# Lolash/graphSAGE-pytorch

Hardware: AMD Instinct MI355X
Metric: sampled nodes/sec (2-layer, fanout 25,10) at 1/2/4/8 MI355X (higher is better)
Workload: dtype fp32

## Files before the change

graphsage-pytorch_amd/_lib.py:

```python
import ctypes
import os

import torch

_HERE = os.path.dirname(os.path.abspath(__file__))
_ASAN_LIB = os.environ.get("GS_HOST_ASAN_LIB")
LIB_PATH = _ASAN_LIB or os.path.join(_HERE, "libgraphsage_amd.so")

GS_OK, GS_EINVAL, GS_ENOMEM, GS_EHIP, GS_ERANGE, GS_EEMPTY, GS_ELIMIT = range(7)
GS_F32, GS_BF16 = 0, 1
GS_AGG_MEAN, GS_AGG_MAX = 0, 1
GS_SAMPLE_GCN, GS_SAMPLE_FULL = 1, 2
GS_DSAMPLER_NO_AUX = 8
GS_DSAMPLER_FAST = 16
GS_SAMPLE_FAIL_EMPTY = 4
GS_MAX_HOPS = 8
GS_TOPT_FUSED_BWD, GS_TOPT_TOP_LAUNCH, GS_TOPT_SELF_ROWS, GS_TOPT_DEFER_UPDATE = range(4)
GS_OPT_SGD, GS_OPT_ADAM = 0, 1
(GS_PK_POS_PTR, GS_PK_POS, GS_PK_DST_IDS, GS_PK_NBR_PTR, GS_PK_NBR, GS_PK_SELF,
 GS_PK_TPTR, GS_PK_TIDX, GS_PK_NFIELDS) = range(9)

_i32, _i64, _u32, _u64, _f32, _f64 = (ctypes.c_int32, ctypes.c_int64, ctypes.c_uint32,
                                      ctypes.c_uint64, ctypes.c_float, ctypes.c_double)
_vp = ctypes.c_void_p
_p = ctypes.POINTER


class HopView(ctypes.Structure):
    _fields_ = [
        ("n_dst", _i64), ("n_pos", _i64), ("n_src", _i64), ("n_nbr", _i64),
        ("dst_ids", _p(_i64)), ("pos_ptr", _p(_i32)), ("pos", _p(_i32)),
        ("src_ids", _p(_i64)), ("nbr_ptr", _p(_i32)), ("nbr", _p(_i32)),
        ("self_local", _p(_i32)), ("set_ptr", _p(_i32)), ("set_items", _p(_i64)),
        ("n_empty", _i64),
    ]


class PackLayout(ctypes.Structure):
    _fields_ = [("total", _i64), ("off", (_i64 * GS_PK_NFIELDS) * GS_MAX_HOPS)]


_SIGS = {
    "gs_last_error": (ctypes.c_char_p, []),
    "gs_version": (ctypes.c_char_p, []),
    "gs_rng_create": (_i32, [_p(_vp)]),
    "gs_rng_destroy": (None, [_vp]),
    "gs_rng_seed_words": (_i32, [_vp, _vp, _i64]),
    "gs_rng_set_state": (_i32, [_vp, _vp, _i64]),
    "gs_rng_get_state": (_i32, [_vp, _vp, _p(_i64)]),
    "gs_rng_getrandbits": (_i32, [_vp, _i32, _i64, _vp]),
    "gs_rng_randbelow": (_i32, [_vp, _u32, _i64, _vp]),
    "gs_rng_sample_positions": (_i32, [_vp, _i64, _i64, _vp]),
    "gs_rng_choice_position": (_i32, [_vp, _i64, _p(_i64)]),
    "gs_pyset_union_of_lists": (_i32, [_vp, _vp, _i64, _vp, _p(_i64)]),
    "gs_graph_build": (_i32, [_vp, _vp, _i64, _i64, _i32, _p(_vp)]),
    "gs_graph_from_tables": (_i32, [_i64, _vp, _vp, _vp, _vp, _vp, _p(_vp)]),
    "gs_graph_destroy": (None, [_vp]),
    "gs_graph_dims": (_i32, [_vp, _p(_i64), _p(_i64), _p(_i64)]),
    "gs_graph_row_ptr": (_vp, [_vp]),
    "gs_graph_col": (_vp, [_vp]),
    "gs_graph_image_bytes": (_i64, [_vp]),
    "gs_graph_write_image": (_i32, [_vp, _vp, _i64]),
    "gs_graph_from_image": (_i32, [_vp, _i64, _p(_vp)]),
    "gs_rmat_pairs": (_i32, [_i32, _i64, _f64, _f64, _f64, _u64, _i32, _i32, _vp, _vp, _p(_i64)]),
    "gs_sample_run": (_i32, [_vp, _vp, _vp, _i64, _vp, _i32, _i32, _p(_vp)]),
    "gs_sample_destroy": (None, [_vp]),
    "gs_sample_n_hops": (_i32, [_vp, _p(_i32)]),
    "gs_sample_hop": (_i32, [_vp, _i32, _p(HopView)]),
    "gs_sample_pack_layout": (_i32, [_vp, _p(PackLayout)]),
    "gs_sample_pack": (_i32, [_vp, _vp, _i64]),
    "gs_sample_pack_bound": (_i64, [_vp, _i64, _vp, _i32]),
    "gs_sample_pack_run": (_i32, [_vp, _vp, _vp, _i64, _vp, _i32, _i32, _vp, _i64, _vp, _vp, _p(_i64)]),
    "gs_sample_pack_bound_multi": (_i64, [_vp, _i64, _i64, _vp, _i32]),
    "gs_sample_pack_run_multi": (_i32, [_vp, _vp, _vp, _i64, _i64, _vp, _i32, _i32, _vp, _i64, _vp, _vp,
                                        _p(_i64)]),
    "gs_fsample_pack_run": (_i32, [_vp, _u64, _i64, _vp, _i64, _vp, _i32, _i32, _vp, _i64, _vp, _vp, _p(_i64)]),
    "gs_philox4x32": (_i32, [_vp, _vp, _vp]),
    "gs_team_create": (_i32, [_i32, _p(_vp)]),
    "gs_team_create_shared": (_i32, [_vp, _p(_vp)]),
    "gs_team_destroy": (None, [_vp]),
    "gs_sample_pack_run_multi_team": (_i32, [_vp, _vp, _vp, _i64, _i64, _vp, _i32, _i32, _vp, _i64, _vp,
                                             _vp, _p(_i64), _vp]),
    "gs_fill_uniform": (_i32, [_vp, _i32, _i64, _i64, _i64, _u64, _vp]),
    "gs_uniform_host": (_i32, [_u64, _i64, _i64, _i64, _vp]),
    "gs_agg_fwd": (_i32, [_i32, _i32, _vp, _i64, _i64, _i64, _vp, _vp, _vp, _vp, _vp, _i32,
                          _vp, _i32, _i64, _vp, _vp]),
    "gs_sage_linear_fwd": (_i32, [_i32, _i64, _i64, _i64, _vp, _i64, _vp, _vp, _i64, _vp, _vp,
                                  _i64, _i32, _vp]),
    "gs_sage_linear_bwd_weight_ws": (_i64, [_i64, _i64, _i64]),
    "gs_sage_linear_bwd_weight": (_i32, [_i32, _i64, _i64, _i64, _vp, _i64, _vp, _vp, _i64, _vp,
                                         _vp, _i64, _i32, _vp, _vp, _i64, _vp]),
    "gs_sage_linear_bwd_input": (_i32, [_i64, _i64, _i64, _vp, _vp, _i64, _i32, _vp, _vp, _vp,
                                        _i64, _vp]),
    "gs_agg_bwd": (_i32, [_i32, _i64, _i64, _vp, _vp, _vp, _vp, _vp, _i64, _vp, _vp, _i64, _vp,
                          _vp]),
    "gs_sage1_fwd_supported": (_i32, [_i32, _i64, _i64, _i32]),
    "gs_sage1_fwd": (_i32, [_i32, _i32, _vp, _i64, _i64, _i64, _i64, _vp, _vp, _vp, _vp, _i32,
                            _vp, _vp, _i64, _vp, _i64, _i32, _vp]),
    "gs_cls_nll_ws_floats": (_i64, [_i64, _i64, _i64]),
    "gs_cls_nll_fwd_bwd": (_i32, [_i64, _i64, _i64, _vp, _vp, _vp, _vp, _vp, _i32, _vp, _vp, _vp,
                                  _vp, _vp, _vp]),
    "gs_clip_sgd": (_i32, [_i32, _vp, _vp, _vp, _f32, _f32, _f32, _vp, _vp]),
    "gs_clip_adam": (_i32, [_i32, _vp, _vp, _vp, _vp, _vp, _f32, _f32, _f32, _f32, _f32, _f32, _f32, _i64, _vp,
                            _vp]),
    "gs_unsup_create": (_i32, [_vp, _vp, _i64, _i32, _i32, _i32, _p(_vp)]),
    "gs_unsup_destroy": (None, [_vp]),
    "gs_unsup_attach_device": (_i32, [_vp, _vp]),
    "gs_unsup_extend": (_i32, [_vp, _vp, _vp, _i64, _i64, _i32, _i32, _vp]),
    "gs_unsup_fetch": (_i32, [_vp, _vp, _vp, _vp, _vp, _vp, _vp]),
    "gs_unsup_loss_plan": (_i32, [_vp, _vp, _i64, _vp, _p(_i64)]),
    "gs_unsup_loss_ws_floats": (_i64, [_i64, _i64, _i64]),
    "gs_unsup_loss_fwd": (_i32, [_i32, _i64, _i64, _i64, _i64, _i64, _vp, _i64, _vp, _f32, _f32, _vp, _vp,
                                 _vp]),
    "gs_unsup_loss_bwd": (_i32, [_i64, _i64, _i64, _i64, _i64, _vp, _i64, _vp, _vp, _vp, _vp, _i64, _vp]),
    "gs_cast_f32_bf16": (_i32, [_vp, _vp, _i64, _vp]),
    "gs_trainer_create": (_i32, [_vp, _p(_vp)]),
    "gs_trainer_destroy": (None, [_vp]),
    "gs_trainer_n_params": (_i64, [_vp]),
    "gs_trainer_ws_bytes": (_i64, [_vp, _vp]),
    "gs_trainer_forward_backward": (_i32, [_vp, _vp, _vp, _vp, _vp, _i64, _vp, _i64, _vp, _vp]),
    "gs_trainer_update": (_i32, [_vp, _f32, _vp, _vp]),
    "gs_trainer_update_local": (_i32, [_vp, _vp]),
    "gs_trainer_defer": (_i32, [_vp, _i32, _p(_i32), _vp]),
    "gs_trainer_gather_reserve": (_i32, [_vp, _i64, _i32]),
    "gs_trainer_gather": (_i32, [_vp, _vp, _vp, _vp, _i32, _vp]),
    "gs_trainer_forward_backward_gathered": (_i32, [_vp, _vp, _vp, _vp, _vp, _i64, _i32, _vp, _i64, _vp, _vp]),
    "gs_trainer_forward": (_i32, [_vp, _vp, _vp, _vp, _vp, _i64, _vp, _vp]),
    "gs_trainer_forward_gathered": (_i32, [_vp, _vp, _vp, _vp, _i32, _vp, _i64, _vp, _vp]),
    "gs_trainer_time_agg": (_i32, [_vp, _i64]),
    "gs_trainer_agg_times": (_i64, [_vp, _vp, _i64]),
    "gs_trainer_kernel_times": (_i64, [_vp, _i32, _vp, _i64]),
    "gs_trainer_kernel_block_stats": (_i64, [_vp, _i32, _vp, _i64]),
    "gs_trainer_kernel_stamps": (_i64, [_vp, _i32, _i64, _vp, _vp]),
    "gs_trainer_time_kernels": (_i32, [_vp, _i32, _i64]),
    "gs_trainer_time_kernels_every": (_i32, [_vp, _i32, _i64, _i64]),
    "gs_trainer_kernel_name": (ctypes.c_char_p, [_vp, _i32]),
    "gs_trainer_grads": (_vp, [_vp]),
    "gs_trainer_set_option": (_i32, [_vp, _i32, _i32]),
    "gs_trainer_set_optimizer": (_i32, [_vp, _vp]),
    "gs_trainer_opt_step": (_i64, [_vp]),
    "gs_trainer_capture": (_i32, [_vp, _vp, _i64, _vp, _i64]),
    "gs_trainer_captured": (_i64, [_vp]),
    "gs_comm_unique_id": (_i32, [_vp]),
    "gs_comm_create": (_i32, [_vp, _i32, _i32, _p(_vp)]),
    "gs_comm_destroy": (None, [_vp]),
    "gs_comm_allreduce_sum": (_i32, [_vp, _vp, _i64, _vp]),
    "gs_runner_create": (_i32, [_vp, _p(_vp)]),
    "gs_runner_run": (_i32, [_vp, _i64, _vp, _vp]),
    "gs_runner_stats_get": (_i32, [_vp, _vp]),
    "gs_runner_stats_reset": (None, [_vp]),
    "gs_runner_destroy": (None, [_vp]),
    "gs_runner_release": (_i32, [_vp, _i64]),
    "gs_runner_progress": (_i32, [_vp, _p(_i64), _p(_i64)]),
    "gs_runner_sync_rngs": (_i32, [_vp]),
    "gs_dsampler_create": (_i32, [_vp, _vp, _i32, _i64, _i32, _p(_vp)]),
    "gs_dsampler_destroy": (None, [_vp]),
    "gs_dsampler_set_rng": (_i32, [_vp, _vp, _i64, _vp]),
    "gs_dsampler_get_rng": (_i32, [_vp, _vp, _p(_i64), _vp]),
    "gs_dsampler_words": (_i32, [_vp, _i64, _vp, _vp]),
    "gs_dsampler_pack_bound": (_i64, [_vp, _i64]),
    "gs_dsampler_run": (_i32, [_vp, _vp, _i64, _vp, _i64, _vp]),
    "gs_dsampler_result": (_i32, [_vp, _vp, _vp, _p(_i64)]),
    "gs_dsampler_runs": (_i64, [_vp]),
    "gs_dsampler_result_of": (_i32, [_vp, _i64, _vp, _vp, _p(_i64)]),
    "gs_dsampler_debug": (_i32, [_vp, _vp, _i32]),
    "gs_dsampler_set_seed": (_i32, [_vp, _u64]),
    "gs_dsampler_run_at": (_i32, [_vp, _i64, _vp, _i64, _vp, _i64, _vp]),
    "gs_full_plan_create": (_i32, [_vp, _vp, _i64, _i32, _i64, _p(_vp)]),
    "gs_full_plan_destroy": (None, [_vp]),
    "gs_full_plan_dims": (_i32, [_vp, _vp]),
    "gs_full_plan_array": (_vp, [_vp, _i32]),
    "gs_agg_full_ws_bytes": (_i64, [_vp, _i64, _i64, _i64]),
    "gs_agg_full": (_i32, [_vp, _vp, _i32, _i32, _vp, _i64, _i64, _vp, _vp, _i64, _i64, _vp, _i64, _vp, _i64,
                           _vp]),
    "gs_infer_full_ws_bytes": (_i64, [_vp, _vp]),
    "gs_infer_full": (_i32, [_vp, _vp, _vp, _vp, _i64, _vp, _i64, _vp]),
    "gs_full_plan_transpose": (_i32, [_vp, _vp, _vp, _i64, _p(_vp)]),
    "gs_agg_full_argmax_ws_bytes": (_i64, [_vp, _i64, _i64, _i64]),
    "gs_agg_full_argmax": (_i32, [_vp, _vp, _i32, _vp, _i64, _i64, _vp, _vp, _i64, _i64, _vp, _i64, _vp, _i64, _vp,
                                  _i64, _vp]),
    "gs_agg_full_bwd_ws_bytes": (_i64, [_vp, _i64]),
    "gs_agg_full_bwd": (_i32, [_vp, _vp, _i32, _i64, _vp, _vp, _vp, _vp, _i64, _vp, _i64, _vp, _vp, _i64, _vp, _i64,
                               _vp]),
    "gs_train_full_ws_offset": (_i64, [_vp, _vp, _vp, _i32, _i32]),
    "gs_train_full_ws_bytes": (_i64, [_vp, _vp, _vp]),
    "gs_train_full_forward_backward": (_i32, [_vp, _vp, _vp, _vp, _vp, _vp, _i64, _i32, _i32, _vp, _vp, _i64, _vp]),
    "gs_full_field_bytes": (_i64, [_vp, _vp, _i32]),
    "gs_full_field_offset": (_i64, [_vp, _vp, _i32, _i32, _i32]),
    "gs_full_field_build": (_i32, [_vp, _vp, _vp, _vp, _vp, _vp, _vp, _i64, _i32, _vp, _vp]),
    "gs_full_field_counts": (_i32, [_vp, _vp, _vp, _vp]),
    "gs_agg_full_field": (_i32, [_vp, _vp, _vp, _vp, _i32, _i32, _i32, _vp, _i64, _i64, _vp, _vp, _vp, _i64, _vp,
                                 _i64, _vp, _i64, _vp]),
    "gs_agg_full_bwd_field": (_i32, [_vp, _vp, _vp, _vp, _i32, _i32, _i64, _vp, _vp, _vp, _vp, _i64, _vp, _i64, _vp,
                                     _i64, _vp, _i64, _vp, _i64, _vp]),
    "gs_train_full_field_forward_backward": (_i32, [_vp, _vp, _vp, _vp, _vp, _vp, _vp, _i64, _i32, _i32, _vp, _vp,
                                                    _i64, _vp]),
    "gs_train_full_unsup_ws_bytes": (_i64, [_i32, _i64, _i64, _i64, _i64]),
    "gs_train_full_unsup_forward_backward": (_i32, [_vp, _vp, _vp, _vp, _vp, _vp, _vp, _i64, _vp, _vp, _i64, _i32,
                                                    _i32, _vp, _vp, _i64, _vp]),
}

(GS_FP_N_NODES, GS_FP_N_ITEMS, GS_FP_N_SLOTS, GS_FP_N_SPLIT, GS_FP_N_EMPTY, GS_FP_SEG_LEN, GS_FP_GCN,
 GS_FP_N_ENTRIES, GS_FP_NDIMS) = range(9)
(GS_FP_ITEMS, GS_FP_ITEM_PTR, GS_FP_SLOT_PTR, GS_FP_SPLIT_PTR, GS_FP_SPLIT_ROWS, GS_FP_COUNT, GS_FP_SELF_LOOP,
 GS_FP_EMPTY_ROWS) = range(8)
GS_FP_T_ROW_PTR, GS_FP_T_COL = 8, 9
GS_TF_FORWARD, GS_TF_HEAD, GS_TF_BACKWARD, GS_TF_ALL = 1, 2, 4, 7
GS_FF_LAYER0, GS_FF_NCOUNTS = GS_MAX_HOPS + 1, GS_MAX_HOPS + 1 + 4 * GS_MAX_HOPS
GS_FF_ROWS, GS_FF_POS, GS_FF_ITEMS, GS_FF_SPLIT, GS_FF_T_ITEMS, GS_FF_T_SPLIT = range(6)


class FullPlanDev(ctypes.Structure):
    _fields_ = [("items", _vp), ("slot_ptr", _vp), ("split_rows", _vp), ("count", _vp), ("self_loop", _vp)]


class FullField(ctypes.Structure):
    _fields_ = [("n_layers", _i32), ("pad_", _i32), ("buf", _vp), ("buf_bytes", _i64), ("counts", _i64 * GS_FF_NCOUNTS)]


class InferFullConfig(ctypes.Structure):
    _fields_ = [
        ("n_layers", _i32), ("hidden", _i32), ("agg", _i32), ("feat_dtype", _i32),
        ("feat_dim", _i64), ("feat_ld", _i64), ("X", _vp), ("row_ptr", _vp), ("col", _vp),
        ("W", _vp * GS_MAX_HOPS), ("chunk_rows", _i64),
    ]


class TrainFullConfig(ctypes.Structure):
    _fields_ = [
        ("n_layers", _i32), ("hidden", _i32), ("n_classes", _i32), ("agg", _i32), ("feat_dtype", _i32),
        ("pad_", _i32), ("feat_dim", _i64), ("feat_ld", _i64), ("max_nodes", _i64), ("X", _vp), ("row_ptr", _vp),
        ("col", _vp), ("t_row_ptr", _vp), ("t_col", _vp), ("labels", _vp), ("params", _vp), ("grads", _vp),
    ]


class TrainFullUnsup(ctypes.Structure):
    _fields_ = [
        ("kind", _i32), ("with_sup", _i32), ("M", _i64), ("P", _i64), ("N", _i64), ("plan", _vp), ("q", _f32),
        ("margin", _f32),
    ]


class TrainerConfig(ctypes.Structure):
    _fields_ = [
        ("n_layers", _i32), ("hidden", _i32), ("n_classes", _i32), ("agg", _i32), ("gcn", _i32),
        ("feat_dtype", _i32), ("feat_dim", _i64), ("feat_ld", _i64),
        ("X", _vp), ("row_ptr", _vp), ("col", _vp), ("labels", _vp), ("params", _vp), ("grads", _vp),
        ("lr", _f32), ("max_norm", _f32),
    ]


class OptimizerConfig(ctypes.Structure):
    _fields_ = [
        ("kind", _i32), ("beta1", _f32), ("beta2", _f32), ("eps", _f32), ("weight_decay", _f32),
        ("m", _vp), ("v", _vp), ("step", _i64),
    ]


class RunnerConfig(ctypes.Structure):
    _fields_ = [
        ("graph", _vp), ("trainer", _vp), ("batches", _vp), ("n_batches", _i64), ("batch", _i64),
        ("fanouts", _vp), ("n_hops", _i32), ("flags", _i32), ("n_streams", _i32), ("rngs", _vp),
        ("depth", _i32), ("comm", _vp), ("world", _i32), ("embed_out", _vp), ("embed_ld", _i64),
        ("merge", _i32), ("hold", _i32), ("ar_buckets", _i32), ("helpers", _i32), ("warm", _i32),
        ("device_sampler", _i32), ("sampler_seed", _u64),
    ]


class RunnerStats(ctypes.Structure):
    _fields_ = [
        ("steps", _i64), ("wait_s", ctypes.c_double), ("issue_s", ctypes.c_double),
        ("sample_s", ctypes.c_double), ("hop_sizes", ctypes.c_double * (4 * GS_MAX_HOPS)),
        ("wait_sample_s", ctypes.c_double), ("wait_ring_s", ctypes.c_double),
        ("wait_gather_s", ctypes.c_double), ("fwd_bwd_s", ctypes.c_double), ("update_s", ctypes.c_double),
        ("max_step_s", ctypes.c_double), ("lookahead_misses", _i64),
    ]


_lib = None


class LibraryMissing(RuntimeError):
    pass


class DeviceLimit(RuntimeError):
    """GS_ELIMIT: a device-path capacity (the device sampler's rejection
    windows, walks or frontier tables) was too small for this batch.  The
    batch itself is valid and the caller's stream state is untouched, so the
    host path computes the same result."""


_DIAGNOSTIC = {"gs_trainer_kernel_block_stats", "gs_trainer_kernel_stamps"}


def lib():
    global _lib
    if _lib is None:
        if not os.path.exists(LIB_PATH):
            raise LibraryMissing(
                f"{LIB_PATH} is not built; run __graft_entry__.build() or "
                "`make -C graphsage-pytorch_amd/csrc` (no CPU fallback exists)")
        L = ctypes.CDLL(LIB_PATH)
        for name, (res, args) in _SIGS.items():
            if (_ASAN_LIB or name in _DIAGNOSTIC) and not hasattr(L, name):
                continue
            fn = getattr(L, name)
            fn.restype = res
            fn.argtypes = args
        _lib = L
    return _lib


def exported_symbols():
    return list(_SIGS)


def check(rc, what=""):
    if rc == GS_OK:
        return
    msg = lib().gs_last_error().decode(errors="replace") or what
    if rc in (GS_EINVAL,):
        raise ValueError(msg)
    if rc == GS_ERANGE:
        raise (ValueError if "Sample larger" in msg else IndexError)(msg)
    if rc == GS_EEMPTY:
        raise IndexError(msg)
    if rc == GS_ENOMEM:
        raise MemoryError(msg)
    if rc == GS_ELIMIT:
        raise DeviceLimit(msg)
    raise RuntimeError(msg)


def ptr(t):
    if t is None:
        return None
    if isinstance(t, torch.Tensor):
        return t.data_ptr()
    return t.ctypes.data


def stream_ptr(device=None):
    return torch.cuda.current_stream(device).cuda_stream
```

graphsage-pytorch_amd/csrc/kernels/agg.hip:

```cpp
#include "agg_dev.hpp"
#include "internal.hpp"

#include <algorithm>
#include <cstdlib>

namespace gs {

__global__ __launch_bounds__(kBlock) void resolve_ids_kernel(int n_dst, int k, const int* __restrict__ ptr,
                                                             const int* __restrict__ ent,
                                                             const int* __restrict__ col,
                                                             const int* __restrict__ dst_ids, int gcn,
                                                             int* __restrict__ ids) {
    const int64_t t = blockIdx.x * int64_t(kBlock) + threadIdx.x;
    if (t >= static_cast<int64_t>(n_dst) * k) return;
    const int r = static_cast<int>(t / k), j = static_cast<int>(t - static_cast<int64_t>(r) * k);
    const int e = ptr[r] + j;
    int nb = -1;
    if (e < ptr[r + 1]) nb = col[ent[e]];
    if (!gcn && nb == dst_ids[r]) nb = -1;
    ids[t] = nb;
}

__global__ __launch_bounds__(kBlock) void resolve_top_kernel(int n_dst, int k, const int* __restrict__ ptr,
                                                             const int* __restrict__ ent,
                                                             const int* __restrict__ col,
                                                             const int* __restrict__ dst_ids, int gcn,
                                                             int* __restrict__ ids, int n_top, int tk,
                                                             const int* __restrict__ tptr,
                                                             const int* __restrict__ tnbr,
                                                             const int* __restrict__ tself, int* __restrict__ tout,
                                                             int n_rec, const int* __restrict__ rptr,
                                                             const int* __restrict__ ridx, int* __restrict__ rout) {
    const int64_t t = blockIdx.x * int64_t(kBlock) + threadIdx.x;
    const int64_t n1 = static_cast<int64_t>(n_dst) * k;
    if (t < n1) {
        const int r = static_cast<int>(t / k), j = static_cast<int>(t - static_cast<int64_t>(r) * k);
        const int e = ptr[r] + j;
        int nb = -1;
        if (e < ptr[r + 1]) nb = col[ent[e]];
        if (!gcn && nb == dst_ids[r]) nb = -1;
        ids[t] = nb;
        return;
    }
    const int64_t u = t - n1;
    const int64_t n2 = static_cast<int64_t>(n_top) * (tk + 1);
    if (u >= n2) {
        const int64_t q = u - n2;
        if (q >= static_cast<int64_t>(n_rec) * 8) return;
        const int c = static_cast<int>(q >> 3), j = static_cast<int>(q & 7);
        const int b = rptr[c], n = rptr[c + 1] - b;
        rout[q] = j == 0 ? n : j == 1 ? b : (j - 2 < n ? ridx[b + j - 2] : 0);
        return;
    }
    const int r = static_cast<int>(u / (tk + 1)), j = static_cast<int>(u - static_cast<int64_t>(r) * (tk + 1));
    int v;
    if (j == 0) {
        v = tself[r];
    } else {
        const int e = tptr[r] + j - 1;
        v = e < tptr[r + 1] ? tnbr[e] : -1;
    }
    tout[u] = v;
}

template <typename T, int VEC>
struct RawVec {
    using type = T;
    static __device__ __forceinline__ void unpack(const T& r, float (&v)[VEC]) {
        RowIO<T, VEC>::load(&r, v);
    }
};
template <>
struct RawVec<float, 4> {
    using type = float4;
    static __device__ __forceinline__ void unpack(const float4& r, float (&v)[4]) {
        v[0] = r.x; v[1] = r.y; v[2] = r.z; v[3] = r.w;
    }
};
template <>
struct RawVec<bf16_t, 8> {
    using type = uint4;
    static __device__ __forceinline__ void unpack(const uint4& r, float (&v)[8]) {
        const uint32_t w[4] = {r.x, r.y, r.z, r.w};
#pragma unroll
        for (int i = 0; i < 4; ++i) {
            v[2 * i] = __uint_as_float(w[i] << 16);
            v[2 * i + 1] = __uint_as_float(w[i] & 0xffff0000u);
        }
    }
};

template <int OP, typename T, int VEC, int G, bool SELF, bool ONE, int NR1 = kRows>
__global__ __launch_bounds__(kBlock) void agg_ids_kernel(const T* __restrict__ X, int64_t ldx, int F, int n_dst, int k,
                                                         const int* __restrict__ ids, const int* __restrict__ dst_ids,
                                                         int gcn, T* __restrict__ out, int64_t ldo,
                                                         T* __restrict__ self_out, int64_t ldso) {
    const int gl = threadIdx.x % G;
    if constexpr (ONE) {
        using Raw = typename RawVec<T, VEC>::type;
        constexpr int NR = NR1;
        static_assert(NR % 4 == 0 && NR <= kRows, "row loads: whole chunks of 4");
        const int r = blockIdx.x * (kBlock / G) + threadIdx.x / G;
        if (r >= n_dst) return;
        const int f0 = gl * VEC;
        const int node = SELF ? dst_ids[r] : 0;
        const int nb = gl < k ? ids[static_cast<int64_t>(r) * k + gl] : -1;
        int rows[NR];
        bool ok[NR];
#pragma unroll
        for (int u = 0; u < NR; ++u) {
            rows[u] = __shfl(nb, u, G);
            ok[u] = u < k && rows[u] >= 0;
        }
        const int fallback = SELF ? node : (rows[0] >= 0 ? rows[0] : 0);
        Raw xself{};
        if (SELF) xself = *reinterpret_cast<const Raw*>(X + static_cast<int64_t>(node) * ldx + f0);
        Raw x[NR];
#pragma unroll
        for (int u = 0; u < NR; ++u)
            x[u] = *reinterpret_cast<const Raw*>(X + static_cast<int64_t>(ok[u] ? rows[u] : fallback) * ldx + f0);
        __builtin_amdgcn_sched_barrier(0);
        float acc[VEC];
#pragma unroll
        for (int v = 0; v < VEC; ++v) acc[v] = (OP == GS_AGG_MAX) ? -INFINITY : 0.f;
        int cnt = 0;
        int ka = k;
        asm volatile("" : "+s"(ka));
#pragma unroll
        for (int q = 0; q < NR / 4; ++q)
            if (4 * q < ka) {
#pragma unroll
                for (int u = 4 * q; u < 4 * q + 4; ++u) {
                    cnt += ok[u];
                    float xv[VEC];
                    RawVec<T, VEC>::unpack(x[u], xv);
#pragma unroll
                    for (int v = 0; v < VEC; ++v) {
                        if (OP == GS_AGG_MEAN) {
                            acc[v] += ok[u] ? xv[v] : 0.f;
                        } else {
                            const bool take = ok[u] && xv[v] > acc[v];
                            acc[v] = take ? xv[v] : acc[v];
                        }
                    }
                }
            }
        if (SELF) *reinterpret_cast<Raw*>(self_out + static_cast<int64_t>(r) * ldso + f0) = xself;
        if (OP == GS_AGG_MEAN) {
            const float inv = 1.0f / static_cast<float>(cnt);
#pragma unroll
            for (int v = 0; v < VEC; ++v) acc[v] *= inv;
        }
        RowIO<T, VEC>::store(out + static_cast<int64_t>(r) * ldo + f0, acc);
        return;
    }
    for (int r = blockIdx.x * (kBlock / G) + threadIdx.x / G; r < n_dst; r += gridDim.x * (kBlock / G)) {
    const int node = (gcn || SELF) ? dst_ids[r] : 0;
    const int* rid = ids + static_cast<int64_t>(r) * k;
    constexpr int NR = kRows;
    const int nf = (F + G * VEC - 1) / (G * VEC);
    for (int fi = 0; fi < nf; ++fi) {
        const int f0 = fi * G * VEC + gl * VEC;
        const bool act = f0 < F;
        const int f0c = act ? f0 : 0;
        using Raw = typename RawVec<T, VEC>::type;
        Raw xself{};
        if (SELF) xself = *reinterpret_cast<const Raw*>(X + static_cast<int64_t>(node) * ldx + f0c);
        float acc[VEC];
#pragma unroll
        for (int v = 0; v < VEC; ++v) acc[v] = (OP == GS_AGG_MAX) ? -INFINITY : 0.f;
        int cnt = 0;
        bool self_seen = false;
        for (int base = 0; base < k; base += G) {
            const int m = min(G, k - base);
            const bool mine = gl < m;
            const int nb = rid[mine ? base + gl : base];
            if (gcn) self_seen |= group_bits<G>(mine && nb == node) != 0;
            const int my = mine ? nb : -1;
            for (int j = 0; j < m; j += NR) {
                int rows[NR];
                bool ok[NR];
#pragma unroll
                for (int u = 0; u < NR; ++u) {
                    rows[u] = __shfl(my, j + u < m ? j + u : j, G);
                    ok[u] = (j + u < m) && rows[u] >= 0;
                }
                const int fallback = rows[0] >= 0 ? rows[0] : node;
                Raw x[NR];
#pragma unroll
                for (int u = 0; u < NR; ++u)
                    x[u] = *reinterpret_cast<const Raw*>(X + static_cast<int64_t>(ok[u] ? rows[u] : fallback) * ldx + f0c);
#pragma unroll
                for (int u = 0; u < NR; ++u) {
                    cnt += ok[u];
                    float xv[VEC];
                    RawVec<T, VEC>::unpack(x[u], xv);
#pragma unroll
                    for (int v = 0; v < VEC; ++v) {
                        if (OP == GS_AGG_MEAN) {
                            acc[v] += ok[u] ? xv[v] : 0.f;
                        } else {
                            const bool take = ok[u] && xv[v] > acc[v];
                            acc[v] = take ? xv[v] : acc[v];
                        }
                    }
                }
            }
        }
        if (gcn && !self_seen) {
            ++cnt;
            float x[VEC];
            RowIO<T, VEC>::load(X + static_cast<int64_t>(node) * ldx + f0c, x);
#pragma unroll
            for (int v = 0; v < VEC; ++v) {
                if (OP == GS_AGG_MEAN) acc[v] += x[v];
                else acc[v] = x[v] > acc[v] ? x[v] : acc[v];
            }
        }
        if (!act) continue;
        if (SELF) *reinterpret_cast<Raw*>(self_out + static_cast<int64_t>(r) * ldso + f0) = xself;
        if (OP == GS_AGG_MEAN) {
            const float inv = 1.0f / static_cast<float>(cnt);
#pragma unroll
            for (int v = 0; v < VEC; ++v) acc[v] *= inv;
        }
        RowIO<T, VEC>::store(out + static_cast<int64_t>(r) * ldo + f0, acc);
    }
    }
}

void resolve_ids_launch(int64_t n_dst, int k, const int32_t* ptr, const int32_t* ent, const int32_t* col,
                        const int32_t* dst_ids, int gcn, int32_t* ids, hipStream_t st) {
    GS_REQUIRE(n_dst >= 0 && k >= 1 && n_dst * k < (int64_t(1) << 31), GS_EINVAL, "bad sizes");
    if (n_dst == 0) return;
    const int64_t total = n_dst * k;
    resolve_ids_kernel<<<dim3(static_cast<unsigned>((total + kBlock - 1) / kBlock)), kBlock, 0, st>>>(
        static_cast<int>(n_dst), k, ptr, ent, col, dst_ids, gcn, ids);
    check_launch("resolve_ids");
}

void resolve_top_launch(int64_t n_dst, int k, const int32_t* ptr, const int32_t* ent, const int32_t* col,
                        const int32_t* dst_ids, int gcn, int32_t* ids, int64_t n_top, int tk, const int32_t* tptr,
                        const int32_t* tnbr, const int32_t* tself, int32_t* tout, hipStream_t st, int64_t n_rec,
                        const int32_t* rptr, const int32_t* ridx, int32_t* rout) {
    GS_REQUIRE(n_dst >= 0 && k >= 1 && n_dst * k < (int64_t(1) << 31) && n_top >= 0 && tk >= 1 &&
                   n_top * (tk + 1) < (int64_t(1) << 30) && n_rec >= 0 && n_rec < (int64_t(1) << 27) &&
                   (n_rec == 0 || (rptr && ridx && rout)),
               GS_EINVAL, "bad sizes");
    const int64_t total = n_dst * k + n_top * (tk + 1) + n_rec * 8;
    if (total == 0) return;
    resolve_top_kernel<<<dim3(static_cast<unsigned>((total + kBlock - 1) / kBlock)), kBlock, 0, st>>>(
        static_cast<int>(n_dst), k, ptr, ent, col, dst_ids, gcn, ids, static_cast<int>(n_top), tk, tptr, tnbr, tself,
        tout, static_cast<int>(n_rec), rptr, ridx, rout);
    check_launch("resolve_top");
}

static int agg_ids_block_cap() { return 1 << 30; }

void agg_ids_launch(gs_agg op, gs_dtype dt, const void* X, int64_t ldx, int64_t F, int64_t n_dst, int k,
                    const int32_t* ids, const int32_t* dst_ids, int gcn, void* out, int64_t ldo, hipStream_t st,
                    void* self_out, int64_t ldso, LaunchTimer* timer) {
    GS_REQUIRE(op == GS_AGG_MEAN || op == GS_AGG_MAX, GS_EINVAL, "agg_func must be MEAN or MAX");
    GS_REQUIRE(F >= 1 && n_dst >= 0 && k >= 1 && ldx >= F && ldo >= F, GS_EINVAL, "bad sizes");
    GS_REQUIRE(!self_out || (dst_ids && ldso >= F), GS_EINVAL, "self rows need dst_ids and ldso >= F");
    if (n_dst == 0) return;
    const int V = dt == GS_F32 ? 4 : 8;
    const bool vec = F % V == 0 && ldx % V == 0 && ldo % V == 0 && aligned16(X) && aligned16(out) &&
                     (!self_out || (ldso % V == 0 && aligned16(self_out)));
    const int f = static_cast<int>(F), n = static_cast<int>(n_dst);
    static const int cap = agg_ids_block_cap();
#define GS_IDS2(OPV, TT, VV, GG, ONE, NRV)                                                                       \
    do {                                                                                                         \
        const dim3 grid_(std::min((n + (kBlock / GG) - 1) / (kBlock / GG), cap));                                \
        if (self_out)                                                                                            \
            launch_k(timer, agg_ids_kernel<OPV, TT, VV, GG, true, ONE, NRV>, grid_, dim3(kBlock), 0, st,         \
                     static_cast<const TT*>(X), ldx, f, n, k, ids, dst_ids, gcn, static_cast<TT*>(out), ldo,      \
                     static_cast<TT*>(self_out), ldso);                                                          \
        else                                                                                                     \
            launch_k(timer, agg_ids_kernel<OPV, TT, VV, GG, false, ONE, NRV>, grid_, dim3(kBlock), 0, st,        \
                     static_cast<const TT*>(X), ldx, f, n, k, ids, dst_ids, gcn, static_cast<TT*>(out), ldo,      \
                     static_cast<TT*>(nullptr), ldso);                                                           \
    } while (0)
#define GS_IDS1(OPV, TT, VV, GG, ONE)                                                                            \
    do {                                                                                                         \
        if (!(ONE)) GS_IDS2(OPV, TT, VV, GG, false, kRows);                                                      \
        else if (k <= 4) GS_IDS2(OPV, TT, VV, GG, true, 4);                                                      \
        else if (k <= 8) GS_IDS2(OPV, TT, VV, GG, true, 8);                                                      \
        else if (k <= 12) GS_IDS2(OPV, TT, VV, GG, true, 12);                                                    \
        else GS_IDS2(OPV, TT, VV, GG, true, kRows);                                                              \
    } while (0)
    const bool one_ok = !gcn && k <= kRows && static_cast<int64_t>(n + 1) * 64 < (int64_t(1) << 31) &&
                        cap >= (n + 3) / 4;
#define GS_IDS(OPV, TT, VV, GG)                                      \
    do {                                                             \
        if (one_ok && f == (GG) * (VV)) GS_IDS1(OPV, TT, VV, GG, true); \
        else GS_IDS1(OPV, TT, VV, GG, false);                        \
    } while (0)
#define GS_IDS_T(OPV, TT)                                                     \
    do {                                                                      \
        constexpr int VV = sizeof(TT) == 4 ? 4 : 8;                           \
        if (!vec) GS_IDS(OPV, TT, 1, 64);                                     \
        else {                                                                \
            const int G = pick_group(f, VV);                                  \
            if (G == 16) GS_IDS(OPV, TT, VV, 16);                             \
            else if (G == 32) GS_IDS(OPV, TT, VV, 32);                        \
            else GS_IDS(OPV, TT, VV, 64);                                     \
        }                                                                     \
    } while (0)
    if (op == GS_AGG_MEAN) {
        if (dt == GS_F32) GS_IDS_T(GS_AGG_MEAN, float);
        else GS_IDS_T(GS_AGG_MEAN, bf16_t);
    } else {
        if (dt == GS_F32) GS_IDS_T(GS_AGG_MAX, float);
        else GS_IDS_T(GS_AGG_MAX, bf16_t);
    }
#undef GS_IDS_T
#undef GS_IDS
#undef GS_IDS1
#undef GS_IDS2
    check_launch("agg_ids");
}

template <int OP, typename T, bool EXPAND>
static void launch_fwd(int vec, const T* X, int64_t ldx, int F, int n_dst, const int* ptr,
                       const int* idx, const int64_t* row_ptr, const int* col, const int* dst_ids,
                       int gcn, T* out, int64_t ldo, int* am, hipStream_t st, LaunchTimer* timer) {
    constexpr int V = sizeof(T) == 4 ? 4 : 8;
    if (vec == 1) {
        const dim3 grid((n_dst + (kBlock / 64) - 1) / (kBlock / 64));
        launch_k(timer, agg_fwd_kernel<OP, T, 1, 64, EXPAND>, grid, dim3(kBlock), 0, st, X, ldx, F, n_dst, ptr, idx,
                 row_ptr, col, dst_ids, gcn, out, ldo, am);
        return;
    }
    const int G = pick_group(F, V);
    const dim3 grid((n_dst + (kBlock / G) - 1) / (kBlock / G));
#define GS_AGG_FWD(GG)                                                                                   \
    launch_k(timer, agg_fwd_kernel<OP, T, V, GG, EXPAND>, grid, dim3(kBlock), 0, st, X, ldx, F, n_dst, ptr, idx, \
             row_ptr, col, dst_ids, gcn, out, ldo, am)
    if (G == 16) GS_AGG_FWD(16);
    else if (G == 32) GS_AGG_FWD(32);
    else GS_AGG_FWD(64);
#undef GS_AGG_FWD
}

template <int OP>
static void launch_bwd(int vec, int n_src, int F, const int* tptr, const int* tidx, const int* ptr,
                       const float* dA, const float* dSelf, int64_t ldd, const int* am,
                       const float* Hprev, int64_t ldh, float* dH, hipStream_t st) {
    if (vec == 1) {
        const dim3 grid((n_src + 3) / 4);
        agg_bwd_kernel<OP, 1, 64><<<grid, kBlock, 0, st>>>(n_src, F, tptr, tidx, ptr, dA, dSelf, ldd, am,
                                                           Hprev, ldh, dH);
        return;
    }
    const int G = pick_group(F, 4);
    const dim3 grid((n_src + (kBlock / G) - 1) / (kBlock / G));
#define GS_AGG_BWD(GG)                                                                          \
    agg_bwd_kernel<OP, 4, GG><<<grid, kBlock, 0, st>>>(n_src, F, tptr, tidx, ptr, dA, dSelf, ldd, am, \
                                                       Hprev, ldh, dH)
    if (G == 16) GS_AGG_BWD(16);
    else if (G == 32) GS_AGG_BWD(32);
    else GS_AGG_BWD(64);
#undef GS_AGG_BWD
}

void agg_fwd_launch(gs_agg op, gs_dtype xdt, const void* X, int64_t ldx, int64_t F, int64_t n_dst,
                    const int32_t* ptr, const int32_t* idx, const int64_t* row_ptr, const int32_t* col,
                    const int32_t* dst_ids, int32_t gcn, void* out, gs_dtype odt, int64_t ldo, int32_t* argmax,
                    hipStream_t st, LaunchTimer* timer) {
    GS_REQUIRE(op == GS_AGG_MEAN || op == GS_AGG_MAX, GS_EINVAL, "agg_func must be MEAN or MAX");
    GS_REQUIRE(xdt == odt, GS_EINVAL, "output dtype must equal feature dtype");
    GS_REQUIRE(F >= 1 && F < (1 << 30) && n_dst >= 0 && n_dst < (int64_t(1) << 31), GS_EINVAL, "bad sizes");
    GS_REQUIRE(ldx >= F && ldo >= F, GS_EINVAL, "leading dimension smaller than F");
    if (n_dst == 0) return;
    GS_REQUIRE(X && ptr && idx && out, GS_EINVAL, "NULL device pointer");
    const bool expand = col != nullptr;
    GS_REQUIRE(!expand || dst_ids, GS_EINVAL, "expand mode needs dst_ids");
    GS_REQUIRE(!(argmax && expand), GS_EINVAL, "argmax is only produced in explicit mode");
    const int V = xdt == GS_F32 ? 4 : 8;
    const int vec = (F % V == 0 && ldx % V == 0 && ldo % V == 0 && aligned16(X) && aligned16(out)) ? V : 1;
    const int f = static_cast<int>(F), n = static_cast<int>(n_dst);
#define GS_DISPATCH(OPV, TT)                                                                              \
    do {                                                                                                  \
        if (expand)                                                                                       \
            launch_fwd<OPV, TT, true>(vec, static_cast<const TT*>(X), ldx, f, n, ptr, idx, row_ptr, col,  \
                                      dst_ids, gcn, static_cast<TT*>(out), ldo, nullptr, st, timer);      \
        else                                                                                              \
            launch_fwd<OPV, TT, false>(vec, static_cast<const TT*>(X), ldx, f, n, ptr, idx, nullptr,      \
                                       nullptr, nullptr, 0, static_cast<TT*>(out), ldo, argmax, st, timer); \
    } while (0)
    if (op == GS_AGG_MEAN) {
        if (xdt == GS_F32) GS_DISPATCH(GS_AGG_MEAN, float);
        else GS_DISPATCH(GS_AGG_MEAN, bf16_t);
    } else {
        if (xdt == GS_F32) GS_DISPATCH(GS_AGG_MAX, float);
        else GS_DISPATCH(GS_AGG_MAX, bf16_t);
    }
#undef GS_DISPATCH
    check_launch("gs_agg_fwd");
}

}

extern "C" {

int gs_agg_fwd(gs_agg op, gs_dtype xdt, const void* X, int64_t ldx, int64_t F, int64_t n_dst,
               const int32_t* ptr, const int32_t* idx, const int64_t* row_ptr, const int32_t* col,
               const int32_t* dst_ids, int32_t gcn, void* out, gs_dtype odt, int64_t ldo,
               int32_t* argmax, void* stream) {
    GS_API_BEGIN
    gs::agg_fwd_launch(op, xdt, X, ldx, F, n_dst, ptr, idx, row_ptr, col, dst_ids, gcn, out, odt, ldo, argmax,
                       gs::as_stream(stream));
    GS_API_END
}

int gs_agg_bwd(gs_agg op, int64_t n_src, int64_t F, const int32_t* tptr, const int32_t* tidx,
               const int32_t* ptr, const float* dA, const float* dSelf, int64_t ldd,
               const int32_t* argmax, const float* Hprev, int64_t ldh, float* dH, void* stream) {
    GS_API_BEGIN
    using namespace gs;
    GS_REQUIRE(op == GS_AGG_MEAN || op == GS_AGG_MAX, GS_EINVAL, "agg_func must be MEAN or MAX");
    GS_REQUIRE(F >= 1 && n_src >= 0 && n_src < (int64_t(1) << 31), GS_EINVAL, "bad sizes");
    GS_REQUIRE(ldd >= F && ldh >= F, GS_EINVAL, "leading dimension smaller than F");
    if (n_src == 0) return GS_OK;
    GS_REQUIRE(tptr && tidx && ptr && dA && dH, GS_EINVAL, "NULL device pointer");
    GS_REQUIRE(op != GS_AGG_MAX || argmax, GS_EINVAL, "MAX backward needs argmax");
    const int vec = (F % 4 == 0 && ldd % 4 == 0 && ldh % 4 == 0 && aligned16(dA) && (!dSelf || aligned16(dSelf)) &&
                     aligned16(dH) && (!Hprev || aligned16(Hprev)))
                        ? 4
                        : 1;
    hipStream_t st = as_stream(stream);
    if (op == GS_AGG_MEAN)
        launch_bwd<GS_AGG_MEAN>(vec, static_cast<int>(n_src), static_cast<int>(F), tptr, tidx, ptr, dA, dSelf,
                                ldd, argmax, Hprev, ldh, dH, st);
    else
        launch_bwd<GS_AGG_MAX>(vec, static_cast<int>(n_src), static_cast<int>(F), tptr, tidx, ptr, dA, dSelf,
                               ldd, argmax, Hprev, ldh, dH, st);
    check_launch("gs_agg_bwd");
    GS_API_END
}

}
```

graphsage-pytorch_amd/csrc/kernels/internal.hpp:

```cpp
#pragma once
#include <functional>

#include "kcommon.hpp"

struct gs_trainer;
struct gs_dsampler;

namespace gs {

void trainer_set_upper_hook(gs_trainer* t, std::function<void(hipStream_t)> hook);
void trainer_set_w1_chunk_hook(gs_trainer* t, int chunks,
                               std::function<void(hipStream_t, int64_t, int64_t)> hook);
void trainer_keep_lowp(gs_trainer* t, bool keep);
bool trainer_defer_update(gs_trainer* t, bool on, hipStream_t st, bool comm = false);
int64_t trainer_w1_floats(const gs_trainer* t);
void trainer_set_done(gs_trainer* t, int64_t* ptr, int64_t value);
bool trainer_done_taken(const gs_trainer* t);

bool linear_fwd_wide_ok(gs_dtype dt, int64_t F, const void* Xs, int64_t ldxs, const void* A, int64_t lda,
                        const void* W);
void linear_fwd_launch(gs_dtype dt, int64_t n, int64_t F, int64_t H, const void* Xs, int64_t ldxs,
                       const int32_t* sidx, const void* A, int64_t lda, const void* Wd, float* out, int64_t ldo,
                       int32_t relu, hipStream_t st, const FwdSpec* pend = nullptr, LaunchTimer* timer = nullptr);
int linear_dw_slabs(gs_dtype dt, int64_t n, int64_t F, int64_t H, const void* Xs, int64_t ldxs,
                    const int32_t* sidx, const void* A, int64_t lda, const float* dout, const float* out,
                    int64_t ldo, int32_t relu, float* dW, void* ws, int64_t ws_bytes, hipStream_t st,
                    int64_t H_split = -1, int phases = 1, LaunchTimer* timer = nullptr);
inline constexpr int kDw1Phases = 2;
int sum_slabs_launch(const float* slabs, int S, int64_t len, float* out, float* part, hipStream_t st);
struct SlabSum {
    const float* slabs;
    int S;
    int64_t len;
    float* out;
    float* part;
};
bool sum_slabs_pair_ok(int64_t len1, int64_t len2);
int sum_slabs_pair_parts2(int64_t len2);
int sum_slabs_pair_launch(const SlabSum& s1, const SlabSum& s2, hipStream_t st, const float* spec_P = nullptr,
                          float* spec_S = nullptr, float lr = 0.f, uint16_t* spec_S_lp = nullptr, DoneFlag done = {},
                          LaunchTimer* timer = nullptr);
void spec_finalize_launch(const FwdSpec& sp, float* w1_out, int64_t w1_floats, hipStream_t st);
int sum_slabs_grid(int64_t len);

void resolve_ids_launch(int64_t n_dst, int k, const int32_t* ptr, const int32_t* ent, const int32_t* col,
                        const int32_t* dst_ids, int gcn, int32_t* ids, hipStream_t st);
void resolve_top_launch(int64_t n_dst, int k, const int32_t* ptr, const int32_t* ent, const int32_t* col,
                        const int32_t* dst_ids, int gcn, int32_t* ids, int64_t n_top, int tk, const int32_t* tptr,
                        const int32_t* tnbr, const int32_t* tself, int32_t* tout, hipStream_t st, int64_t n_rec = 0,
                        const int32_t* rptr = nullptr, const int32_t* ridx = nullptr, int32_t* rout = nullptr);
void trainer_reserve_top(gs_trainer* t, int64_t B, int32_t tk);
void agg_ids_launch(gs_agg op, gs_dtype dt, const void* X, int64_t ldx, int64_t F, int64_t n_dst, int k,
                    const int32_t* ids, const int32_t* dst_ids, int gcn, void* out, int64_t ldo, hipStream_t st,
                    void* self_out = nullptr, int64_t ldso = 0, LaunchTimer* timer = nullptr);
void agg_fwd_launch(gs_agg op, gs_dtype xdt, const void* X, int64_t ldx, int64_t F, int64_t n_dst,
                    const int32_t* ptr, const int32_t* idx, const int64_t* row_ptr, const int32_t* col,
                    const int32_t* dst_ids, int32_t gcn, void* out, gs_dtype odt, int64_t ldo, int32_t* argmax,
                    hipStream_t st, LaunchTimer* timer = nullptr);

int cls_rows_launch(int64_t B, int64_t D, int64_t C, const float* E, const float* Wc, const float* bc,
                    const int32_t* labels, const int32_t* roots, int32_t mask_relu, float* dE, float* ws,
                    hipStream_t st);
void sgd_with_parts(int32_t n_groups, const int64_t* goff_host, const int* npart, int pstride, float* params,
                    float* grads, const float* part, float grad_scale, float max_norm, float lr, hipStream_t st,
                    LowpShadow shadow = {}, DoneFlag done = {});
void clip_sgd_launch(int32_t n_groups, const int64_t* goff_host, float* params, float* grads, float grad_scale,
                     float max_norm, float lr, float* ws, hipStream_t st, LowpShadow shadow = {}, DoneFlag done = {});
struct AdamStep {
    float lr, beta1, beta2, eps, weight_decay;
    int64_t step;
};
void adam_require(float beta1, float beta2, float eps, float weight_decay);
void adam_with_parts(int32_t n_groups, const int64_t* goff_host, const int* npart, int pstride, float* params,
                     float* grads, float* m, float* v, const float* part, float grad_scale, float max_norm,
                     const AdamStep& a, hipStream_t st, LowpShadow shadow = {}, DoneFlag done = {});
void clip_adam_launch(int32_t n_groups, const int64_t* goff_host, float* params, float* grads, float* m, float* v,
                      float grad_scale, float max_norm, const AdamStep& a, float* ws, hipStream_t st,
                      LowpShadow shadow = {}, DoneFlag done = {});
int sumsq_spec_launch(int32_t n_groups, const int64_t* goff_host, const float* grads, float* part, const float* P,
                      float* S, uint16_t* S_lp, int64_t n1, float lr, float scale, hipStream_t st, DoneFlag done = {});

struct LayerBwd {
    int64_t n, fin, H;
    const float* Xs;
    int64_t ldxs;
    const int32_t* sidx;
    const float* A;
    int64_t lda = 0;
    const float* dZ;
    const float* W;
    float* dW;
    float* slabs;
    int64_t slab_bytes;
    float* dIn;
    int agg;
    int64_t n_src;
    const int32_t* tptr;
    const int32_t* tidx;
    const int32_t* ptr;
    const int32_t* argmax;
    const int4* trec = nullptr;
    const float* Hprev;
    float* dH;
    bool din_ready = false;
};

struct ClsReduce {
    int64_t B, D, C;
    int n_row_blocks;
    const float* slab;
    float* dWc;
    float* dbc;
    float* loss;
    float* part;
};
int layer_bwd_top(const LayerBwd& a, const ClsReduce& cls, SlabSum* deferred, hipStream_t st);

bool layer_bwd_fusable(const LayerBwd& a);
int cls_reduce_grid(int64_t C, int64_t D);
int layer_bwd(const LayerBwd& a, const ClsReduce* cls, float* part, hipStream_t st);

bool top_supported(int64_t H, int64_t C, bool gcn);
int top_fwd_bwd(int agg, int64_t B, int64_t C, const float* Hprev, const int32_t* ptr, const int32_t* nbr,
                const int32_t* self, const float* W, const float* Wc, const float* bc, const int32_t* labels,
                const int32_t* roots, float* aggo, int32_t* argmax, float* E, float* dZ, float* dIn, float* slab,
                hipStream_t st, const int32_t* tids = nullptr, int tk = 0, LaunchTimer* timer = nullptr);

bool dsampler_ready(gs_dsampler* ds);
bool dsampler_run_ready(gs_dsampler* ds, int64_t run);

}
```

graphsage-pytorch_amd/csrc/kernels/step.hip:

```cpp
#include <algorithm>

#include "trainer.hpp"

namespace gs {

static inline void ok(int rc) {
    if (rc != GS_OK) fail(rc, gs_last_error());
}

static inline const int32_t* pack_field(const int32_t* pack, const int64_t* offsets, int hop, int f) {
    const int64_t o = offsets[(hop - 1) * GS_PK_NFIELDS + f];
    GS_REQUIRE(o >= 0, GS_EINVAL, "pack field missing");
    return pack + o;
}

static void gather1(gs_trainer& T, const int32_t* pack, const int64_t* hop_sizes, const int64_t* offsets,
                    void* out, hipStream_t st, int64_t ldo = 0) {
    const gs_trainer_config& c = T.cfg;
    const int L = c.n_layers;
    const int64_t F = c.feat_dim;
    auto fld = [&](int f) { return pack_field(pack, offsets, L, f); };
    LaunchTimer timed = timed_arm(T, 0);
    agg_fwd_launch(static_cast<gs_agg>(c.agg), static_cast<gs_dtype>(c.feat_dtype), c.X, c.feat_ld, F,
                   hop_sizes[4 * (L - 1)], fld(GS_PK_POS_PTR), fld(GS_PK_POS), nullptr, c.col, fld(GS_PK_DST_IDS),
                   c.gcn, out, static_cast<gs_dtype>(c.feat_dtype), ldo > 0 ? ldo : F, nullptr, st, &timed);
    timed_done(T, 0, timed);
}

static void gather1_ids(gs_trainer& T, const int32_t* pack, const int64_t* hop_sizes, const int64_t* offsets,
                        int slot, hipStream_t st) {
    const gs_trainer_config& c = T.cfg;
    const int L = c.n_layers;
    auto fld = [&](int f) { return pack_field(pack, offsets, L, f); };
    const int64_t n_dst = hop_sizes[4 * (L - 1)];
    int32_t* ids = T.ids_slot[slot];
    const int64_t n_top = hop_sizes[0];
    T.top_ready[slot] = T.top_k > 0 && L == 2 && !c.gcn && n_top <= T.top_rows && T.top_slot[slot] &&
                        hop_sizes[3] <= n_top * T.top_k;
    const int64_t n_rec = hop_sizes[2];
    T.rec_ready[slot] = T.top_ready[slot] && T.rec_slot[slot] && n_rec <= T.rec_rows;
    if (T.top_ready[slot]) {
        auto f1 = [&](int f) { return pack_field(pack, offsets, 1, f); };
        resolve_top_launch(n_dst, T.k_ids, fld(GS_PK_POS_PTR), fld(GS_PK_POS), c.col, fld(GS_PK_DST_IDS), c.gcn, ids,
                           n_top, T.top_k, f1(GS_PK_NBR_PTR), f1(GS_PK_NBR), f1(GS_PK_SELF), T.top_slot[slot], st,
                           T.rec_ready[slot] ? n_rec : 0, f1(GS_PK_TPTR), f1(GS_PK_TIDX), T.rec_slot[slot]);
    } else {
        resolve_ids_launch(n_dst, T.k_ids, fld(GS_PK_POS_PTR), fld(GS_PK_POS), c.col, fld(GS_PK_DST_IDS), c.gcn, ids,
                           st);
    }
    LaunchTimer timed = timed_arm(T, 0);
    if (T.self_rows) {
        char* base = static_cast<char*>(T.a1_slot[slot]);
        const int64_t xsz = c.feat_dtype == GS_BF16 ? 2 : 4;
        agg_ids_launch(static_cast<gs_agg>(c.agg), static_cast<gs_dtype>(c.feat_dtype), c.X, c.feat_ld, c.feat_dim,
                       n_dst, T.k_ids, ids, fld(GS_PK_DST_IDS), c.gcn, base + c.feat_dim * xsz, 2 * c.feat_dim, st,
                       base, 2 * c.feat_dim, &timed);
        T.self_in_slot[slot] = true;
    } else {
        agg_ids_launch(static_cast<gs_agg>(c.agg), static_cast<gs_dtype>(c.feat_dtype), c.X, c.feat_ld, c.feat_dim,
                       n_dst, T.k_ids, ids, fld(GS_PK_DST_IDS), c.gcn, T.a1_slot[slot], c.feat_dim, st, nullptr, 0,
                       &timed);
    }
    timed_done(T, 0, timed);
}

struct StepPlan {
    int64_t rows[GS_MAX_HOPS], in_dim[GS_MAX_HOPS];
    void* agg[GS_MAX_HOPS];
    float* h[GS_MAX_HOPS];
    int32_t* am[GS_MAX_HOPS];
    float *demb, *cls_ws, *dIn, *dbuf[2];
    char *dw_ws, *dw2_ws;
    int64_t dw_need, dw2_need, used;
};

static StepPlan plan_step(gs_trainer& T, const int64_t* hop_sizes, int64_t B, char* ws, int64_t ws_bytes, int a1_slot,
                          float* embed_out) {
    const gs_trainer_config& c = T.cfg;
    const int L = c.n_layers;
    const int64_t H = c.hidden, F = c.feat_dim;
    GS_REQUIRE(hop_sizes[0] == B, GS_EINVAL, "roots / hop-1 size mismatch");
    Carve cv{ws, ws_bytes};
    StepPlan p{};
    for (int l = 1; l <= L; ++l) {
        p.rows[l - 1] = hop_sizes[4 * (L - l)];
        p.in_dim[l - 1] = l == 1 ? F : H;
        if (l == 1) {
            if (a1_slot >= 0) {
                GS_REQUIRE(p.rows[0] <= T.a1_rows && T.a1_slot[a1_slot], GS_EINVAL, "gather slot too small");
                p.agg[0] = T.a1_slot[a1_slot];
            } else {
                p.agg[0] = cv.take<char>(p.rows[0] * F * (c.feat_dtype == GS_BF16 ? 2 : 4));
            }
        }
        else p.agg[l - 1] = cv.take<float>(p.rows[l - 1] * (L == 2 ? 2 * H : H));
        p.h[l - 1] = (embed_out && l == L) ? embed_out : cv.take<float>(p.rows[l - 1] * H);
        if (l >= 2 && c.agg == GS_AGG_MAX) p.am[l - 1] = cv.take<int32_t>(p.rows[l - 1] * H);
    }
    p.demb = cv.take<float>(B * H);
    p.cls_ws = cv.take<float>(gs_cls_nll_ws_floats(B, H, c.n_classes));
    int64_t dx_rows = 0, dprev_rows = 0;
    for (int l = 1; l <= L; ++l) {
        p.dw_need = std::max(p.dw_need, gs_sage_linear_bwd_weight_ws(p.rows[l - 1], T.w_cols[l - 1], H));
        if (l >= 2) {
            dx_rows = std::max(dx_rows, p.rows[l - 1]);
            dprev_rows = std::max(dprev_rows, p.rows[l - 2]);
        }
    }
    p.dw_ws = cv.take<char>(p.dw_need);
    p.dw2_need = L == 2 ? gs_sage_linear_bwd_weight_ws(p.rows[1], T.w_cols[1], H) : 0;
    p.dw2_ws = p.dw2_need > 0 ? cv.take<char>(p.dw2_need) : nullptr;
    p.dIn = cv.take<float>(dx_rows * (c.gcn ? H : 2 * H));
    p.dbuf[0] = cv.take<float>(dprev_rows * H);
    p.dbuf[1] = cv.take<float>(dprev_rows * H);
    p.used = cv.at;
    return p;
}

struct Layer1In {
    const void* x1;
    int64_t ldx1;
    const int32_t* sidx1;
    const void* a1;
    int64_t lda1;
};

struct Step {
    gs_trainer& T;
    const int32_t* pack;
    const int64_t* offsets;
    const int32_t* roots;
    int64_t B;
    float* loss;
    hipStream_t st;
    int a1_slot;
    const StepPlan p;
    const gs_trainer_config& c = T.cfg;
    const int L = c.n_layers;
    const int64_t H = c.hidden, F = c.feat_dim, K1 = T.w_cols[0];
    float *const P = c.params, *const G = c.grads;
    const gs_dtype dt = static_cast<gs_dtype>(c.feat_dtype);
    Layer1In in{};
    const void* W1 = nullptr;
    FwdSpec sp;
    bool pend = false;

    const int32_t* fld(int hop, int f) const { return pack_field(pack, offsets, hop, f); }

    void layer1_operands() {
        in = {c.gcn ? nullptr : c.X, c.feat_ld, fld(L, GS_PK_DST_IDS), p.agg[0], F};
        if (a1_slot >= 0 && T.self_rows) {
            in.a1 = static_cast<const char*>(p.agg[0]) + F * (dt == GS_BF16 ? 2 : 4);
            in.lda1 = 2 * F;
            if (T.self_in_slot[a1_slot] && !c.gcn) {
                in.x1 = p.agg[0];
                in.ldx1 = 2 * F;
                in.sidx1 = nullptr;
            }
        }
    }

    void cast_w1_lowp() {
        if (dt != GS_BF16) return;
        if (T.defer) {
            if (!T.lp_valid && !T.pending) {
                ok(gs_cast_f32_bf16(T.w1_buf(T.w1_cur), T.lp_buf(T.w1_cur), T.w_rows[0] * K1, st));
                T.lp_valid = true;
            }
        } else if (!(T.lp_keep && T.lp_valid)) {
            ok(gs_cast_f32_bf16(P + T.w_off[0], T.w1_lp, T.w_rows[0] * K1, st));
            T.lp_valid = T.lp_keep;
        }
    }

    void apply_pending_alone() {
        trainer_defer_update(&T, false, st);
        trainer_defer_update(&T, true, st);
    }

    void w1_for_forward() {
        const bool lowp = dt == GS_BF16;
        auto buf = [&](int i) { return lowp ? static_cast<const void*>(T.lp_buf(i)) : T.w1_buf(i); };
        W1 = lowp ? static_cast<const void*>(T.w1_lp) : P + T.w_off[0];
        pend = T.defer && T.pending;
        if (pend && !(T.pend_np[0] >= 1 && T.pend_np[0] <= 512 && T.pend_np[1] >= 1 && T.pend_np[1] <= 512 &&
                      linear_fwd_wide_ok(dt, F, in.x1, in.ldx1, in.a1, in.lda1, buf(T.w1_cur ^ 1)))) {
            apply_pending_alone();
            pend = false;
        }
        if (!T.defer) return;
        W1 = buf(pend ? T.w1_cur ^ 1 : T.w1_cur);
        if (!pend) return;
        sp = pending_spec(T);
        sp.Wn = T.w1_buf(T.w1_cur ^ 1);
        if (lowp) sp.S_lp = sp.Wn_lp = T.lp_buf(T.w1_cur ^ 1);
    }

    void forward_layer1() {
        LaunchTimer timed = timed_arm(T, 1);
        linear_fwd_launch(dt, p.rows[0], F, H, in.x1, in.ldx1, in.sidx1, in.a1, in.lda1, W1, p.h[0], H, 1, st, &sp,
                          &timed);
        timed_done(T, 1, timed);
        if (pend) {
            T.w1_cur ^= 1;
            T.pending = false;
        }
    }

    void forward_upper() {
        for (int l = 2; l <= L; ++l) {
            const int j = L - l + 1;
            ok(gs_agg_fwd(static_cast<gs_agg>(c.agg), GS_F32, p.h[l - 2], H, H, p.rows[l - 1], fld(j, GS_PK_NBR_PTR),
                          fld(j, GS_PK_NBR), nullptr, nullptr, nullptr, 0, p.agg[l - 1], GS_F32, H, p.am[l - 1], st));
            ok(gs_sage_linear_fwd(GS_F32, p.rows[l - 1], H, H, c.gcn ? nullptr : p.h[l - 2], H, fld(j, GS_PK_SELF),
                                  p.agg[l - 1], H, P + T.w_off[l - 1], p.h[l - 1], H, 1, st));
        }
    }

    bool layer_bwd_args(bool top, LayerBwd* lb) const {
        int flip_f = 0;
        bool fusable = true;
        for (int l = L; l >= 2; --l) {
            const int j = L - l + 1;
            LayerBwd& a = lb[L - l];
            a.n = p.rows[l - 1];
            a.fin = H;
            a.H = H;
            a.Xs = c.gcn ? nullptr : p.h[l - 2];
            a.ldxs = H;
            a.sidx = fld(j, GS_PK_SELF);
            a.A = static_cast<const float*>(p.agg[l - 1]);
            if (top && l == L) {
                a.Xs = static_cast<const float*>(p.agg[l - 1]);
                a.ldxs = 2 * H;
                a.sidx = nullptr;
                a.A = static_cast<const float*>(p.agg[l - 1]) + H;
                a.lda = 2 * H;
            }
            a.dZ = l == L ? p.demb : p.dbuf[flip_f ^ 1];
            a.W = P + T.w_off[l - 1];
            a.dW = G + T.w_off[l - 1];
            a.slabs = reinterpret_cast<float*>(p.dw_ws);
            a.slab_bytes = p.dw_need;
            a.dIn = p.dIn;
            a.agg = c.agg;
            a.n_src = p.rows[l - 2];
            a.tptr = fld(j, GS_PK_TPTR);
            a.tidx = fld(j, GS_PK_TIDX);
            a.ptr = fld(j, GS_PK_NBR_PTR);
            a.argmax = p.am[l - 1];
            a.Hprev = p.h[l - 2];
            a.dH = p.dbuf[flip_f];
            if (top && l == L && a1_slot >= 0 && T.rec_ready[a1_slot])
                a.trec = reinterpret_cast<const int4*>(T.rec_slot[a1_slot]);
            flip_f ^= 1;
            fusable = fusable && layer_bwd_fusable(a);
        }
        return fusable;
    }

    ClsReduce cls_reduce_role(int cls_rows) const {
        return {B, H, c.n_classes, cls_rows, p.cls_ws, G + T.cls_w_off, G + T.cls_b_off, loss, T.norm_part + T.pstride};
    }

    int dw1_slabs(const float* dH) {
        LaunchTimer timed = timed_arm(T, 2);
        const int S1 = linear_dw_slabs(dt, p.rows[0], F, H, in.x1, in.ldx1, in.sidx1, in.a1, in.lda1, dH, p.h[0], H, 0,
                                       G + T.w_off[0], p.dw_ws, p.dw_need, st, -1, kDw1Phases, &timed);
        timed_done(T, 2, timed);
        return S1;
    }

    void keep_norm_parts(int np, bool parts) {
        T.npart[0] = np;
        T.npart[1] = cls_reduce_grid(c.n_classes, H);
        T.norm_ready = parts && np <= T.pstride && T.npart[1] <= T.pstride;
    }

    void backward_fused(const LayerBwd* lb, int n_lb, const ClsReduce& cr) {
        const float* dws = reinterpret_cast<const float*>(p.dw_ws);
        int np = 0;
        bool parts = true;
        for (int i = 0; i < n_lb; ++i) {
            const int n = layer_bwd(lb[i], i == 0 ? &cr : nullptr, T.norm_part + np, st);
            parts = parts && n > 0;
            np += n;
        }
        if (T.upper_hook) T.upper_hook(st);
        const float* dH1 = lb[n_lb - 1].dH;
        if (T.w1_chunk_hook && T.w1_chunks > 1 && H % (64 * T.w1_chunks) == 0) {
            const int64_t Hc = H / T.w1_chunks;
            for (int q = 0; q < T.w1_chunks; ++q) {
                const int64_t h0 = q * Hc;
                float* dWq = G + T.w_off[0] + h0 * K1;
                const int Sq = linear_dw_slabs(dt, p.rows[0], F, Hc, in.x1, in.ldx1, in.sidx1, in.a1, in.lda1, dH1 + h0,
                                               p.h[0] + h0, H, 0, dWq, p.dw_ws, p.dw_need, st, H, kDw1Phases);
                if (Sq > 1) sum_slabs_launch(dws, Sq, Hc * K1, dWq, nullptr, st);
                T.w1_chunk_hook(st, T.w_off[0] + h0 * K1, Hc * K1);
            }
            T.npart[0] = 0;
            T.npart[1] = 0;
            T.norm_ready = false;
            return;
        }
        const int S1 = dw1_slabs(dH1);
        if (S1 > 1) np += sum_slabs_launch(dws, S1, H * K1, G + T.w_off[0], T.norm_part + np, st);
        else parts = false;
        keep_norm_parts(np, parts);
    }

    void backward_top(LayerBwd& lb2) {
        LaunchTimer timed = timed_arm(T, 3);
        const bool tids = a1_slot >= 0 && T.top_ready[a1_slot];
        const int cls_rows = top_fwd_bwd(c.agg, B, c.n_classes, p.h[0], fld(1, GS_PK_NBR_PTR), fld(1, GS_PK_NBR),
                                         fld(1, GS_PK_SELF), P + T.w_off[1], P + T.cls_w_off, P + T.cls_b_off, c.labels,
                                         roots, static_cast<float*>(p.agg[1]), p.am[1], p.h[1], p.demb, p.dIn, p.cls_ws,
                                         st, tids ? T.top_slot[a1_slot] : nullptr, tids ? T.top_k : 0, &timed);
        timed_done(T, 3, timed);
        lb2.din_ready = true;
        const ClsReduce cr = cls_reduce_role(cls_rows);
        const bool late_sum2 = !T.upper_hook && p.dw2_ws && sum_slabs_pair_ok(H * K1, H * T.w_cols[1]);
        if (!late_sum2) return backward_fused(&lb2, 1, cr);
        lb2.slabs = reinterpret_cast<float*>(p.dw2_ws);
        lb2.slab_bytes = p.dw2_need;
        SlabSum d2{};
        int np = layer_bwd_top(lb2, cr, &d2, st);
        bool parts = np > 0;
        const int S1 = dw1_slabs(lb2.dH);
        const int n_cls = cls_reduce_grid(c.n_classes, H);
        if (S1 > 1) {
            d2.part = T.norm_part;
            const bool spec = T.defer && !T.defer_comm && parts && np + sum_slabs_grid(H * K1) <= T.pstride &&
                              n_cls <= T.pstride;
            LaunchTimer timed4 = timed_arm(T, 4);
            const SlabSum s1{reinterpret_cast<const float*>(p.dw_ws), S1, H * K1, G + T.w_off[0], T.norm_part + np};
            np += sum_slabs_pair_launch(s1, d2, st, spec ? T.w1_buf(T.w1_cur) : nullptr,
                                        spec ? T.w1_buf(T.w1_cur ^ 1) : nullptr, c.lr,
                                        spec && dt == GS_BF16 ? T.lp_buf(T.w1_cur ^ 1) : nullptr,
                                        spec ? T.take_done() : DoneFlag{}, &timed4);
            timed_done(T, 4, timed4);
            T.pending = spec;
            if (spec) {
                T.pend_part = T.norm_part;
                T.pend_pstride = T.pstride;
                T.pend_np[0] = np;
                T.pend_np[1] = n_cls;
                T.pend_scale = 1.f;
            }
        } else {
            if (d2.S > 1) sum_slabs_launch(d2.slabs, d2.S, d2.len, d2.out, nullptr, st);
            parts = false;
        }
        keep_norm_parts(np, parts);
    }

    void backward_unfused() {
        ok(gs_cls_nll_fwd_bwd(B, H, c.n_classes, p.h[L - 1], P + T.cls_w_off, P + T.cls_b_off, c.labels, roots, 1, loss,
                              p.demb, G + T.cls_w_off, G + T.cls_b_off, p.cls_ws, st));
        const float* dH = p.demb;
        const int relu = 0;
        int flip = 0;
        for (int l = L; l >= 1; --l) {
            const int j = L - l + 1;
            const bool first = l == 1;
            const void* x_in = first ? in.x1 : (c.gcn ? nullptr : p.h[l - 2]);
            const int32_t* sidx = first ? in.sidx1 : fld(j, GS_PK_SELF);
            const int64_t fin = p.in_dim[l - 1], ldx = first ? in.ldx1 : H;
            if (first && L >= 2 && T.upper_hook) T.upper_hook(st);
            {
                const int64_t Kl = x_in ? 2 * fin : fin;
                const int Sl = linear_dw_slabs(first ? dt : GS_F32, p.rows[l - 1], fin, H, x_in, ldx, sidx,
                                               first ? in.a1 : p.agg[l - 1], first ? in.lda1 : fin, dH, p.h[l - 1], H,
                                               relu, G + T.w_off[l - 1], p.dw_ws, p.dw_need, st, -1,
                                               first ? kDw1Phases : 1);
                if (Sl > 1) sum_slabs_launch(reinterpret_cast<const float*>(p.dw_ws), Sl, H * Kl, G + T.w_off[l - 1],
                                             nullptr, st);
            }
            if (first) break;
            const int64_t ldd = c.gcn ? H : 2 * H;
            float* dSelf = c.gcn ? nullptr : p.dIn;
            float* dA = c.gcn ? p.dIn : p.dIn + H;
            ok(gs_sage_linear_bwd_input(p.rows[l - 1], H, H, dH, p.h[l - 1], H, relu, P + T.w_off[l - 1], dSelf, dA,
                                        ldd, st));
            float* dprev = p.dbuf[flip];
            flip ^= 1;
            ok(gs_agg_bwd(static_cast<gs_agg>(c.agg), p.rows[l - 2], H, fld(j, GS_PK_TPTR), fld(j, GS_PK_TIDX),
                          fld(j, GS_PK_NBR_PTR), dA, dSelf, ldd, p.am[l - 1], p.h[l - 2], H, dprev, st));
            dH = dprev;
        }
    }
};

static int64_t run_step(gs_trainer& T, const int32_t* pack, const int64_t* hop_sizes, const int64_t* offsets,
                        const int32_t* roots, int64_t B, char* ws, int64_t ws_bytes, float* loss, hipStream_t st,
                        int a1_slot = -1, float* embed_out = nullptr) {
    Step s{T, pack, offsets, roots, B, loss, st, a1_slot,
           plan_step(T, hop_sizes, B, ws, ws_bytes, a1_slot, embed_out)};
    const StepPlan& p = s.p;
    const int L = s.L;
    T.last_emb = p.h[L - 1];
    if (!ws) return p.used + 256;
    GS_REQUIRE(p.used <= ws_bytes, GS_EINVAL, "workspace too small");
    s.cast_w1_lowp();
    s.layer1_operands();
    GS_REQUIRE(!T.defer || !embed_out, GS_EINVAL, "deferred update: unsupported step");
    s.w1_for_forward();
    if (a1_slot < 0) gather1(T, pack, hop_sizes, offsets, p.agg[0], st);
    s.forward_layer1();
    const bool top = !embed_out && roots && T.fuse_bwd && T.use_top && L == 2 &&
                     top_supported(s.H, T.cfg.n_classes, T.cfg.gcn != 0);
    if (!top) s.forward_upper();
    if (embed_out) return p.used;
    T.norm_ready = false;
    if (T.fuse_bwd && L >= 2) {
        LayerBwd lb[GS_MAX_HOPS] = {};
        const bool fusable = s.layer_bwd_args(top, lb);
        GS_REQUIRE(!top || fusable, GS_EINVAL, "top launch needs the fused backward");
        if (fusable) {
            if (top) {
                s.backward_top(lb[0]);
            } else {
                const int cls_rows = cls_rows_launch(B, s.H, T.cfg.n_classes, p.h[L - 1], s.P + T.cls_w_off,
                                                     s.P + T.cls_b_off, T.cfg.labels, roots, 1, p.demb, p.cls_ws, st);
                s.backward_fused(lb, L - 1, s.cls_reduce_role(cls_rows));
            }
            return p.used;
        }
    }
    s.backward_unfused();
    return p.used;
}

static void capture_step(gs_trainer& T, int64_t B, hipStream_t st) {
    auto& c = T.cap;
    if (c.n >= c.max_steps || (!c.emb && !c.grads)) return;
    if (c.emb) {
        GS_REQUIRE(B * T.cfg.hidden <= c.emb_stride, GS_EINVAL, "capture: batch larger than the embedding stride");
        GS_REQUIRE(hipMemcpyAsync(c.emb + c.n * c.emb_stride, T.last_emb, B * T.cfg.hidden * sizeof(float),
                                  hipMemcpyDeviceToDevice, st) == hipSuccess,
                   GS_EHIP, "hipMemcpyAsync(capture)");
    }
    if (c.grads)
        GS_REQUIRE(hipMemcpyAsync(c.grads + c.n * T.total, T.cfg.grads, T.total * sizeof(float),
                                  hipMemcpyDeviceToDevice, st) == hipSuccess,
                   GS_EHIP, "hipMemcpyAsync(capture)");
    ++c.n;
}

void trainer_set_upper_hook(gs_trainer* t, std::function<void(hipStream_t)> hook) { t->upper_hook = std::move(hook); }
void trainer_set_w1_chunk_hook(gs_trainer* t, int chunks, std::function<void(hipStream_t, int64_t, int64_t)> hook) {
    t->w1_chunks = hook ? std::max(1, chunks) : 1;
    t->w1_chunk_hook = std::move(hook);
}

void trainer_reserve_top(gs_trainer* t, int64_t B, int32_t tk) {
    if (t->cfg.n_layers != 2 || t->cfg.gcn || tk < 1 || tk > 31 || B < 1) return;
    if (B <= t->top_rows && tk == t->top_k) return;
    for (int32_t*& p : t->top_slot) {
        if (p) GS_REQUIRE(hipFree(p) == hipSuccess, GS_EHIP, "hipFree");
        p = nullptr;
        GS_REQUIRE(hipMalloc(&p, std::max<int64_t>(B * (tk + 1) * 4, 256)) == hipSuccess, GS_ENOMEM,
                   "hipMalloc(top records)");
    }
    for (bool& r : t->top_ready) r = false;
    t->top_rows = B;
    t->top_k = tk;
    for (int32_t*& p : t->rec_slot) {
        if (p) GS_REQUIRE(hipFree(p) == hipSuccess, GS_EHIP, "hipFree");
        p = nullptr;
        GS_REQUIRE(hipMalloc(&p, std::max<int64_t>(t->a1_rows * 8 * 4, 256)) == hipSuccess, GS_ENOMEM,
                   "hipMalloc(backward records)");
    }
    for (bool& r : t->rec_ready) r = false;
    t->rec_rows = t->a1_rows;
}

int64_t trainer_w1_floats(const gs_trainer* t) { return t->w_rows[0] * t->w_cols[0]; }

void trainer_set_done(gs_trainer* t, int64_t* ptr, int64_t value) { t->done = {ptr, value}; }
bool trainer_done_taken(const gs_trainer* t) { return t->done.ptr == nullptr; }

}

extern "C" {

int gs_trainer_create(const gs_trainer_config* cfg, gs_trainer** out) {
    GS_API_BEGIN
    GS_REQUIRE(cfg && out, GS_EINVAL, "NULL argument");
    GS_REQUIRE(cfg->n_layers >= 1 && cfg->n_layers <= GS_MAX_HOPS, GS_EINVAL, "n_layers out of range");
    GS_REQUIRE(cfg->hidden >= 16 && cfg->hidden <= 256 && cfg->hidden % 16 == 0, GS_EINVAL, "bad hidden size");
    GS_REQUIRE(cfg->n_classes >= 1 && cfg->feat_dim >= 1 && cfg->feat_ld >= cfg->feat_dim, GS_EINVAL, "bad dims");
    GS_REQUIRE(cfg->X && cfg->col && cfg->labels && cfg->params && cfg->grads, GS_EINVAL,
               "NULL device pointer");
    auto* T = new gs_trainer();
    T->cfg = *cfg;
    int64_t at = 0;
    for (int l = 1; l <= cfg->n_layers; ++l) {
        const int64_t in = l == 1 ? cfg->feat_dim : cfg->hidden;
        T->w_off.push_back(at);
        T->w_rows.push_back(cfg->hidden);
        T->w_cols.push_back(cfg->gcn ? in : 2 * in);
        at += cfg->hidden * T->w_cols.back();
    }
    T->cls_w_off = at;
    at += static_cast<int64_t>(cfg->n_classes) * cfg->hidden;
    T->cls_b_off = at;
    at += cfg->n_classes;
    T->total = at;
    {
        int64_t np = 0;
        for (int l = 1; l <= cfg->n_layers; ++l) np += gs::sum_slabs_grid(cfg->hidden * T->w_cols[l - 1]);
        np = std::max<int64_t>({np, gs::cls_reduce_grid(cfg->n_classes, cfg->hidden), 64});
        T->pstride = static_cast<int>((np + 63) / 64 * 64);
        if (hipMalloc(&T->norm_part, 2 * T->pstride * sizeof(float)) != hipSuccess) {
            delete T;
            gs::fail(GS_ENOMEM, "hipMalloc(norm partials)");
        }
        if (cfg->feat_dtype == GS_BF16 &&
            hipMalloc(&T->w1_lp, T->w_rows[0] * T->w_cols[0] * sizeof(uint16_t)) != hipSuccess) {
            delete T;
            gs::fail(GS_ENOMEM, "hipMalloc(bf16 W1)");
        }
    }
    *out = T;
    GS_API_END
}

void gs_trainer_destroy(gs_trainer* t) { delete t; }

int64_t gs_trainer_n_params(const gs_trainer* t) { return t ? t->total : -1; }

float* gs_trainer_grads(const gs_trainer* t) { return t ? t->cfg.grads : nullptr; }

int gs_trainer_set_option(gs_trainer* t, int32_t opt, int32_t value) {
    GS_API_BEGIN
    GS_REQUIRE(t, GS_EINVAL, "NULL argument");
    GS_REQUIRE(!t->defer && !t->pending, GS_EINVAL, "options cannot change inside a runner loop");
    const bool on = value != 0;
    switch (opt) {
        case GS_TOPT_FUSED_BWD: t->fuse_bwd = on; break;
        case GS_TOPT_TOP_LAUNCH: t->use_top = on; break;
        case GS_TOPT_SELF_ROWS: t->want_self_rows = on; break;
        case GS_TOPT_DEFER_UPDATE: t->opt_defer = on; break;
        default: GS_REQUIRE(false, GS_EINVAL, "unknown trainer option");
    }
    GS_API_END
}

int64_t gs_trainer_ws_bytes(gs_trainer* t, const int64_t* hop_sizes) {
    try {
        std::vector<int64_t> off(GS_MAX_HOPS * GS_PK_NFIELDS, 0);
        return gs::run_step(*t, nullptr, hop_sizes, off.data(), nullptr, hop_sizes[0], nullptr, 0, nullptr,
                            nullptr);
    } catch (const gs::Error& e) {
        gs::set_error(e.what());
        return -1;
    }
}

int gs_trainer_forward_backward(gs_trainer* t, const int32_t* pack, const int64_t* hop_sizes,
                                const int64_t* offsets, const int32_t* roots, int64_t n_roots, void* ws,
                                int64_t ws_bytes, float* loss, void* stream) {
    GS_API_BEGIN
    GS_REQUIRE(t && pack && hop_sizes && offsets && roots && ws && loss, GS_EINVAL, "NULL argument");
    gs::run_step(*t, pack, hop_sizes, offsets, roots, n_roots, static_cast<char*>(ws), ws_bytes, loss,
                 gs::as_stream(stream));
    gs::capture_step(*t, n_roots, gs::as_stream(stream));
    GS_API_END
}

int gs_trainer_capture(gs_trainer* t, float* emb, int64_t emb_stride, float* grads, int64_t max_steps) {
    GS_API_BEGIN
    GS_REQUIRE(t && max_steps >= 0 && (!emb || emb_stride >= t->cfg.hidden), GS_EINVAL, "bad arguments");
    t->cap = {};
    t->cap.emb = emb;
    t->cap.emb_stride = emb_stride;
    t->cap.grads = grads;
    t->cap.max_steps = max_steps;
    GS_API_END
}

int64_t gs_trainer_captured(const gs_trainer* t) { return t ? t->cap.n : -1; }

int gs_trainer_gather_reserve(gs_trainer* t, int64_t max_rows, int32_t max_fanout) {
    GS_API_BEGIN
    GS_REQUIRE(t && max_rows >= 0 && max_fanout >= 0, GS_EINVAL, "bad arguments");
    const bool self_rows = t->want_self_rows && !t->cfg.gcn && t->cfg.n_layers >= 1;
    if (max_rows <= t->a1_rows && max_fanout <= t->k_ids && self_rows == t->self_rows) return GS_OK;
    max_rows = std::max(max_rows, t->a1_rows);
    t->self_rows = self_rows;
    for (bool& b : t->self_in_slot) b = false;
    const int64_t bytes = max_rows * t->cfg.feat_dim * (self_rows ? 2 : 1) * (t->cfg.feat_dtype == GS_BF16 ? 2 : 4);
    for (void*& p : t->a1_slot) {
        if (p) GS_REQUIRE(hipFree(p) == hipSuccess, GS_EHIP, "hipFree");
        p = nullptr;
        GS_REQUIRE(hipMalloc(&p, std::max<int64_t>(bytes, 256)) == hipSuccess, GS_ENOMEM, "hipMalloc(gather slot)");
    }
    for (int32_t*& p : t->ids_slot) {
        if (p) GS_REQUIRE(hipFree(p) == hipSuccess, GS_EHIP, "hipFree");
        p = nullptr;
    }
    t->k_ids = 0;
    if (max_fanout > 0) {
        GS_REQUIRE(max_rows * max_fanout < (int64_t(1) << 31), GS_EINVAL, "gather slot too large for int32 ids");
        for (int32_t*& p : t->ids_slot)
            GS_REQUIRE(hipMalloc(&p, std::max<int64_t>(max_rows * max_fanout * 4, 256)) == hipSuccess, GS_ENOMEM,
                       "hipMalloc(gather ids)");
        t->k_ids = max_fanout;
    }
    t->a1_rows = max_rows;
    GS_API_END
}

int gs_trainer_gather(gs_trainer* t, const int32_t* pack, const int64_t* hop_sizes, const int64_t* offsets,
                      int32_t slot, void* stream) {
    GS_API_BEGIN
    GS_REQUIRE(t && pack && hop_sizes && offsets && slot >= 0 && slot < gs_trainer::kSlots, GS_EINVAL,
               "bad arguments");
    const int L = t->cfg.n_layers;
    GS_REQUIRE(hop_sizes[4 * (L - 1)] <= t->a1_rows && t->a1_slot[slot], GS_EINVAL,
               "gather slot too small (gs_trainer_gather_reserve)");
    const int64_t n_dst = hop_sizes[4 * (L - 1)], n_pos = hop_sizes[4 * (L - 1) + 1];
    if (t->k_ids > 0 && n_pos <= n_dst * t->k_ids) {
        gs::gather1_ids(*t, pack, hop_sizes, offsets, slot, gs::as_stream(stream));
    } else if (t->self_rows) {
        const int64_t F = t->cfg.feat_dim, xsz = t->cfg.feat_dtype == GS_BF16 ? 2 : 4;
        gs::gather1(*t, pack, hop_sizes, offsets, static_cast<char*>(t->a1_slot[slot]) + F * xsz,
                    gs::as_stream(stream), 2 * F);
        t->self_in_slot[slot] = false;
    } else {
        gs::gather1(*t, pack, hop_sizes, offsets, t->a1_slot[slot], gs::as_stream(stream));
    }
    GS_API_END
}

int gs_trainer_forward_backward_gathered(gs_trainer* t, const int32_t* pack, const int64_t* hop_sizes,
                                         const int64_t* offsets, const int32_t* roots, int64_t n_roots,
                                         int32_t slot, void* ws, int64_t ws_bytes, float* loss, void* stream) {
    GS_API_BEGIN
    GS_REQUIRE(t && pack && hop_sizes && offsets && roots && ws && loss && slot >= 0 && slot < gs_trainer::kSlots,
               GS_EINVAL, "bad arguments");
    gs::run_step(*t, pack, hop_sizes, offsets, roots, n_roots, static_cast<char*>(ws), ws_bytes, loss,
                 gs::as_stream(stream), slot);
    gs::capture_step(*t, n_roots, gs::as_stream(stream));
    GS_API_END
}

int gs_trainer_forward(gs_trainer* t, const int32_t* pack, const int64_t* hop_sizes, const int64_t* offsets,
                       void* ws, int64_t ws_bytes, float* out, void* stream) {
    GS_API_BEGIN
    GS_REQUIRE(t && pack && hop_sizes && offsets && ws && out, GS_EINVAL, "NULL argument");
    gs::run_step(*t, pack, hop_sizes, offsets, nullptr, hop_sizes[0], static_cast<char*>(ws), ws_bytes, nullptr,
                 gs::as_stream(stream), -1, out);
    GS_API_END
}

int gs_trainer_forward_gathered(gs_trainer* t, const int32_t* pack, const int64_t* hop_sizes,
                                const int64_t* offsets, int32_t slot, void* ws, int64_t ws_bytes, float* out,
                                void* stream) {
    GS_API_BEGIN
    GS_REQUIRE(t && pack && hop_sizes && offsets && ws && out && slot >= 0 && slot < gs_trainer::kSlots, GS_EINVAL,
               "bad arguments");
    gs::run_step(*t, pack, hop_sizes, offsets, nullptr, hop_sizes[0], static_cast<char*>(ws), ws_bytes, nullptr,
                 gs::as_stream(stream), slot, out);
    GS_API_END
}

}
```

graphsage-pytorch_amd/csrc/kernels/trainer.hpp:

```cpp
#pragma once
#include <string>
#include <vector>

#include "internal.hpp"

struct gs_trainer {
    gs_trainer_config cfg;
    std::vector<int64_t> w_off;
    std::vector<int64_t> w_rows, w_cols;
    int64_t cls_w_off = 0, cls_b_off = 0, total = 0;
    static constexpr int kSites = 5;
    struct Timer {
        std::vector<hipEvent_t> ev0, ev1;
        int64_t n = 0;
        int64_t every = 1, calls = 0;
        std::string kernel;
        unsigned long long* st0 = nullptr;
        unsigned long long* st1 = nullptr;
        std::vector<char> stamped;
    } timer[kSites];
    static constexpr int kSlots = 3;
    void* a1_slot[kSlots] = {};
    int64_t a1_rows = 0;
    bool self_rows = false;
    bool self_in_slot[kSlots] = {};
    int32_t* ids_slot[kSlots] = {};
    int k_ids = 0;
    int32_t* top_slot[kSlots] = {};
    bool top_ready[kSlots] = {};
    int64_t top_rows = 0;
    int top_k = 0;
    int32_t* rec_slot[kSlots] = {};
    int64_t rec_rows = 0;
    bool rec_ready[kSlots] = {};
    bool fuse_bwd = true;
    bool use_top = true;
    bool want_self_rows = true;
    bool opt_defer = true;
    float* norm_part = nullptr;
    int pstride = 0;
    int npart[2] = {0, 0};
    bool norm_ready = false;
    std::function<void(hipStream_t)> upper_hook;
    std::function<void(hipStream_t, int64_t, int64_t)> w1_chunk_hook;
    int w1_chunks = 1;
    uint16_t* w1_lp = nullptr;
    bool lp_keep = false, lp_valid = false;
    bool defer = false, pending = false;
    bool defer_comm = false;
    const float* pend_part = nullptr;
    int pend_pstride = 0;
    int pend_np[2] = {0, 0};
    float pend_scale = 1.f;
    float* w1_alt = nullptr;
    int w1_cur = 0;
    float* w1_buf(int i) { return i == 0 ? cfg.params + w_off[0] : w1_alt; }
    uint16_t* w1_lp_alt = nullptr;
    uint16_t* lp_buf(int i) { return i == 0 ? w1_lp : w1_lp_alt; }
    struct Capture {
        float* emb = nullptr;
        int64_t emb_stride = 0;
        float* grads = nullptr;
        int64_t max_steps = 0, n = 0;
    } cap;
    const float* last_emb = nullptr;
    gs_optimizer_config opt{GS_OPT_SGD, 0.9f, 0.999f, 1e-8f, 0.f, nullptr, nullptr, 0};
    gs::DoneFlag done;
    gs::DoneFlag take_done() {
        const gs::DoneFlag d = done;
        done = {};
        return d;
    }
    ~gs_trainer() {
        if (w1_alt) (void)hipFree(w1_alt);
        if (w1_lp_alt) (void)hipFree(w1_lp_alt);
        if (norm_part) (void)hipFree(norm_part);
        if (w1_lp) (void)hipFree(w1_lp);
        for (auto& tm : timer) {
            for (auto e : tm.ev0) (void)hipEventDestroy(e);
            for (auto e : tm.ev1) (void)hipEventDestroy(e);
        }
        for (void* p : a1_slot)
            if (p) (void)hipFree(p);
        for (int32_t* p : ids_slot)
            if (p) (void)hipFree(p);
        for (int32_t* p : top_slot)
            if (p) (void)hipFree(p);
        for (int32_t* p : rec_slot)
            if (p) (void)hipFree(p);
        for (auto& tm : timer)
            if (tm.st0) (void)hipFree(tm.st0);
    }
};

namespace gs {

struct Carve {
    char* base;
    int64_t cap, at = 0;
    template <class T>
    T* take(int64_t n) {
        at = (at + 255) & ~int64_t(255);
        T* p = base ? reinterpret_cast<T*>(base + at) : nullptr;
        at += n * static_cast<int64_t>(sizeof(T));
        return p;
    }
};

LaunchTimer timed_arm(gs_trainer& T, int site);
void timed_done(gs_trainer& T, int site, const LaunchTimer& lt);

FwdSpec pending_spec(gs_trainer& T);

}
```

graphsage-pytorch_amd/csrc/runtime/runner.hip:

```cpp
#include <rccl/rccl.h>
#include <sys/mman.h>

#include <algorithm>
#include <atomic>
#include <chrono>
#include <condition_variable>
#include <sched.h>
#include <cstdio>
#include <cstdlib>
#include <cstring>
#include <deque>
#include <memory>
#include <mutex>
#include <string>
#include <thread>
#include <vector>

#include "../kernels/internal.hpp"

namespace gs {

using Clock = std::chrono::steady_clock;

static double secs(Clock::time_point a, Clock::time_point b) {
    return std::chrono::duration<double>(b - a).count();
}

static void hip_ok(hipError_t e, const char* what) {
    if (e != hipSuccess) fail(GS_EHIP, std::string(what) + ": " + hipGetErrorString(e));
}

static unsigned sync_event_flags() {
    return hipEventDisableTiming | static_cast<unsigned>(hipEventDisableSystemFence);
}

struct PackSlot {
    int32_t* host = nullptr;
    int32_t* dev = nullptr;
    size_t thp_bytes = 0;
    int64_t batch = -1;
    int64_t hop_sizes[4 * GS_MAX_HOPS];
    int64_t offsets[GS_MAX_HOPS * GS_PK_NFIELDS];
    int64_t used = 0;
    double sample_s = 0;
    int status = GS_OK;
    std::string error;
};

struct SamplerStream {
    gs_rng* rng = nullptr;
    gs_team* team = nullptr;
    std::vector<int64_t> batches;
    std::vector<PackSlot> slots;
    std::deque<int> free, ready;
    struct Consumed {
        int slot;
        int64_t batch;
    };
    std::deque<Consumed> copying;
    std::mutex mu;
    std::condition_variable cv;
    std::thread th;
};

}

namespace gs {
struct Inflight {
    int stream = -1, slot = -1;
};
}

struct gs_runner {
    gs_runner_config cfg{};
    std::vector<int32_t> fanouts;
    std::vector<int64_t> roots;
    int64_t cap = 0;
    int64_t merge = 1;
    int64_t n_units = 0;
    std::vector<std::unique_ptr<gs::SamplerStream>> streams;
    std::atomic<bool> stop{false};
    std::atomic<int64_t> release_mark{INT64_MAX};
    std::atomic<int64_t> sampled{0};
    std::mutex warm_mu;
    std::condition_variable warm_cv;
    int warmed = 0;
    int64_t next_batch = 0;
    hipStream_t comm_stream = nullptr;
    hipEvent_t upper_ready = nullptr, upper_reduced = nullptr;
    hipEvent_t w1_ready = nullptr;
    int w1_issued = 0;
    static constexpr int kDev = 3;
    hipStream_t copy_stream = nullptr;
    hipEvent_t dev_done[kDev] = {};
    bool dev_busy[kDev] = {};
    int64_t entry_batch[kDev] = {-1, -1, -1};
    int64_t done_upto = -1;
    bool use_flag = false;
    int64_t* done_host = nullptr;
    int64_t* done_dev = nullptr;
    int64_t flag_step[kDev] = {-1, -1, -1};
    void wait_flag(int64_t want) {
        const auto t0 = std::chrono::steady_clock::now();
        for (uint64_t spin = 0; __atomic_load_n(done_host, __ATOMIC_ACQUIRE) < want; ++spin) {
            __builtin_ia32_pause();
            if ((spin & 63) == 63) sched_yield();
            if ((spin & 0xfffff) == 0xfffff && std::chrono::steady_clock::now() - t0 > std::chrono::seconds(5)) {
                gs::hip_ok(hipDeviceSynchronize(), "hipDeviceSynchronize");
                if (__atomic_load_n(done_host, __ATOMIC_ACQUIRE) < want)
                    gs::fail(GS_EHIP, "runner: step completion flag never arrived");
            }
        }
        done_upto = std::max(done_upto, want);
    }
    void wait_entry(int k) {
        if (flag_step[k] >= 0) {
            wait_flag(flag_step[k]);
            flag_step[k] = -1;
        }
        if (dev_busy[k]) gs::hip_ok(hipEventSynchronize(dev_done[k]), "hipEventSynchronize");
        done_upto = std::max(done_upto, entry_batch[k]);
    }
    bool step_done(int64_t b, bool block) {
        if (b <= done_upto) return true;
        if (use_flag) {
            const int64_t seen = __atomic_load_n(done_host, __ATOMIC_ACQUIRE);
            if (seen >= b) {
                done_upto = std::max(done_upto, seen);
                return true;
            }
        }
        const int k = static_cast<int>(b % kDev);
        if (dev_busy[k] && entry_batch[k] >= b) {
            const hipError_t e = block ? hipEventSynchronize(dev_done[k]) : hipEventQuery(dev_done[k]);
            if (e == hipErrorNotReady) return false;
            gs::hip_ok(e, "step event");
            done_upto = std::max(done_upto, entry_batch[k]);
            return true;
        }
        if (!block) return false;
        GS_REQUIRE(use_flag && flag_step[k] >= b, GS_EINVAL, "runner: a consumed slot's step signals nowhere");
        wait_flag(b);
        return true;
    }
    hipEvent_t gathered[kDev] = {};
    hipStream_t side = nullptr;
    gs::Inflight inflight[kDev];
    int64_t issued = 0;
    void* ws = nullptr;
    int64_t ws_bytes = 0;
    float* clip_ws = nullptr;
    int device = 0;
    gs_runner_stats stats{};

    static constexpr int kDevDepthMax = 2;
    struct DevStream {
        gs_dsampler* ds = nullptr;
        hipStream_t st = nullptr;
        int nq = 0;
        int64_t qb[kDevDepthMax] = {}, qrun[kDevDepthMax] = {};
        hipEvent_t t0[kDevDepthMax] = {}, t1[kDevDepthMax] = {};
        bool counted[kDevDepthMax] = {};
        int64_t next = 0;
    };
    int dev_depth = kDevDepthMax;
    struct DevResult {
        int64_t hop_sizes[4 * GS_MAX_HOPS];
        int64_t offsets[GS_MAX_HOPS * GS_PK_NFIELDS];
        int64_t used = 0;
        double sample_s = 0;
    };
    bool devmode = false;
    bool fastmode = false;
    std::recursive_mutex dev_mu;
    std::vector<DevStream> dstreams;
    int32_t* roots_dev = nullptr;
    int64_t n_dpack = 0, dcap = 0;
    std::vector<int32_t*> dpack;
    std::vector<DevResult> dres;
    void dev_enqueue(int w);
    bool dev_take(int64_t b, bool block);
    void dev_poll();
    void dev_sync_rngs();

    ~gs_runner();
    void sampler_loop(gs::SamplerStream& s);
    void recycle(gs::SamplerStream& s, bool block);
    bool issue(int64_t b, bool block);
    int take_slot(int64_t b, bool block);
};

void gs_runner::recycle(gs::SamplerStream& s, bool block) {
    int n_back = 0;
    while (!s.copying.empty()) {
        const int q = s.copying.front().slot;
        if (!step_done(s.copying.front().batch, block && n_back == 0)) break;
        s.copying.pop_front();
        {
            std::lock_guard<std::mutex> lk(s.mu);
            s.free.push_back(q);
        }
        ++n_back;
    }
    if (n_back) s.cv.notify_all();
}

void gs_runner::sampler_loop(gs::SamplerStream& s) {
    const hipError_t dev_err = hipSetDevice(device);
    if (cfg.warm) {
        gs_rng* tmp = nullptr;
        uint32_t mt[624];
        int64_t pos = 0;
        if (!s.batches.empty() && !s.free.empty() && gs_rng_create(&tmp) == GS_OK &&
            gs_rng_get_state(s.rng, mt, &pos) == GS_OK && gs_rng_set_state(tmp, mt, pos) == GS_OK) {
            gs::PackSlot& slot = s.slots[s.free.front()];
            const int64_t b = s.batches.back();
            const int64_t nb = std::min(merge, cfg.n_batches - b * merge);
            (void)gs_sample_pack_run_multi_team(cfg.graph, tmp, roots.data() + b * merge * cfg.batch, nb * cfg.batch,
                                                cfg.batch, fanouts.data(), cfg.n_hops, cfg.flags, slot.host, cap,
                                                slot.hop_sizes, slot.offsets, &slot.used, s.team);
        }
        if (tmp) gs_rng_destroy(tmp);
        {
            std::lock_guard<std::mutex> lk(warm_mu);
            ++warmed;
        }
        warm_cv.notify_all();
    }
    for (int64_t b : s.batches) {
        int slot_id;
        {
            std::unique_lock<std::mutex> lk(s.mu);
            s.cv.wait(lk, [&] { return stop.load() || (!s.free.empty() && b < release_mark.load()); });
            if (stop) return;
            slot_id = s.free.front();
            s.free.pop_front();
        }
        gs::PackSlot& slot = s.slots[slot_id];
        const auto t0 = gs::Clock::now();
        slot.batch = b;
        const int64_t nb = std::min(merge, cfg.n_batches - b * merge);
        slot.status = gs_sample_pack_run_multi_team(cfg.graph, s.rng, roots.data() + b * merge * cfg.batch,
                                                    nb * cfg.batch, cfg.batch, fanouts.data(), cfg.n_hops, cfg.flags,
                                                    slot.host, cap, slot.hop_sizes, slot.offsets, &slot.used, s.team);
        if (slot.status != GS_OK) {
            slot.error = gs_last_error();
        } else {
            hipError_t e = dev_err;
            if (e == hipSuccess)
                e = hipMemcpyAsync(slot.dev, slot.host, static_cast<size_t>(slot.used) * sizeof(int32_t),
                                   hipMemcpyHostToDevice, copy_stream);
            if (e == hipSuccess) e = hipStreamSynchronize(copy_stream);
            if (e != hipSuccess) {
                slot.status = GS_EHIP;
                slot.error = std::string("runner: pack copy to the device: ") + hipGetErrorString(e);
            }
        }
        slot.sample_s = gs::secs(t0, gs::Clock::now());
        {
            std::lock_guard<std::mutex> lk(s.mu);
            s.ready.push_back(slot_id);
        }
        sampled.fetch_add(1);
        s.cv.notify_all();
        if (slot.status != GS_OK) return;
    }
}

int gs_runner::take_slot(int64_t b, bool block) {
    using namespace gs;
    SamplerStream& s = *streams[b % cfg.n_streams];
    int slot_id;
    const auto tw = Clock::now();
    for (;;) {
        std::unique_lock<std::mutex> lk(s.mu);
        if (!s.ready.empty()) {
            slot_id = s.ready.front();
            s.ready.pop_front();
            break;
        }
        if (!block) return -1;
        s.cv.wait(lk, [&] { return !s.ready.empty() || (s.free.empty() && !s.copying.empty()); });
        if (!s.ready.empty()) continue;
        lk.unlock();
        recycle(s, true);
    }
    stats.wait_sample_s += secs(tw, Clock::now());
    PackSlot& slot = s.slots[slot_id];
    GS_REQUIRE(slot.batch == b, GS_EINVAL, "sampler ring out of order");
    if (slot.status != GS_OK) fail(slot.status, slot.error);
    return slot_id;
}

void gs_runner::dev_enqueue(int w) {
    using namespace gs;
    std::lock_guard<std::recursive_mutex> lk(dev_mu);
    DevStream& d = dstreams[w];
    while (d.nq < dev_depth) {
        const int64_t b = d.next;
        if (b >= n_units || b >= release_mark.load()) return;
        const int q = d.nq;
        hip_ok(hipEventRecord(d.t0[q], d.st), "hipEventRecord");
        const int rc = fastmode ? gs_dsampler_run_at(d.ds, b, roots_dev + b * cfg.batch, cfg.batch, dpack[b % n_dpack],
                                                     dcap, d.st)
                                : gs_dsampler_run(d.ds, roots_dev + b * cfg.batch, cfg.batch, dpack[b % n_dpack], dcap,
                                                  d.st);
        if (rc != GS_OK) fail(rc, gs_last_error());
        hip_ok(hipEventRecord(d.t1[q], d.st), "hipEventRecord");
        d.qb[q] = b;
        d.qrun[q] = gs_dsampler_runs(d.ds) - 1;
        d.counted[q] = false;
        d.nq = q + 1;
        d.next = b + cfg.n_streams;
    }
}

bool gs_runner::dev_take(int64_t b, bool block) {
    using namespace gs;
    std::lock_guard<std::recursive_mutex> lk(dev_mu);
    DevStream& d = dstreams[b % cfg.n_streams];
    const bool queued = d.nq > 0 && d.qb[0] == b;
    if (!block && (!queued || !dsampler_run_ready(d.ds, d.qrun[0]))) return false;
    GS_REQUIRE(queued, GS_EINVAL, "device sampler: batch not enqueued (past the release mark?)");
    const auto tw = Clock::now();
    DevResult& R = dres[b % n_dpack];
    const int rc = gs_dsampler_result_of(d.ds, d.qrun[0], R.hop_sizes, R.offsets, &R.used);
    if (rc != GS_OK) fail(rc, gs_last_error());
    hip_ok(hipEventSynchronize(d.t1[0]), "hipEventSynchronize");
    float ms = 0.f;
    hip_ok(hipEventElapsedTime(&ms, d.t0[0], d.t1[0]), "hipEventElapsedTime");
    R.sample_s = 1e-3 * ms;
    stats.wait_sample_s += secs(tw, Clock::now());
    if (!d.counted[0]) sampled.fetch_add(1);
    const hipEvent_t e0 = d.t0[0], e1 = d.t1[0];
    for (int q = 1; q < kDevDepthMax; ++q) {
        d.qb[q - 1] = d.qb[q];
        d.qrun[q - 1] = d.qrun[q];
        d.t0[q - 1] = d.t0[q];
        d.t1[q - 1] = d.t1[q];
        d.counted[q - 1] = d.counted[q];
    }
    d.t0[kDevDepthMax - 1] = e0;
    d.t1[kDevDepthMax - 1] = e1;
    --d.nq;
    return true;
}

void gs_runner::dev_poll() {
    std::lock_guard<std::recursive_mutex> lk(dev_mu);
    for (auto& d : dstreams)
        for (int q = 0; q < d.nq; ++q)
            if (!d.counted[q] && gs::dsampler_run_ready(d.ds, d.qrun[q])) {
                d.counted[q] = true;
                sampled.fetch_add(1);
            }
}

void gs_runner::dev_sync_rngs() {
    using namespace gs;
    if (fastmode) return;
    for (int w = 0; w < static_cast<int>(dstreams.size()); ++w) {
        DevStream& d = dstreams[w];
        if (!d.ds) continue;
        uint32_t mt[624];
        int64_t pos = 0;
        int rc = gs_dsampler_get_rng(d.ds, mt, &pos, d.st);
        if (rc != GS_OK) fail(rc, gs_last_error());
        rc = gs_rng_set_state(cfg.rngs[w], mt, pos);
        if (rc != GS_OK) fail(rc, gs_last_error());
    }
}

bool gs_runner::issue(int64_t b, bool block) {
    using namespace gs;
    int slot_id = -1;
    if (devmode) {
        if (!dev_take(b, block)) return false;
    } else {
        slot_id = take_slot(b, block);
        if (slot_id < 0) return false;
    }
    const auto tr = Clock::now();
    const int k = static_cast<int>(b % kDev);
    wait_entry(k);
    stats.wait_ring_s += secs(tr, Clock::now());
    if (devmode) {
        const DevResult& R = dres[b % n_dpack];
        const int rc = gs_trainer_gather(cfg.trainer, dpack[b % n_dpack], R.hop_sizes, R.offsets, k, side);
        if (rc != GS_OK) fail(rc, gs_last_error());
        hip_ok(hipEventRecord(gathered[k], side), "hipEventRecord");
        inflight[k] = {-1, static_cast<int>(b % n_dpack)};
        issued = b + 1;
        dev_enqueue(static_cast<int>(b % cfg.n_streams));
        return true;
    }
    const Inflight f{static_cast<int>(b % cfg.n_streams), slot_id};
    PackSlot& slot = streams[f.stream]->slots[f.slot];
    const int rc = gs_trainer_gather(cfg.trainer, slot.dev, slot.hop_sizes, slot.offsets, k, side);
    if (rc != GS_OK) fail(rc, gs_last_error());
    hip_ok(hipEventRecord(gathered[k], side), "hipEventRecord");
    inflight[k] = f;
    issued = b + 1;
    return true;
}

gs_runner::~gs_runner() {
    if (devmode) {
        for (auto& d : dstreams)
            if (d.st) (void)hipStreamSynchronize(d.st);
        try {
            dev_sync_rngs();
        } catch (...) {
        }
        for (auto& d : dstreams) {
            if (d.ds) gs_dsampler_destroy(d.ds);
            for (int q = 0; q < kDevDepthMax; ++q) {
                if (d.t0[q]) (void)hipEventDestroy(d.t0[q]);
                if (d.t1[q]) (void)hipEventDestroy(d.t1[q]);
            }
            if (d.st) (void)hipStreamDestroy(d.st);
        }
    }
    stop = true;
    for (auto& s : streams) {
        { std::lock_guard<std::mutex> lk(s->mu); }
        s->cv.notify_all();
    }
    for (auto& s : streams)
        if (s->th.joinable()) s->th.join();
    for (auto& s : streams) gs_team_destroy(s->team);
    if (copy_stream) (void)hipStreamSynchronize(copy_stream);
    if (side) (void)hipStreamSynchronize(side);
    if (comm_stream) (void)hipStreamSynchronize(comm_stream);
    for (int d = 0; d < kDev; ++d)
        if (dev_busy[d]) (void)hipEventSynchronize(dev_done[d]);
    if (done_host) (void)hipHostFree(done_host);
    for (auto& s : streams)
        for (auto& slot : s->slots) {
            if (slot.host && slot.thp_bytes) {
                (void)hipHostUnregister(slot.host);
                munmap(slot.host, slot.thp_bytes);
            } else if (slot.host) {
                (void)hipHostFree(slot.host);
            }
            if (slot.dev) (void)hipFree(slot.dev);
        }
    for (int32_t* p : dpack)
        if (p) (void)hipFree(p);
    if (roots_dev) (void)hipFree(roots_dev);
    for (int d = 0; d < kDev; ++d) {
        if (dev_done[d]) (void)hipEventDestroy(dev_done[d]);
        if (gathered[d]) (void)hipEventDestroy(gathered[d]);
    }
    if (cfg.trainer && comm_stream) {
        gs::trainer_set_upper_hook(cfg.trainer, {});
        gs::trainer_set_w1_chunk_hook(cfg.trainer, 1, {});
    }
    if (w1_ready) (void)hipEventDestroy(w1_ready);
    if (upper_ready) (void)hipEventDestroy(upper_ready);
    if (upper_reduced) (void)hipEventDestroy(upper_reduced);
    if (comm_stream) (void)hipStreamDestroy(comm_stream);
    if (side) (void)hipStreamDestroy(side);
    if (copy_stream) (void)hipStreamDestroy(copy_stream);
    if (ws) (void)hipFree(ws);
    if (clip_ws) (void)hipFree(clip_ws);
}

extern "C" {

int gs_comm_unique_id(uint8_t id[128]) {
    GS_API_BEGIN
    GS_REQUIRE(id, GS_EINVAL, "NULL argument");
    static_assert(sizeof(ncclUniqueId) == 128, "ncclUniqueId size");
    ncclUniqueId u;
    GS_REQUIRE(ncclGetUniqueId(&u) == ncclSuccess, GS_EHIP, "ncclGetUniqueId failed");
    std::memcpy(id, &u, 128);
    GS_API_END
}

int gs_comm_create(const uint8_t id[128], int32_t n_ranks, int32_t rank, void** comm) {
    GS_API_BEGIN
    GS_REQUIRE(id && comm && n_ranks >= 1 && rank >= 0 && rank < n_ranks, GS_EINVAL, "bad arguments");
    ncclUniqueId u;
    std::memcpy(&u, id, 128);
    ncclComm_t c = nullptr;
    const ncclResult_t r = ncclCommInitRank(&c, n_ranks, u, rank);
    GS_REQUIRE(r == ncclSuccess, GS_EHIP, std::string("ncclCommInitRank: ") + ncclGetErrorString(r));
    *comm = c;
    GS_API_END
}

void gs_comm_destroy(void* comm) {
    if (comm) (void)ncclCommDestroy(static_cast<ncclComm_t>(comm));
}

int gs_comm_allreduce_sum(void* comm, float* buf, int64_t n, void* stream) {
    GS_API_BEGIN
    GS_REQUIRE(comm && buf && n >= 0, GS_EINVAL, "bad arguments");
    const ncclResult_t r = ncclAllReduce(buf, buf, static_cast<size_t>(n), ncclFloat32, ncclSum,
                                         static_cast<ncclComm_t>(comm), gs::as_stream(stream));
    GS_REQUIRE(r == ncclSuccess, GS_EHIP, std::string("ncclAllReduce: ") + ncclGetErrorString(r));
    GS_API_END
}

int gs_runner_create(const gs_runner_config* cfg, gs_runner** out) {
    GS_API_BEGIN
    using namespace gs;
    GS_REQUIRE(cfg && out, GS_EINVAL, "NULL argument");
    const bool fast = cfg->device_sampler == 2;
    GS_REQUIRE(cfg->graph && cfg->trainer && cfg->batches && (cfg->rngs || fast), GS_EINVAL,
               "NULL pointer in config");
    GS_REQUIRE(cfg->device_sampler >= 0 && cfg->device_sampler <= 2, GS_EINVAL, "device_sampler out of [0, 2]");
    GS_REQUIRE(cfg->n_batches >= 1 && cfg->batch >= 1 && cfg->batch < (int64_t(1) << 30), GS_EINVAL,
               "bad batch shape");
    GS_REQUIRE(cfg->n_hops >= 1 && cfg->n_hops <= GS_MAX_HOPS, GS_EINVAL, "n_hops out of [1, 8]");
    GS_REQUIRE(cfg->n_streams >= 1 && cfg->n_streams <= 64 && cfg->depth >= 1 && cfg->depth <= 64, GS_EINVAL,
               "n_streams / depth out of range");
    GS_REQUIRE(cfg->world >= 1 && (cfg->world == 1 || cfg->comm), GS_EINVAL, "world > 1 needs a communicator");
    GS_REQUIRE(!cfg->embed_out || (cfg->embed_ld >= 1 && !cfg->comm), GS_EINVAL,
               "embed_out needs embed_ld >= 1 and no communicator");
    GS_REQUIRE(cfg->merge <= 1 || cfg->embed_out, GS_EINVAL, "merge > 1 is inference only (embed_out)");
    GS_REQUIRE(cfg->helpers >= 0 && cfg->helpers <= 64, GS_EINVAL, "helpers out of [0, 64]");
    for (int32_t w = 0; w < cfg->n_streams && !fast; ++w) GS_REQUIRE(cfg->rngs[w], GS_EINVAL, "NULL rng");
    std::unique_ptr<gs_runner> r(new gs_runner());
    r->cfg = *cfg;
    r->fanouts.assign(cfg->fanouts ? cfg->fanouts : nullptr, cfg->fanouts ? cfg->fanouts + cfg->n_hops : nullptr);
    if (r->fanouts.empty()) r->fanouts.assign(cfg->n_hops, 10);
    r->cfg.fanouts = r->fanouts.data();
    r->roots.assign(cfg->batches, cfg->batches + cfg->n_batches * cfg->batch);
    r->cfg.batches = r->roots.data();
    r->merge = std::max<int64_t>(1, std::min<int64_t>(cfg->merge, cfg->n_batches));
    r->n_units = (cfg->n_batches + r->merge - 1) / r->merge;
    const int64_t mb = r->merge * cfg->batch;
    const int64_t bound = gs_sample_pack_bound_multi(cfg->graph, mb, cfg->batch, r->fanouts.data(), cfg->n_hops);
    GS_REQUIRE(bound > 0, GS_EINVAL, "pack bound failed");
    r->cap = bound + mb;
    hip_ok(hipGetDevice(&r->device), "hipGetDevice");
    {
        int lo = 0, hi = 0;
        hip_ok(hipDeviceGetStreamPriorityRange(&lo, &hi), "hipDeviceGetStreamPriorityRange");
        hip_ok(hipStreamCreateWithPriority(&r->side, hipStreamNonBlocking, hi), "hipStreamCreateWithPriority");
    }
    for (int d = 0; d < gs_runner::kDev; ++d) {
        hip_ok(hipEventCreateWithFlags(&r->dev_done[d], sync_event_flags()), "hipEventCreate");
        hip_ok(hipEventCreateWithFlags(&r->gathered[d], sync_event_flags()), "hipEventCreate");
    }
    hip_ok(hipMalloc(&r->clip_ws, 64 * 8 * sizeof(float)), "hipMalloc(clip ws)");
    r->use_flag = !cfg->embed_out;
    if (r->use_flag) {
        void* hp = nullptr;
        hip_ok(hipHostMalloc(&hp, 64, hipHostMallocCoherent | hipHostMallocMapped), "hipHostMalloc(done flag)");
        r->done_host = static_cast<int64_t*>(hp);
        *r->done_host = -1;
        void* dp = nullptr;
        hip_ok(hipHostGetDevicePointer(&dp, hp, 0), "hipHostGetDevicePointer");
        r->done_dev = static_cast<int64_t*>(dp);
    }
    {
        int64_t nn = 0, ne = 0, md = 0;
        GS_REQUIRE(gs_graph_dims(cfg->graph, &nn, &ne, &md) == GS_OK, GS_EINVAL, "gs_graph_dims");
        int64_t nd = cfg->batch;
        for (int32_t j = 0; j + 1 < cfg->n_hops; ++j) {
            const int64_t k = r->fanouts[j];
            const int64_t per = k > 0 ? std::min<int64_t>(k, md) : md;
            nd = std::min<int64_t>(nn, nd + nd * per);
        }
        const int32_t k_last = r->fanouts[cfg->n_hops - 1];
        const int rc = gs_trainer_gather_reserve(cfg->trainer, nd * r->merge, k_last > 0 ? k_last : 0);
        if (rc != GS_OK) fail(rc, gs_last_error());
        if (!cfg->embed_out && cfg->n_hops == 2 && !(cfg->flags & GS_SAMPLE_GCN) && r->fanouts[0] > 0)
            trainer_reserve_top(cfg->trainer, cfg->batch, r->fanouts[0]);
        int64_t hs[4 * GS_MAX_HOPS] = {};
        int64_t d = cfg->batch * r->merge;
        for (int32_t j = 0; j < cfg->n_hops; ++j) {
            const int64_t k = r->fanouts[j];
            const int64_t per = k > 0 ? std::min<int64_t>(k, md) : md;
            const int64_t np = d * per, ns = std::min<int64_t>(nn, d + np);
            hs[4 * j] = d;
            hs[4 * j + 1] = np;
            hs[4 * j + 2] = ns;
            hs[4 * j + 3] = np;
            d = ns;
        }
        const int64_t need = gs_trainer_ws_bytes(cfg->trainer, hs);
        GS_REQUIRE(need >= 0, GS_EINVAL, gs_last_error());
        r->ws_bytes = need + (1 << 20);
        hip_ok(hipMalloc(&r->ws, r->ws_bytes), "hipMalloc(ws)");
    }
    const int32_t S = cfg->n_streams;
    r->devmode = cfg->device_sampler != 0;
    r->fastmode = fast;
    if (r->devmode) {
        GS_REQUIRE(r->merge == 1, GS_EINVAL, "device_sampler: merge must be 1");
        GS_REQUIRE(!(cfg->flags & GS_SAMPLE_FULL), GS_EINVAL, "device_sampler: no GS_SAMPLE_FULL");
        std::vector<int32_t> r32(r->roots.size());
        for (size_t i = 0; i < r32.size(); ++i) {
            GS_REQUIRE(r->roots[i] >= 0 && r->roots[i] < (int64_t(1) << 31), GS_ERANGE, "root id out of range");
            r32[i] = static_cast<int32_t>(r->roots[i]);
        }
        hip_ok(hipMalloc(&r->roots_dev, r32.size() * sizeof(int32_t)), "hipMalloc(roots)");
        hip_ok(hipMemcpy(r->roots_dev, r32.data(), r32.size() * sizeof(int32_t), hipMemcpyHostToDevice), "hipMemcpy");
        r->dstreams.resize(S);
        for (int32_t w = 0; w < S; ++w) {
            gs_runner::DevStream& d = r->dstreams[w];
            hip_ok(hipStreamCreateWithFlags(&d.st, hipStreamNonBlocking), "hipStreamCreate(dsampler)");
            for (int q = 0; q < gs_runner::kDevDepthMax; ++q) {
                hip_ok(hipEventCreate(&d.t0[q]), "hipEventCreate");
                hip_ok(hipEventCreate(&d.t1[q]), "hipEventCreate");
            }
            int rc = gs_dsampler_create(cfg->graph, r->fanouts.data(), cfg->n_hops, cfg->batch,
                                        (cfg->flags & (GS_SAMPLE_GCN | GS_SAMPLE_FAIL_EMPTY)) |
                                            (fast ? GS_DSAMPLER_FAST : S > 1 ? GS_DSAMPLER_NO_AUX : 0),
                                        &d.ds);
            if (rc != GS_OK) fail(rc, gs_last_error());
            d.next = w;
            if (fast) {
                rc = gs_dsampler_set_seed(d.ds, cfg->sampler_seed);
                if (rc != GS_OK) fail(rc, gs_last_error());
                continue;
            }
            uint32_t mt[624];
            int64_t pos = 0;
            rc = gs_rng_get_state(cfg->rngs[w], mt, &pos);
            if (rc != GS_OK) fail(rc, gs_last_error());
            rc = gs_dsampler_set_rng(d.ds, mt, pos, d.st);
            if (rc != GS_OK) fail(rc, gs_last_error());
            d.next = w;
        }
        r->dcap = std::max<int64_t>(r->cap, gs_dsampler_pack_bound(r->dstreams[0].ds, cfg->batch));
        r->dev_depth = gs_runner::kDevDepthMax;
        r->n_dpack = r->dev_depth * S + 3;
        r->dpack.assign(r->n_dpack, nullptr);
        for (auto& p : r->dpack) hip_ok(hipMalloc(&p, r->dcap * sizeof(int32_t)), "hipMalloc(pack)");
        r->dres.resize(r->n_dpack);
    }
    const char* shared_env = std::getenv("GS_SHARED_HELPERS");
    const bool shared_helpers = shared_env && std::atoi(shared_env) == 1;
    if (!r->devmode) hip_ok(hipStreamCreateWithFlags(&r->copy_stream, hipStreamNonBlocking), "hipStreamCreate(copy)");
    for (int32_t w = 0; w < S && !r->devmode; ++w) {
        auto s = std::make_unique<SamplerStream>();
        s->rng = cfg->rngs[w];
        if (cfg->helpers > 0) {
            const int rc = shared_helpers && w > 0 ? gs_team_create_shared(r->streams[0]->team, &s->team)
                                                   : gs_team_create(shared_helpers ? cfg->helpers * S : cfg->helpers,
                                                                    &s->team);
            if (rc != GS_OK) fail(GS_EINVAL, gs_last_error());
        }
        for (int64_t b = w; b < r->n_units; b += S) s->batches.push_back(b);
        s->slots.resize(cfg->depth);
        for (int32_t q = 0; q < cfg->depth; ++q) {
            PackSlot& sl = s->slots[q];
            {
                constexpr size_t kHuge = size_t(2) << 20;
                const size_t bytes = (r->cap * sizeof(int32_t) + kHuge - 1) / kHuge * kHuge;
                void* p = mmap(nullptr, bytes + kHuge, PROT_READ | PROT_WRITE, MAP_PRIVATE | MAP_ANONYMOUS, -1, 0);
                if (p == MAP_FAILED) fail(GS_ENOMEM, "mmap(pack slot)");
                const uintptr_t a = (reinterpret_cast<uintptr_t>(p) + kHuge - 1) / kHuge * kHuge;
                const size_t head = a - reinterpret_cast<uintptr_t>(p);
                if (head) munmap(p, head);
                if (kHuge - head) munmap(reinterpret_cast<char*>(a) + bytes, kHuge - head);
                (void)madvise(reinterpret_cast<void*>(a), bytes, MADV_HUGEPAGE);
                std::memset(reinterpret_cast<void*>(a), 0, bytes);
                sl.host = reinterpret_cast<int32_t*>(a);
                sl.thp_bytes = bytes;
                hip_ok(hipHostRegister(sl.host, bytes, hipHostRegisterDefault), "hipHostRegister(pack slot)");
            }
            hip_ok(hipMalloc(&sl.dev, r->cap * sizeof(int32_t)), "hipMalloc(pack twin)");
            s->free.push_back(q);
        }
        r->streams.push_back(std::move(s));
    }
    r->release_mark = cfg->hold ? 0 : INT64_MAX;
    for (int32_t w = 0; w < S && r->devmode; ++w) r->dev_enqueue(w);
    if (cfg->comm && cfg->ar_buckets == 2 && !cfg->embed_out && cfg->n_hops >= 2) {
        hip_ok(hipStreamCreateWithFlags(&r->comm_stream, hipStreamNonBlocking), "hipStreamCreate(comm)");
        hip_ok(hipEventCreateWithFlags(&r->upper_ready, hipEventDisableTiming), "hipEventCreate");
        hip_ok(hipEventCreateWithFlags(&r->upper_reduced, hipEventDisableTiming), "hipEventCreate");
        gs_runner* rp = r.get();
        trainer_set_upper_hook(cfg->trainer, [rp](hipStream_t st) {
            const int64_t w1 = trainer_w1_floats(rp->cfg.trainer);
            const int64_t n = gs_trainer_n_params(rp->cfg.trainer);
            hip_ok(hipEventRecord(rp->upper_ready, st), "hipEventRecord");
            hip_ok(hipStreamWaitEvent(rp->comm_stream, rp->upper_ready, 0), "hipStreamWaitEvent");
            const int rc = gs_comm_allreduce_sum(rp->cfg.comm, gs_trainer_grads(rp->cfg.trainer) + w1, n - w1,
                                                 rp->comm_stream);
            if (rc != GS_OK) fail(rc, gs_last_error());
        });
        const char* ch_env = std::getenv("GS_AR_W1_CHUNKS");
        const int chunks = ch_env ? std::atoi(ch_env) : 2;
        if (chunks > 1) {
            hip_ok(hipEventCreateWithFlags(&r->w1_ready, hipEventDisableTiming), "hipEventCreate");
            trainer_set_w1_chunk_hook(cfg->trainer, chunks, [rp](hipStream_t st, int64_t off, int64_t n) {
                hip_ok(hipEventRecord(rp->w1_ready, st), "hipEventRecord");
                hip_ok(hipStreamWaitEvent(rp->comm_stream, rp->w1_ready, 0), "hipStreamWaitEvent");
                const int rc = gs_comm_allreduce_sum(rp->cfg.comm, gs_trainer_grads(rp->cfg.trainer) + off, n,
                                                     rp->comm_stream);
                if (rc != GS_OK) fail(rc, gs_last_error());
                ++rp->w1_issued;
            });
        }
    }
// ... 215 lines not shown
```

graphsage-pytorch_amd/train.py:

```python
import ctypes
import os
import queue
import threading
import time

import numpy as np
import torch
import torch.distributed as dist

from . import _lib
from . import hip_ops as ops
from ._lib import check, lib
from .models import Classification, DeviceSample, SageLayer
from .sampler import RNG, sample


def reference_init(num_layers, input_size, hidden, n_classes, gcn=False, seed=824):
    torch.manual_seed(seed)
    layers = [SageLayer(input_size if i == 1 else hidden, hidden, gcn=gcn) for i in range(1, num_layers + 1)]
    cls = Classification(hidden, n_classes)
    return [l.weight.detach().clone() for l in layers], cls.layer[0].weight.detach().clone(), \
        cls.layer[0].bias.detach().clone()


class FlatParams:

    def __init__(self, tensors, names, groups, device):
        sizes = [t.numel() for t in tensors]
        self.offsets = np.concatenate([[0], np.cumsum(sizes)]).astype(np.int64)
        self.params = torch.empty(int(self.offsets[-1]), dtype=torch.float32, device=device)
        self.grads = torch.zeros_like(self.params)
        self.names = names
        self.shapes = [tuple(t.shape) for t in tensors]
        for i, t in enumerate(tensors):
            self.view(i).copy_(t.to(device=device, dtype=torch.float32))
        self.group_off = np.array([self.offsets[g] for g in groups] + [self.offsets[-1]], np.int64)

    def view(self, i, grad=False):
        buf = self.grads if grad else self.params
        return buf[int(self.offsets[i]):int(self.offsets[i + 1])].view(self.shapes[i])

    def state_dict(self):
        return {n: self.view(i).detach().clone() for i, n in enumerate(self.names)}


_OPTIMIZERS = {"sgd": _lib.GS_OPT_SGD, "adam": _lib.GS_OPT_ADAM}


def optimizer_kind(name):
    try:
        return _OPTIMIZERS[name]
    except (KeyError, TypeError):
        raise ValueError(f"optimizer must be one of {sorted(_OPTIMIZERS)}, got {name!r}") from None


class NativeTrainer:

    def __init__(self, graph, features, labels, n_classes, num_layers=2, hidden=128, fanouts=(10, 10),
                 agg_func="MEAN", gcn=False, lr=0.7, max_norm=5.0, seed=824, weights=None, optimizer="sgd",
                 betas=(0.9, 0.999), eps=1e-8, weight_decay=0.0):
        self.optimizer = optimizer
        self._opt_kind = optimizer_kind(optimizer)
        self.betas, self.eps, self.weight_decay = (float(betas[0]), float(betas[1])), float(eps), float(weight_decay)
        if not features.is_cuda:
            raise RuntimeError("NativeTrainer runs on a HIP device")
        self.device = features.device
        self.graph, self.X = graph, features
        self.labels = labels.to(device=self.device, dtype=torch.int32)
        self.L, self.H, self.C = num_layers, hidden, n_classes
        self.fanouts = list(fanouts)
        self.agg, self.gcn, self.lr, self.max_norm = agg_func, gcn, lr, max_norm
        if weights is None:
            weights = reference_init(num_layers, features.shape[1], hidden, n_classes, gcn, seed)
        sage_w, cls_w, cls_b = weights
        names = [f"sage_layer{i}.weight" for i in range(1, num_layers + 1)] + ["layer.0.weight", "layer.0.bias"]
        self.p = FlatParams(list(sage_w) + [cls_w, cls_b], names, [0, num_layers], self.device)
        self.row_ptr, self.col = graph.device_csr(self.device)
        self.loss = torch.zeros(1, dtype=torch.float32, device=self.device)
        self.clip_ws = torch.empty(65 * 2, dtype=torch.float32, device=self.device)
        X = self.X
        cfg = _lib.TrainerConfig(
            n_layers=num_layers, hidden=hidden, n_classes=n_classes, agg=ops.agg_op(agg_func), gcn=int(gcn),
            feat_dtype=_lib.GS_BF16 if X.dtype == torch.bfloat16 else _lib.GS_F32,
            feat_dim=X.shape[1], feat_ld=X.stride(0), X=X.data_ptr(), row_ptr=self.row_ptr.data_ptr(),
            col=self.col.data_ptr(), labels=self.labels.data_ptr(), params=self.p.params.data_ptr(),
            grads=self.p.grads.data_ptr(), lr=lr, max_norm=max_norm)
        h = ctypes.c_void_p()
        check(lib().gs_trainer_create(ctypes.byref(cfg), ctypes.byref(h)))
        self._h = h
        if lib().gs_trainer_n_params(h) != self.p.params.numel():
            raise RuntimeError("flat parameter layout mismatch")
        self._ws = torch.empty(0, dtype=torch.uint8, device=self.device)
        self.opt_m = self.opt_v = None
        if self._opt_kind == _lib.GS_OPT_ADAM:
            self.opt_m = torch.zeros_like(self.p.params)
            self.opt_v = torch.zeros_like(self.p.params)
            self._set_optimizer(0)

    def _set_optimizer(self, step):
        oc = _lib.OptimizerConfig(kind=self._opt_kind, beta1=self.betas[0], beta2=self.betas[1], eps=self.eps,
                                  weight_decay=self.weight_decay, m=_lib.ptr(self.opt_m),
                                  v=_lib.ptr(self.opt_v), step=int(step))
        check(lib().gs_trainer_set_optimizer(self._h, ctypes.byref(oc)))

    def optimizer_state(self):
        return {"step": int(lib().gs_trainer_opt_step(self._h)),
                "m": None if self.opt_m is None else self.opt_m.detach().clone(),
                "v": None if self.opt_v is None else self.opt_v.detach().clone()}

    def load_optimizer_state(self, state):
        if self.opt_m is not None:
            if state["m"] is None or state["v"] is None:
                raise ValueError("load_optimizer_state: the state holds no Adam moments")
            if state["m"].numel() != self.opt_m.numel() or state["v"].numel() != self.opt_v.numel():
                raise ValueError("load_optimizer_state: moment size != parameter count")
            self.opt_m.copy_(state["m"].reshape(-1))
            self.opt_v.copy_(state["v"].reshape(-1))
        self._set_optimizer(state["step"])

    def load_state_dict(self, sd):
        for i, n in enumerate(self.p.names):
            self.p.view(i).copy_(sd[n])

    def state_dict(self):
        return self.p.state_dict()

    def weights(self):
        return [self.p.view(i) for i in range(self.L)]

    def forward_backward(self, ds, roots_dev):
        sizes, offs = ds.native_sizes()
        self._reserve_ws(sizes)
        check(lib().gs_trainer_forward_backward(
            self._h, ds.buf.data_ptr(), sizes.ctypes.data, offs.ctypes.data, roots_dev.data_ptr(),
            roots_dev.numel(), self._ws.data_ptr(), self._ws.numel(), self.loss.data_ptr(),
            _lib.stream_ptr(self.device)))
        return self.loss

    def _reserve_ws(self, sizes):
        need = int(lib().gs_trainer_ws_bytes(self._h, sizes.ctypes.data))
        if need < 0:
            check(_lib.GS_EINVAL)
        if self._ws.numel() < need:
            self._ws = torch.empty(int(need * 1.25) + (1 << 20), dtype=torch.uint8, device=self.device)

    def forward(self, ds, out):
        if not (out.is_contiguous() and out.dtype == torch.float32 and out.shape[1] == self.H):
            raise ValueError("out must be a contiguous fp32 [n_roots, hidden] tensor")
        sizes, offs = ds.native_sizes()
        if out.shape[0] != sizes[0]:
            raise ValueError("out rows != batch roots")
        self._reserve_ws(sizes)
        check(lib().gs_trainer_forward(self._h, ds.buf.data_ptr(), sizes.ctypes.data, offs.ctypes.data,
                                       self._ws.data_ptr(), self._ws.numel(), out.data_ptr(),
                                       _lib.stream_ptr(self.device)))
        return out

    _OPTIONS = {"fused_bwd": _lib.GS_TOPT_FUSED_BWD, "top_launch": _lib.GS_TOPT_TOP_LAUNCH,
                "self_rows": _lib.GS_TOPT_SELF_ROWS, "defer_update": _lib.GS_TOPT_DEFER_UPDATE}

    def set_option(self, name, value):
        check(lib().gs_trainer_set_option(self._h, self._OPTIONS[name], int(bool(value))))
        return self

    def capture(self, n_steps, batch):
        emb = torch.zeros(n_steps, batch, self.H, dtype=torch.float32, device=self.device)
        grads = torch.zeros(n_steps, self.p.params.numel(), dtype=torch.float32, device=self.device)
        self._cap = (emb, grads)
        check(lib().gs_trainer_capture(self._h, emb.data_ptr(), batch * self.H, grads.data_ptr(), n_steps))
        return emb, grads

    def captured(self):
        return int(lib().gs_trainer_captured(self._h))

    def update(self, grad_scale=1.0):
        check(lib().gs_trainer_update(self._h, float(grad_scale), self.clip_ws.data_ptr(),
                                      _lib.stream_ptr(self.device)))

    def defer(self, on):
        active = ctypes.c_int32(0)
        check(lib().gs_trainer_defer(self._h, int(bool(on)), ctypes.byref(active), _lib.stream_ptr(self.device)))
        return bool(active.value)

    def apply_update(self, world_size=1, group=None):
        if world_size > 1:
            dist.all_reduce(self.p.grads, group=group)
            check(lib().gs_trainer_update(self._h, 1.0 / world_size, self.clip_ws.data_ptr(),
                                          _lib.stream_ptr(self.device)))
        else:
            check(lib().gs_trainer_update_local(self._h, _lib.stream_ptr(self.device)))

    def __del__(self):
        h = getattr(self, "_h", None)
        if h is not None and h.value and getattr(_lib, "_lib", None) is not None:
            _lib._lib.gs_trainer_destroy(h)
            self._h = None

    def step(self, ds, roots_dev, world_size=1, group=None):
        loss = self.forward_backward(ds, roots_dev)
        self.apply_update(world_size, group)
        return loss


def rank_batches(candidates, batch_size, rank, world_size, seed, epoch=0):
    perm = np.random.RandomState(seed + epoch).permutation(np.asarray(candidates, np.int64))
    n_steps = len(perm) // (batch_size * world_size)
    for i in range(n_steps):
        b = i * world_size + rank
        yield perm[b * batch_size:(b + 1) * batch_size]


def rank_seed(seed, rank, stream=0):
    return seed + rank + 64 * stream


class SampleInfo:

    def __init__(self, n_hops, sizes, offsets, used, n_roots):
        self.n_hops = n_hops
        self._sizes = [tuple(int(x) for x in sizes[4 * j:4 * j + 4]) for j in range(n_hops)]
        self.offsets = offsets.reshape(_lib.GS_MAX_HOPS, _lib.GS_PK_NFIELDS)[:n_hops].tolist()
        self.pack_total = int(used) - n_roots
        self.n_roots = n_roots

    def sizes(self, j):
        return self._sizes[j - 1]


class _SamplerWorker:

    def __init__(self, graph, rng, batches, fanouts, flags, depth):
        self.graph, self.rng, self.batches, self.flags = graph, rng, batches, flags
        self.fan = np.array([(-1 if k is None else int(k)) for k in fanouts], np.int32)
        self.q = queue.Queue(maxsize=depth)
        self.slots = [None] * (depth + 1)
        self.events = [None] * (depth + 1)
        self.free = queue.Queue()
        for i in range(depth + 1):
            self.free.put(i)
        self.sample_s = []
        self.stop = False
        self.t = threading.Thread(target=self._run, daemon=True)
        self.t.start()

    def _run(self):
        L = len(self.fan)
        try:
            for roots in self.batches:
                if self.stop:
                    break
                roots = np.ascontiguousarray(roots, dtype=np.int64)
                bound = int(lib().gs_sample_pack_bound(self.graph.handle, len(roots), self.fan.ctypes.data, L))
                slot = self.free.get()
                ev = self.events[slot]
                if ev is not None:
                    ev.synchronize()
                buf = self.slots[slot]
                if buf is None or buf.numel() < bound:
                    buf = self.slots[slot] = torch.empty(bound, dtype=torch.int32, pin_memory=True)
                sizes = np.empty(4 * L, np.int64)
                offs = np.empty(_lib.GS_MAX_HOPS * _lib.GS_PK_NFIELDS, np.int64)
                used = ctypes.c_int64()
                t0 = time.perf_counter()
                check(lib().gs_sample_pack_run(self.graph.handle, self.rng._h, roots.ctypes.data, len(roots),
                                               self.fan.ctypes.data, L, self.flags, buf.data_ptr(), buf.numel(),
                                               sizes.ctypes.data, offs.ctypes.data, ctypes.byref(used)))
                self.sample_s.append(time.perf_counter() - t0)
                self.q.put((slot, SampleInfo(L, sizes, offs, used.value, len(roots)), offs, sizes))
        except BaseException as e:
            self.q.put(e)
        self.q.put(None)


class Prefetcher:

    def __init__(self, graph, rng, batches, fanouts, gcn, device, depth=3, rngs=None, fail_empty=False):
        self.device = torch.device(device)
        rngs = list(rngs) if rngs is not None else [rng]
        S = len(rngs)
        batches = list(batches)
        flags = (_lib.GS_SAMPLE_GCN if gcn else 0) | (4 if fail_empty else 0)
        self.workers = [_SamplerWorker(graph, rngs[w], batches[w::S], fanouts, flags, depth) for w in range(S)]
        self.i = 0

    @property
    def sample_s(self):
        return [t for w in self.workers for t in w.sample_s]

    def next(self):
        w = self.workers[self.i % len(self.workers)]
        item = w.q.get()
        if item is None:
            raise StopIteration
        if isinstance(item, BaseException):
            raise item
        self.i += 1
        slot, info, offs, sizes = item
        used = info.pack_total + info.n_roots
        dev = w.slots[slot][:used].to(self.device, non_blocking=True)
        ev = torch.cuda.Event()
        ev.record()
        w.events[slot] = ev
        w.free.put(slot)
        ds = DeviceSample(info, self.device, buf=dev)
        ds._native = (sizes, offs)
        return ds, dev[info.pack_total:used], info

    def __iter__(self):
        return self

    def __next__(self):
        return self.next()

    def close(self):
        for w in self.workers:
            w.stop = True


def init_distributed():
    world = int(os.environ.get("WORLD_SIZE", "1"))
    rank = int(os.environ.get("RANK", "0"))
    if world > 1 and not dist.is_initialized():
        backend = "nccl" if torch.cuda.is_available() else "gloo"
        if backend == "nccl":
            torch.cuda.set_device(int(os.environ.get("LOCAL_RANK", "0")))
        dist.init_process_group(backend=backend)
    return rank, world


def make_rng(seed, rank=0, stream=0):
    return RNG(rank_seed(seed, rank, stream))


class Communicator:

    def __init__(self, rank, world, device):
        self.world = world
        uid = torch.zeros(128, dtype=torch.uint8)
        if rank == 0:
            check(lib().gs_comm_unique_id(uid.numpy().ctypes.data))
        if world > 1:
            t = uid.to(device)
            dist.broadcast(t, 0)
            uid = t.cpu().contiguous()
        h = ctypes.c_void_p()
        check(lib().gs_comm_create(uid.numpy().ctypes.data, world, rank, ctypes.byref(h)))
        self._h = h

    def close(self):
        if self._h is not None and self._h.value:
            lib().gs_comm_destroy(self._h)
        self._h = None


class Runner:

    def __init__(self, trainer, graph, batches, rngs, fanouts, gcn=False, fail_empty=False, depth=4,
                 comm=None, embed_out=None, merge=1, hold=False, ar_buckets=1, helpers=0, warm=False,
                 sampler="host", seed=0):
        if sampler not in ("host", "device", "device-fast"):
            raise ValueError("sampler must be 'host', 'device' or 'device-fast'")
        self.sampler = sampler
        self.trainer, self.graph = trainer, graph
        self.embed_out = embed_out
        fast = sampler == "device-fast"
        if fast:
            n_streams = int(rngs) if isinstance(rngs, int) else len(list(rngs))
            rngs = []
        self.rngs = list(rngs)
        self.batches = np.ascontiguousarray(np.stack([np.asarray(b, np.int64) for b in batches]))
        self.fanouts = np.ascontiguousarray(fanouts, dtype=np.int32)
        self._rng_ptrs = (ctypes.c_void_p * len(self.rngs))(*[r._h.value for r in self.rngs])
        self.comm = comm
        flags = (_lib.GS_SAMPLE_GCN if gcn else 0) | (4 if fail_empty else 0)
        cfg = _lib.RunnerConfig(
            graph=graph._h.value, trainer=trainer._h.value, batches=self.batches.ctypes.data,
            n_batches=self.batches.shape[0], batch=self.batches.shape[1], fanouts=self.fanouts.ctypes.data,
            n_hops=len(self.fanouts), flags=flags, n_streams=n_streams if fast else len(self.rngs),
            rngs=None if fast else ctypes.cast(self._rng_ptrs, ctypes.c_void_p), depth=depth,
            comm=comm._h.value if comm is not None else None, world=comm.world if comm is not None else 1,
            hold=int(bool(hold)), ar_buckets=int(ar_buckets), helpers=int(helpers), warm=int(bool(warm)),
            device_sampler=2 if fast else int(sampler == "device"), sampler_seed=int(seed) & (2 ** 64 - 1))
        if embed_out is not None:
            n_rows = self.batches.shape[0] * self.batches.shape[1]
            if not (embed_out.is_contiguous() and embed_out.dtype == torch.float32
                    and embed_out.device == trainer.device and embed_out.dim() == 2
                    and embed_out.shape[0] >= n_rows and embed_out.shape[1] == trainer.H):
                raise ValueError("embed_out must be a contiguous fp32 [n_batches * batch, hidden] device tensor")
            cfg.embed_out = embed_out.data_ptr()
            cfg.embed_ld = trainer.H
            cfg.merge = max(1, int(merge))
        elif merge > 1:
            raise ValueError("merge > 1 needs embed_out (forward-only)")
        self.merge = max(1, int(merge)) if embed_out is not None else 1
        h = ctypes.c_void_p()
        check(lib().gs_runner_create(ctypes.byref(cfg), ctypes.byref(h)))
        self._h = h

    def run(self, n_steps):
        check(lib().gs_runner_run(self._h, int(n_steps), self.trainer.loss.data_ptr(),
                                  _lib.stream_ptr(self.trainer.device)))
        return self.embed_out if self.embed_out is not None else self.trainer.loss

    def sync_rngs(self):
        check(lib().gs_runner_sync_rngs(self._h))

    def release(self, mark):
        check(lib().gs_runner_release(self._h, int(mark)))

    def progress(self):
        a, b = ctypes.c_int64(), ctypes.c_int64()
        check(lib().gs_runner_progress(self._h, ctypes.byref(a), ctypes.byref(b)))
        return a.value, b.value

    def stats(self, reset=False):
        st = _lib.RunnerStats()
        check(lib().gs_runner_stats_get(self._h, ctypes.byref(st)))
        if reset:
            lib().gs_runner_stats_reset(self._h)
        sizes = np.array(st.hop_sizes[:], dtype=np.float64).reshape(_lib.GS_MAX_HOPS, 4)
        return {"steps": st.steps, "wait_s": st.wait_s, "issue_s": st.issue_s, "sample_s": st.sample_s,
                "wait_sample_s": st.wait_sample_s, "wait_ring_s": st.wait_ring_s,
                "wait_gather_s": st.wait_gather_s, "fwd_bwd_s": st.fwd_bwd_s, "update_s": st.update_s,
                "max_step_s": st.max_step_s, "lookahead_misses": st.lookahead_misses, "hop_sizes_sum": sizes}

    def close(self):
        h = getattr(self, "_h", None)
        if h is not None and h.value and getattr(_lib, "_lib", None) is not None:
            _lib._lib.gs_runner_destroy(h)
        self._h = None

    def __del__(self):
        self.close()


class Embedder:

    def __init__(self, graph, features, weights, fanouts, agg_func="MEAN", gcn=False, depth=4, merge=2, helpers=0,
                 sampler="host", seed=0):
        if sampler not in ("host", "device-fast"):
            raise ValueError("Embedder: sampler must be 'host' or 'device-fast'")
        self.sampler, self.seed = sampler, int(seed)
        weights = [w.detach() for w in weights]
        H = weights[0].shape[0]
        dev = features.device
        dummy_cls = (torch.zeros(1, H, device=dev), torch.zeros(1, device=dev))
        self.trainer = NativeTrainer(graph, features, torch.zeros(1, dtype=torch.int32), 1,
                                     num_layers=len(weights), hidden=H, fanouts=fanouts, agg_func=agg_func,
                                     gcn=gcn, weights=(weights, *dummy_cls))
        self.graph, self.fanouts, self.gcn, self.agg = graph, list(fanouts), gcn, agg_func
        self.depth = depth
        self.merge = max(1, int(merge))
        self.helpers = int(helpers)
        self.last_stats = None

    def embed(self, nodes, batch, rngs):
        nodes = np.ascontiguousarray(nodes, dtype=np.int64).reshape(-1)
        rngs = [None] * rngs if isinstance(rngs, int) else list(rngs)
        n_full = len(nodes) // batch
        out = torch.empty(len(nodes), self.trainer.H, dtype=torch.float32, device=self.trainer.device)
        fast = self.sampler == "device-fast"
        merge = 1 if fast else self.merge
# ... 386 lines not shown
```

include/graphsage_amd.h:

```cpp
#ifndef GRAPHSAGE_AMD_H
#define GRAPHSAGE_AMD_H

#include <stddef.h>
#include <stdint.h>

#ifdef __cplusplus
extern "C" {
#endif

#define GS_OK 0
#define GS_EINVAL 1
#define GS_ENOMEM 2
#define GS_EHIP 3
#define GS_ERANGE 4
#define GS_EEMPTY 5
#define GS_ELIMIT 6

const char* gs_last_error(void);
const char* gs_version(void);

typedef struct gs_rng gs_rng;

int gs_rng_create(gs_rng** out);
void gs_rng_destroy(gs_rng* rng);
int gs_rng_seed_words(gs_rng* rng, const uint32_t* key, int64_t key_len);
int gs_rng_set_state(gs_rng* rng, const uint32_t* mt624, int64_t pos);
int gs_rng_get_state(const gs_rng* rng, uint32_t* mt624, int64_t* pos);
int gs_rng_getrandbits(gs_rng* rng, int32_t k, int64_t count, uint32_t* out);
int gs_rng_randbelow(gs_rng* rng, uint32_t n, int64_t count, uint32_t* out);
int gs_rng_sample_positions(gs_rng* rng, int64_t n, int64_t k, int64_t* out);
int gs_rng_choice_position(gs_rng* rng, int64_t n, int64_t* out);

int gs_pyset_union_of_lists(const int64_t* items, const int64_t* ptr,
                            int64_t n_lists, int64_t* out, int64_t* out_len);

typedef struct gs_graph gs_graph;

int gs_graph_build(const int64_t* src, const int64_t* dst, int64_t n_pairs,
                   int64_t n_nodes, int32_t n_threads, gs_graph** out);
int gs_graph_from_tables(int64_t n_nodes, const int64_t* row_ptr,
                         const int32_t* col, const uint32_t* slot,
                         const uint8_t* log2size, const uint8_t* dirty,
                         gs_graph** out);
void gs_graph_destroy(gs_graph* g);
int gs_graph_dims(const gs_graph* g, int64_t* n_nodes, int64_t* n_entries,
                  int64_t* max_degree);
const int64_t* gs_graph_row_ptr(const gs_graph* g);
const int32_t* gs_graph_col(const gs_graph* g);
int64_t gs_graph_image_bytes(const gs_graph* g);
int gs_graph_write_image(const gs_graph* g, void* dst, int64_t cap);
int gs_graph_from_image(const void* img, int64_t bytes, gs_graph** out);

int gs_rmat_pairs(int32_t scale, int64_t n_pairs, double a, double b, double c,
                  uint64_t seed, int32_t permute, int32_t n_threads,
                  int64_t* src, int64_t* dst, int64_t* n_kept);

#define GS_SAMPLE_GCN 1
#define GS_SAMPLE_FULL 2
#define GS_MAX_HOPS 8

typedef struct gs_sample gs_sample;

typedef struct {
    int64_t n_dst;
    int64_t n_pos;
    int64_t n_src;
    int64_t n_nbr;
    const int64_t* dst_ids;
    const int32_t* pos_ptr;
    const int32_t* pos;
    const int64_t* src_ids;
    const int32_t* nbr_ptr;
    const int32_t* nbr;
    const int32_t* self_local;
    const int32_t* set_ptr;
    const int64_t* set_items;
    int64_t n_empty;
} gs_hop_view;

enum {
    GS_PK_POS_PTR = 0,
    GS_PK_POS,
    GS_PK_DST_IDS,
    GS_PK_NBR_PTR,
    GS_PK_NBR,
    GS_PK_SELF,
    GS_PK_TPTR,
    GS_PK_TIDX,
    GS_PK_NFIELDS
};

typedef struct {
    int64_t total;
    int64_t off[GS_MAX_HOPS][GS_PK_NFIELDS];
} gs_pack_layout;

int gs_sample_run(const gs_graph* g, gs_rng* rng, const int64_t* roots,
                  int64_t n_roots, const int32_t* fanouts, int32_t n_hops,
                  int32_t flags, gs_sample** out);
void gs_sample_destroy(gs_sample* s);
int gs_sample_n_hops(const gs_sample* s, int32_t* n_hops);
int gs_sample_hop(const gs_sample* s, int32_t hop, gs_hop_view* out);
int gs_sample_pack_layout(const gs_sample* s, gs_pack_layout* out);
int gs_sample_pack(const gs_sample* s, int32_t* buf, int64_t cap);

#define GS_SAMPLE_FAIL_EMPTY 4
int64_t gs_sample_pack_bound(const gs_graph* g, int64_t n_roots,
                             const int32_t* fanouts, int32_t n_hops);
int gs_sample_pack_run(const gs_graph* g, gs_rng* rng, const int64_t* roots,
                       int64_t n_roots, const int32_t* fanouts, int32_t n_hops,
                       int32_t flags, int32_t* buf, int64_t cap,
                       int64_t* hop_sizes, int64_t* offsets, int64_t* used);
int64_t gs_sample_pack_bound_multi(const gs_graph* g, int64_t n_roots, int64_t group,
                                   const int32_t* fanouts, int32_t n_hops);
int gs_sample_pack_run_multi(const gs_graph* g, gs_rng* rng, const int64_t* roots,
                             int64_t n_roots, int64_t group, const int32_t* fanouts,
                             int32_t n_hops, int32_t flags, int32_t* buf, int64_t cap,
                             int64_t* hop_sizes, int64_t* offsets, int64_t* used);
int gs_fsample_pack_run(const gs_graph* g, uint64_t seed, int64_t batch_index,
                        const int64_t* roots, int64_t n_roots, const int32_t* fanouts,
                        int32_t n_hops, int32_t flags, int32_t* buf, int64_t cap,
                        int64_t* hop_sizes, int64_t* offsets, int64_t* used);
int gs_philox4x32(const uint32_t* ctr, const uint32_t* key, uint32_t* out);

typedef struct gs_team gs_team;
int gs_team_create(int32_t helpers, gs_team** out);
int gs_team_create_shared(const gs_team* peer, gs_team** out);
void gs_team_destroy(gs_team* team);
int gs_sample_pack_run_multi_team(const gs_graph* g, gs_rng* rng, const int64_t* roots,
                                  int64_t n_roots, int64_t group, const int32_t* fanouts,
                                  int32_t n_hops, int32_t flags, int32_t* buf, int64_t cap,
                                  int64_t* hop_sizes, int64_t* offsets, int64_t* used,
                                  gs_team* team);

typedef struct gs_dsampler gs_dsampler;
#define GS_DSAMPLER_NO_AUX 8
#define GS_DSAMPLER_FAST 16
int gs_dsampler_create(const gs_graph* g, const int32_t* fanouts, int32_t n_hops,
                       int64_t max_roots, int32_t flags, gs_dsampler** out);
void gs_dsampler_destroy(gs_dsampler* ds);
int gs_dsampler_set_rng(gs_dsampler* ds, const uint32_t* mt624, int64_t pos, void* stream);
int gs_dsampler_get_rng(gs_dsampler* ds, uint32_t* mt624, int64_t* pos, void* stream);
int gs_dsampler_words(gs_dsampler* ds, int64_t n, uint32_t* out, void* stream);
int64_t gs_dsampler_pack_bound(const gs_dsampler* ds, int64_t n_roots);
int gs_dsampler_run(gs_dsampler* ds, const int32_t* roots, int64_t n_roots, int32_t* pack,
                    int64_t cap, void* stream);
int gs_dsampler_result(gs_dsampler* ds, int64_t* hop_sizes, int64_t* offsets, int64_t* used);
int gs_dsampler_set_seed(gs_dsampler* ds, uint64_t seed);
int gs_dsampler_run_at(gs_dsampler* ds, int64_t batch_index, const int32_t* roots, int64_t n_roots,
                       int32_t* pack, int64_t cap, void* stream);
int64_t gs_dsampler_runs(const gs_dsampler* ds);
int gs_dsampler_result_of(gs_dsampler* ds, int64_t run, int64_t* hop_sizes, int64_t* offsets, int64_t* used);
int gs_dsampler_debug(gs_dsampler* ds, int64_t* out, int32_t n);

typedef struct gs_unsup gs_unsup;

int gs_unsup_create(const gs_graph* g, const int64_t* train_nodes, int64_t n_train,
                    int32_t n_walks, int32_t walk_len, int32_t n_walk_len,
                    gs_unsup** out);
void gs_unsup_destroy(gs_unsup* u);
int gs_unsup_attach_device(gs_unsup* u, void* stream);
int gs_unsup_extend(gs_unsup* u, gs_rng* rng, const int64_t* nodes, int64_t n,
                    int64_t num_neg, int32_t parts, int32_t n_threads,
                    int64_t* sizes);
int gs_unsup_fetch(const gs_unsup* u, int64_t* unique, int64_t* pos_pairs,
                   int64_t* neg_pairs, int64_t* pos_cnt, int64_t* neg_cnt,
                   uint8_t* has_pos);
int gs_unsup_loss_plan(const gs_unsup* u, int32_t* buf, int64_t cap,
                       int64_t* dims, int64_t* used);

typedef enum { GS_F32 = 0, GS_BF16 = 1 } gs_dtype;
typedef enum { GS_AGG_MEAN = 0, GS_AGG_MAX = 1 } gs_agg;

int gs_fill_uniform(void* X, gs_dtype dt, int64_t N, int64_t F, int64_t ld,
                    uint64_t seed, void* stream);
int gs_uniform_host(uint64_t seed, int64_t row0, int64_t F, int64_t n_rows,
                    float* out);

int gs_agg_fwd(gs_agg op, gs_dtype xdt, const void* X, int64_t ldx, int64_t F,
               int64_t n_dst, const int32_t* ptr, const int32_t* idx,
               const int64_t* row_ptr, const int32_t* col,
               const int32_t* dst_ids, int32_t gcn,
               void* out, gs_dtype odt, int64_t ldo, int32_t* argmax,
               void* stream);

int gs_sage_linear_fwd(gs_dtype dt, int64_t n, int64_t F, int64_t H,
                       const void* Xs, int64_t ldxs, const int32_t* sidx,
                       const void* A, int64_t lda, const void* Wd,
                       float* out, int64_t ldo, int32_t relu, void* stream);

int64_t gs_sage_linear_bwd_weight_ws(int64_t n, int64_t K, int64_t H);
int gs_sage_linear_bwd_weight(gs_dtype dt, int64_t n, int64_t F, int64_t H,
                              const void* Xs, int64_t ldxs, const int32_t* sidx,
                              const void* A, int64_t lda,
                              const float* dout, const float* out, int64_t ldo,
                              int32_t relu, float* dW, void* ws, int64_t ws_bytes,
                              void* stream);
int gs_sage_linear_bwd_input(int64_t n, int64_t F, int64_t H,
                             const float* dout, const float* out, int64_t ldo,
                             int32_t relu, const float* W,
                             float* dSelf, float* dA, int64_t ldd, void* stream);

int gs_agg_bwd(gs_agg op, int64_t n_src, int64_t F, const int32_t* tptr,
               const int32_t* tidx, const int32_t* ptr,
               const float* dA, const float* dSelf, int64_t ldd,
               const int32_t* argmax, const float* Hprev, int64_t ldh,
               float* dH, void* stream);

int gs_sage1_fwd_supported(gs_dtype dt, int64_t F, int64_t H, int32_t gcn);
int gs_sage1_fwd(gs_agg op, gs_dtype dt, const void* X, int64_t ldx, int64_t F,
                 int64_t H, int64_t n_dst, const int32_t* ptr, const int32_t* ent,
                 const int32_t* col, const int32_t* dst_ids, int32_t gcn,
                 const void* W, void* agg_out, int64_t ld_agg, float* out,
                 int64_t ldo, int32_t relu, void* stream);

int64_t gs_cls_nll_ws_floats(int64_t B, int64_t D, int64_t C);
int gs_cls_nll_fwd_bwd(int64_t B, int64_t D, int64_t C, const float* E,
                       const float* Wc, const float* bc, const int32_t* labels,
                       const int32_t* roots, int32_t mask_relu, float* loss,
                       float* dE, float* dWc, float* dbc, float* ws,
                       void* stream);

int64_t gs_unsup_loss_ws_floats(int64_t M, int64_t P, int64_t N);
int gs_unsup_loss_fwd(int32_t kind, int64_t M, int64_t P, int64_t N, int64_t U,
                      int64_t D, const float* emb, int64_t lde, const int32_t* plan,
                      float q, float margin, float* loss, float* ws, void* stream);
int gs_unsup_loss_bwd(int64_t M, int64_t P, int64_t N, int64_t U, int64_t D,
                      const float* emb, int64_t lde, const int32_t* plan,
                      const float* ws, const float* dloss, float* dE, int64_t ldd,
                      void* stream);

int gs_clip_sgd(int32_t n_groups, const int64_t* goff_host, float* params,
                float* grads, float grad_scale, float max_norm, float lr,
                float* ws, void* stream);

int gs_clip_adam(int32_t n_groups, const int64_t* goff_host, float* params,
                 float* grads, float* m, float* v, float grad_scale, float max_norm,
                 float lr, float beta1, float beta2, float eps, float weight_decay,
                 int64_t step, float* ws, void* stream);

int gs_cast_f32_bf16(const float* in, void* out, int64_t n, void* stream);

typedef struct {
    int32_t n_layers, hidden, n_classes;
    int32_t agg;
    int32_t gcn;
    int32_t feat_dtype;
    int64_t feat_dim, feat_ld;
    const void* X;
    const int64_t* row_ptr;
    const int32_t* col;
    const int32_t* labels;
    float* params;
    float* grads;
    float lr, max_norm;
} gs_trainer_config;

typedef struct gs_trainer gs_trainer;
int gs_trainer_create(const gs_trainer_config* cfg, gs_trainer** out);
void gs_trainer_destroy(gs_trainer* t);
int64_t gs_trainer_n_params(const gs_trainer* t);
int64_t gs_trainer_ws_bytes(gs_trainer* t, const int64_t* hop_sizes);
int gs_trainer_forward_backward(gs_trainer* t, const int32_t* pack,
                                const int64_t* hop_sizes, const int64_t* offsets,
                                const int32_t* roots, int64_t n_roots, void* ws,
                                int64_t ws_bytes, float* loss, void* stream);
int gs_trainer_gather_reserve(gs_trainer* t, int64_t max_rows, int32_t max_fanout);
int gs_trainer_gather(gs_trainer* t, const int32_t* pack, const int64_t* hop_sizes,
                      const int64_t* offsets, int32_t slot, void* stream);
int gs_trainer_forward_backward_gathered(gs_trainer* t, const int32_t* pack,
                                         const int64_t* hop_sizes, const int64_t* offsets,
                                         const int32_t* roots, int64_t n_roots, int32_t slot,
                                         void* ws, int64_t ws_bytes, float* loss, void* stream);
int gs_trainer_forward(gs_trainer* t, const int32_t* pack, const int64_t* hop_sizes,
                       const int64_t* offsets, void* ws, int64_t ws_bytes, float* out,
                       void* stream);
int gs_trainer_forward_gathered(gs_trainer* t, const int32_t* pack, const int64_t* hop_sizes,
                                const int64_t* offsets, int32_t slot, void* ws,
                                int64_t ws_bytes, float* out, void* stream);
int gs_trainer_update(gs_trainer* t, float grad_scale, float* ws, void* stream);
int gs_trainer_update_local(gs_trainer* t, void* stream);
int gs_trainer_time_agg(gs_trainer* t, int64_t capacity);
int64_t gs_trainer_agg_times(gs_trainer* t, float* ms, int64_t cap);
int gs_trainer_time_kernels(gs_trainer* t, int32_t site_mask, int64_t capacity);
int gs_trainer_time_kernels_every(gs_trainer* t, int32_t site_mask, int64_t capacity, int64_t every);
int64_t gs_trainer_kernel_times(gs_trainer* t, int32_t site, float* ms, int64_t cap);
int64_t gs_trainer_kernel_block_stats(gs_trainer* t, int32_t site, float* us4, int64_t cap);
int64_t gs_trainer_kernel_stamps(gs_trainer* t, int32_t site, int64_t launch, uint64_t* start, uint64_t* end);
const char* gs_trainer_kernel_name(const gs_trainer* t, int32_t site);
float* gs_trainer_grads(const gs_trainer* t);
int gs_trainer_capture(gs_trainer* t, float* emb, int64_t emb_stride, float* grads, int64_t max_steps);
int64_t gs_trainer_captured(const gs_trainer* t);
int gs_trainer_defer(gs_trainer* t, int32_t on, int32_t* active, void* stream);
enum { GS_TOPT_FUSED_BWD = 0, GS_TOPT_TOP_LAUNCH = 1, GS_TOPT_SELF_ROWS = 2, GS_TOPT_DEFER_UPDATE = 3 };
int gs_trainer_set_option(gs_trainer* t, int32_t opt, int32_t value);
enum { GS_OPT_SGD = 0, GS_OPT_ADAM = 1 };
typedef struct {
    int32_t kind;
    float beta1, beta2, eps, weight_decay;
    float* m;
    float* v;
    int64_t step;
} gs_optimizer_config;
int gs_trainer_set_optimizer(gs_trainer* t, const gs_optimizer_config* oc);
int64_t gs_trainer_opt_step(const gs_trainer* t);

int gs_comm_unique_id(uint8_t id[128]);
int gs_comm_create(const uint8_t id[128], int32_t n_ranks, int32_t rank, void** comm);
void gs_comm_destroy(void* comm);
int gs_comm_allreduce_sum(void* comm, float* buf, int64_t n, void* stream);

typedef struct {
    const gs_graph* graph;
    gs_trainer* trainer;
    const int64_t* batches;
    int64_t n_batches, batch;
    const int32_t* fanouts;
    int32_t n_hops;
    int32_t flags;
    int32_t n_streams;
    gs_rng* const* rngs;
    int32_t depth;
    void* comm;
    int32_t world;
    float* embed_out;
    int64_t embed_ld;
    int32_t merge;
    int32_t hold;
    int32_t ar_buckets;
    int32_t helpers;
    int32_t warm;
    int32_t device_sampler;
    uint64_t sampler_seed;
} gs_runner_config;

typedef struct {
    int64_t steps;
    double wait_s;
    double issue_s;
    double sample_s;
    double hop_sizes[4 * GS_MAX_HOPS];
    double wait_sample_s;
    double wait_ring_s;
    double wait_gather_s;
    double fwd_bwd_s, update_s;
    double max_step_s;
    int64_t lookahead_misses;
} gs_runner_stats;

typedef struct gs_runner gs_runner;
int gs_runner_create(const gs_runner_config* cfg, gs_runner** out);
int gs_runner_run(gs_runner* r, int64_t n_steps, float* loss, void* stream);
int gs_runner_stats_get(const gs_runner* r, gs_runner_stats* out);
void gs_runner_stats_reset(gs_runner* r);
int gs_runner_release(gs_runner* r, int64_t mark);
int gs_runner_progress(const gs_runner* r, int64_t* sampled, int64_t* consumed);
int gs_runner_sync_rngs(gs_runner* r);
void gs_runner_destroy(gs_runner* r);

typedef struct gs_full_plan gs_full_plan;
int gs_full_plan_create(const int64_t* row_ptr, const int32_t* col, int64_t n_nodes,
                        int32_t gcn, int64_t seg_len, gs_full_plan** out);
void gs_full_plan_destroy(gs_full_plan* plan);
enum { GS_FP_N_NODES = 0, GS_FP_N_ITEMS, GS_FP_N_SLOTS, GS_FP_N_SPLIT, GS_FP_N_EMPTY,
       GS_FP_SEG_LEN, GS_FP_GCN, GS_FP_N_ENTRIES, GS_FP_NDIMS };
int gs_full_plan_dims(const gs_full_plan* plan, int64_t* dims);
enum { GS_FP_ITEMS = 0, GS_FP_ITEM_PTR, GS_FP_SLOT_PTR, GS_FP_SPLIT_PTR, GS_FP_SPLIT_ROWS,
       GS_FP_COUNT, GS_FP_SELF_LOOP, GS_FP_EMPTY_ROWS };
const void* gs_full_plan_array(const gs_full_plan* plan, int32_t which);

typedef struct {
    const int32_t* items;
    const int64_t* slot_ptr;
    const int32_t* split_rows;
    const int32_t* count;
    const uint8_t* self_loop;
} gs_full_plan_dev;

int64_t gs_agg_full_ws_bytes(const gs_full_plan* plan, int64_t F, int64_t row0, int64_t n_rows);
int gs_agg_full(const gs_full_plan* plan, const gs_full_plan_dev* dev, gs_agg op, gs_dtype dt,
                const void* X, int64_t ldx, int64_t F, const int64_t* row_ptr, const int32_t* col,
                int64_t row0, int64_t n_rows, void* out, int64_t ldo,
                void* ws, int64_t ws_bytes, void* stream);

typedef struct {
    int32_t n_layers, hidden;
    int32_t agg;
    int32_t feat_dtype;
    int64_t feat_dim, feat_ld;
    const void* X;
    const int64_t* row_ptr;
    const int32_t* col;
    const float* W[GS_MAX_HOPS];
    int64_t chunk_rows;
} gs_infer_full_config;
int64_t gs_infer_full_ws_bytes(const gs_full_plan* plan, const gs_infer_full_config* cfg);
int gs_infer_full(const gs_full_plan* plan, const gs_full_plan_dev* dev, const gs_infer_full_config* cfg,
                  float* out, int64_t ldo, void* ws, int64_t ws_bytes, void* stream);

enum { GS_FP_T_ROW_PTR = 8, GS_FP_T_COL = 9 };
int gs_full_plan_transpose(const gs_full_plan* plan, const int64_t* row_ptr, const int32_t* col,
                           int64_t seg_len, gs_full_plan** out);

int64_t gs_agg_full_argmax_ws_bytes(const gs_full_plan* plan, int64_t F, int64_t row0, int64_t n_rows);
int gs_agg_full_argmax(const gs_full_plan* plan, const gs_full_plan_dev* dev, gs_dtype dt,
                       const void* X, int64_t ldx, int64_t F, const int64_t* row_ptr, const int32_t* col,
                       int64_t row0, int64_t n_rows, void* out, int64_t ldo, int32_t* argmax, int64_t lda,
                       void* ws, int64_t ws_bytes, void* stream);

int64_t gs_agg_full_bwd_ws_bytes(const gs_full_plan* tplan, int64_t F);
int gs_agg_full_bwd(const gs_full_plan* tplan, const gs_full_plan_dev* tdev, gs_agg op, int64_t F,
                    const int64_t* t_row_ptr, const int32_t* t_col, const float* dA, const float* dSelf,
                    int64_t ldd, const int32_t* argmax, int64_t lda, const float* Hprev, float* dH,
                    int64_t ldh, void* ws, int64_t ws_bytes, void* stream);

typedef struct {
    int32_t n_layers, hidden, n_classes;
    int32_t agg;
    int32_t feat_dtype;
    int32_t pad_;
    int64_t feat_dim, feat_ld;
    int64_t max_nodes;
    const void* X;
    const int64_t* row_ptr;
    const int32_t* col;
    const int64_t* t_row_ptr;
    const int32_t* t_col;
    const int32_t* labels;
    const float* params;
    float* grads;
} gs_train_full_config;
enum { GS_TF_FORWARD = 1, GS_TF_HEAD = 2, GS_TF_BACKWARD = 4, GS_TF_ALL = 7 };
int64_t gs_train_full_ws_offset(const gs_full_plan* plan, const gs_full_plan* tplan,
                                const gs_train_full_config* cfg, int32_t which, int32_t layer);
int64_t gs_train_full_ws_bytes(const gs_full_plan* plan, const gs_full_plan* tplan,
                               const gs_train_full_config* cfg);
int gs_train_full_forward_backward(const gs_full_plan* plan, const gs_full_plan_dev* dev,
                                   const gs_full_plan* tplan, const gs_full_plan_dev* tdev,
                                   const gs_train_full_config* cfg, const int32_t* nodes, int64_t n_nodes,
                                   int32_t reuse_agg1, int32_t stages, float* loss,
                                   void* ws, int64_t ws_bytes, void* stream);

enum { GS_FF_LAYER0 = GS_MAX_HOPS + 1, GS_FF_NCOUNTS = GS_MAX_HOPS + 1 + 4 * GS_MAX_HOPS };
enum { GS_FF_ROWS = 0, GS_FF_POS, GS_FF_ITEMS, GS_FF_SPLIT, GS_FF_T_ITEMS, GS_FF_T_SPLIT };
typedef struct {
    int32_t n_layers, pad_;
    void* buf;
    int64_t buf_bytes;
    int64_t counts[GS_FF_NCOUNTS];
} gs_full_field;
int64_t gs_full_field_bytes(const gs_full_plan* plan, const gs_full_plan* tplan, int32_t n_layers);
int64_t gs_full_field_offset(const gs_full_plan* plan, const gs_full_plan* tplan, int32_t n_layers,
                             int32_t which, int32_t level);
int gs_full_field_build(const gs_full_plan* plan, const gs_full_plan_dev* dev,
                        const gs_full_plan* tplan, const gs_full_plan_dev* tdev,
                        const int64_t* row_ptr, const int32_t* col,
                        const int32_t* nodes, int64_t n_nodes, int32_t rebuild,
                        gs_full_field* f, void* stream);
int gs_full_field_counts(const gs_full_plan* plan, const gs_full_plan* tplan, gs_full_field* f, void* stream);

int gs_agg_full_field(const gs_full_plan* plan, const gs_full_plan_dev* dev, const gs_full_plan* tplan,
                      const gs_full_field* f, int32_t layer, gs_agg op, gs_dtype dt,
                      const void* X, int64_t ldx, int64_t F, const int64_t* row_ptr, const int32_t* col,
                      void* out, int64_t ldo, int32_t* argmax, int64_t lda,
                      void* ws, int64_t ws_bytes, void* stream);
int gs_agg_full_bwd_field(const gs_full_plan* plan, const gs_full_plan* tplan, const gs_full_plan_dev* tdev,
                          const gs_full_field* f, int32_t layer, gs_agg op, int64_t F,
                          const int64_t* t_row_ptr, const int32_t* t_col, const float* dA,
                          const float* dSelf, int64_t ldd, const int32_t* argmax, int64_t lda,
                          const float* Hprev, int64_t ldh, float* dH, int64_t ldo,
                          void* ws, int64_t ws_bytes, void* stream);

int gs_train_full_field_forward_backward(const gs_full_plan* plan, const gs_full_plan_dev* dev,
                                         const gs_full_plan* tplan, const gs_full_plan_dev* tdev,
                                         const gs_train_full_config* cfg, const gs_full_field* f,
                                         const int32_t* nodes, int64_t n_nodes,
                                         int32_t reuse_agg1, int32_t stages, float* loss,
                                         void* ws, int64_t ws_bytes, void* stream);

typedef struct {
    int32_t kind;
    int32_t with_sup;
    int64_t M, P, N;
    const int32_t* plan;
    float q, margin;
} gs_train_full_unsup;
int64_t gs_train_full_unsup_ws_bytes(int32_t hidden, int64_t n_nodes, int64_t M, int64_t P, int64_t N);
int gs_train_full_unsup_forward_backward(const gs_full_plan* plan, const gs_full_plan_dev* dev,
                                         const gs_full_plan* tplan, const gs_full_plan_dev* tdev,
                                         const gs_train_full_config* cfg, const gs_full_field* f,
                                         const int32_t* nodes, int64_t n_nodes,
                                         const gs_train_full_unsup* u, void* uws, int64_t uws_bytes,
                                         int32_t reuse_agg1, int32_t stages, float* loss,
                                         void* ws, int64_t ws_bytes, void* stream);

#ifdef __cplusplus
}
#endif
#endif
```

Before: 10.37 million.

## Fold next batch's id resolve and top records into current gather kernel

Adds a gather-ahead path in which the feature-gather kernel launches extra blocks that resolve the next batch's neighbor ids and top/record words, tagged per slot, so the next step can skip its own resolve launch. The runner peeks at whether the next sampled batch is ready and passes it into a new gs_trainer_gather_ahead entry point. This aims to remove a separate small kernel launch per batch and overlap it with the gather. The cost is added bookkeeping: slot tags, try-lock peeks and validity checks. The feature sits behind a gather_ahead option that defaults to false.

```diff
diff --git a/graphsage-pytorch_amd/_lib.py b/graphsage-pytorch_amd/_lib.py
--- a/graphsage-pytorch_amd/_lib.py
+++ b/graphsage-pytorch_amd/_lib.py
@@ -16,6 +16,7 @@
 GS_SAMPLE_FAIL_EMPTY = 4
 GS_MAX_HOPS = 8
 GS_TOPT_FUSED_BWD, GS_TOPT_TOP_LAUNCH, GS_TOPT_SELF_ROWS, GS_TOPT_DEFER_UPDATE = range(4)
+GS_TOPT_GATHER_AHEAD = 5
 GS_OPT_SGD, GS_OPT_ADAM = 0, 1
 (GS_PK_POS_PTR, GS_PK_POS, GS_PK_DST_IDS, GS_PK_NBR_PTR, GS_PK_NBR, GS_PK_SELF,
  GS_PK_TPTR, GS_PK_TIDX, GS_PK_NFIELDS) = range(9)
@@ -124,6 +125,9 @@
     "gs_trainer_defer": (_i32, [_vp, _i32, _p(_i32), _vp]),
     "gs_trainer_gather_reserve": (_i32, [_vp, _i64, _i32]),
     "gs_trainer_gather": (_i32, [_vp, _vp, _vp, _vp, _i32, _vp]),
+    "gs_trainer_gather_ahead": (_i32, [_vp, _vp, _vp, _vp, _i32, _i64, _vp, _vp, _vp, _i32, _i64, _vp]),
+    "gs_trainer_gather_slot_info": (_i32, [_vp, _i32, _vp]),
+    "gs_trainer_gather_slot_copy": (_i32, [_vp, _i32, _i32, _vp, _i64, _i32, _vp]),
     "gs_trainer_forward_backward_gathered": (_i32, [_vp, _vp, _vp, _vp, _vp, _i64, _i32, _vp, _i64, _vp, _vp]),
     "gs_trainer_forward": (_i32, [_vp, _vp, _vp, _vp, _vp, _i64, _vp, _vp]),
     "gs_trainer_forward_gathered": (_i32, [_vp, _vp, _vp, _vp, _i32, _vp, _i64, _vp, _vp]),
diff --git a/graphsage-pytorch_amd/csrc/kernels/agg.hip b/graphsage-pytorch_amd/csrc/kernels/agg.hip
--- a/graphsage-pytorch_amd/csrc/kernels/agg.hip
+++ b/graphsage-pytorch_amd/csrc/kernels/agg.hip
@@ -6,12 +6,9 @@
 
 namespace gs {
 
-__global__ __launch_bounds__(kBlock) void resolve_ids_kernel(int n_dst, int k, const int* __restrict__ ptr,
-                                                             const int* __restrict__ ent,
-                                                             const int* __restrict__ col,
-                                                             const int* __restrict__ dst_ids, int gcn,
-                                                             int* __restrict__ ids) {
-    const int64_t t = blockIdx.x * int64_t(kBlock) + threadIdx.x;
+__device__ __forceinline__ void resolve_ids_slot(int64_t t, int n_dst, int k, const int* __restrict__ ptr,
+                                                 const int* __restrict__ ent, const int* __restrict__ col,
+                                                 const int* __restrict__ dst_ids, int gcn, int* __restrict__ ids) {
     if (t >= static_cast<int64_t>(n_dst) * k) return;
     const int r = static_cast<int>(t / k), j = static_cast<int>(t - static_cast<int64_t>(r) * k);
     const int e = ptr[r] + j;
@@ -19,6 +16,38 @@
     if (e < ptr[r + 1]) nb = col[ent[e]];
     if (!gcn && nb == dst_ids[r]) nb = -1;
     ids[t] = nb;
+}
+
+__global__ __launch_bounds__(kBlock) void resolve_ids_kernel(int n_dst, int k, const int* __restrict__ ptr,
+                                                             const int* __restrict__ ent,
+                                                             const int* __restrict__ col,
+                                                             const int* __restrict__ dst_ids, int gcn,
+                                                             int* __restrict__ ids) {
+    resolve_ids_slot(blockIdx.x * int64_t(kBlock) + threadIdx.x, n_dst, k, ptr, ent, col, dst_ids, gcn, ids);
+}
+
+__device__ __forceinline__ void top_recs_word(int64_t u, int n_top, int tk, const int* __restrict__ tptr,
+                                              const int* __restrict__ tnbr, const int* __restrict__ tself,
+                                              int* __restrict__ tout, int n_rec, const int* __restrict__ rptr,
+                                              const int* __restrict__ ridx, int* __restrict__ rout) {
+    const int64_t n2 = static_cast<int64_t>(n_top) * (tk + 1);
+    if (u >= n2) {
+        const int64_t q = u - n2;
+        if (q >= static_cast<int64_t>(n_rec) * 8) return;
+        const int c = static_cast<int>(q >> 3), j = static_cast<int>(q & 7);
+        const int b = rptr[c], n = rptr[c + 1] - b;
+        rout[q] = j == 0 ? n : j == 1 ? b : (j - 2 < n ? ridx[b + j - 2] : 0);
+        return;
+    }
+    const int r = static_cast<int>(u / (tk + 1)), j = static_cast<int>(u - static_cast<int64_t>(r) * (tk + 1));
+    int v;
+    if (j == 0) {
+        v = tself[r];
+    } else {
+        const int e = tptr[r] + j - 1;
+        v = e < tptr[r + 1] ? tnbr[e] : -1;
+    }
+    tout[u] = v;
 }
 
 __global__ __launch_bounds__(kBlock) void resolve_top_kernel(int n_dst, int k, const int* __restrict__ ptr,
@@ -34,33 +63,10 @@
     const int64_t t = blockIdx.x * int64_t(kBlock) + threadIdx.x;
     const int64_t n1 = static_cast<int64_t>(n_dst) * k;
     if (t < n1) {
-        const int r = static_cast<int>(t / k), j = static_cast<int>(t - static_cast<int64_t>(r) * k);
-        const int e = ptr[r] + j;
-        int nb = -1;
-        if (e < ptr[r + 1]) nb = col[ent[e]];
-        if (!gcn && nb == dst_ids[r]) nb = -1;
-        ids[t] = nb;
+        resolve_ids_slot(t, n_dst, k, ptr, ent, col, dst_ids, gcn, ids);
         return;
     }
-    const int64_t u = t - n1;
-    const int64_t n2 = static_cast<int64_t>(n_top) * (tk + 1);
-    if (u >= n2) {
-        const int64_t q = u - n2;
-        if (q >= static_cast<int64_t>(n_rec) * 8) return;
-        const int c = static_cast<int>(q >> 3), j = static_cast<int>(q & 7);
-        const int b = rptr[c], n = rptr[c + 1] - b;
-        rout[q] = j == 0 ? n : j == 1 ? b : (j - 2 < n ? ridx[b + j - 2] : 0);
-        return;
-    }
-    const int r = static_cast<int>(u / (tk + 1)), j = static_cast<int>(u - static_cast<int64_t>(r) * (tk + 1));
-    int v;
-    if (j == 0) {
-        v = tself[r];
-    } else {
-        const int e = tptr[r] + j - 1;
-        v = e < tptr[r + 1] ? tnbr[e] : -1;
-    }
-    tout[u] = v;
+    top_recs_word(t - n1, n_top, tk, tptr, tnbr, tself, tout, n_rec, rptr, ridx, rout);
 }
 
 template <typename T, int VEC>
@@ -90,11 +96,38 @@
     }
 };
 
-template <int OP, typename T, int VEC, int G, bool SELF, bool ONE, int NR1 = kRows>
+struct AheadRoles {
+    int gather_blocks, rec_blocks;
+    int n_top, tk;
+    const int *tptr, *tnbr, *tself;
+    int* tout;
+    int n_rec;
+    const int *rptr, *ridx;
+    int* rout;
+    int n_dst, k, gcn;
+    const int *ptr, *ent, *col, *dst_ids;
+    int* ids;
+};
+__device__ __forceinline__ bool gather_block() { return true; }
+__device__ __forceinline__ bool gather_block(const AheadRoles& a) {
+    if (static_cast<int>(blockIdx.x) < a.gather_blocks) return true;
+    const int64_t t = (static_cast<int>(blockIdx.x) - a.gather_blocks) * int64_t(kBlock) + threadIdx.x;
+    const int64_t nr = a.rec_blocks * int64_t(kBlock);
+    if (t < nr) top_recs_word(t, a.n_top, a.tk, a.tptr, a.tnbr, a.tself, a.tout, a.n_rec, a.rptr, a.ridx, a.rout);
+    else resolve_ids_slot(t - nr, a.n_dst, a.k, a.ptr, a.ent, a.col, a.dst_ids, a.gcn, a.ids);
+    return false;
+}
+__device__ __forceinline__ unsigned gather_blocks() { return gridDim.x; }
+__device__ __forceinline__ unsigned gather_blocks(const AheadRoles& a) { return a.gather_blocks; }
+
+template <int OP, typename T, int VEC, int G, bool SELF, bool ONE, int NR1 = kRows, typename... Roles>
 __global__ __launch_bounds__(kBlock) void agg_ids_kernel(const T* __restrict__ X, int64_t ldx, int F, int n_dst, int k,
                                                          const int* __restrict__ ids, const int* __restrict__ dst_ids,
                                                          int gcn, T* __restrict__ out, int64_t ldo,
-                                                         T* __restrict__ self_out, int64_t ldso) {
+                                                         T* __restrict__ self_out, int64_t ldso, Roles... roles) {
+    static_assert(sizeof...(Roles) <= 1, "at most one AheadRoles");
+    if constexpr (sizeof...(Roles) > 0)
+        if (!gather_block(roles...)) return;
     const int gl = threadIdx.x % G;
     if constexpr (ONE) {
         using Raw = typename RawVec<T, VEC>::type;
@@ -154,7 +187,7 @@
         RowIO<T, VEC>::store(out + static_cast<int64_t>(r) * ldo + f0, acc);
         return;
     }
-    for (int r = blockIdx.x * (kBlock / G) + threadIdx.x / G; r < n_dst; r += gridDim.x * (kBlock / G)) {
+    for (int r = blockIdx.x * (kBlock / G) + threadIdx.x / G; r < n_dst; r += gather_blocks(roles...) * (kBlock / G)) {
     const int node = (gcn || SELF) ? dst_ids[r] : 0;
     const int* rid = ids + static_cast<int64_t>(r) * k;
     constexpr int NR = kRows;
@@ -259,27 +292,72 @@
 
 void agg_ids_launch(gs_agg op, gs_dtype dt, const void* X, int64_t ldx, int64_t F, int64_t n_dst, int k,
                     const int32_t* ids, const int32_t* dst_ids, int gcn, void* out, int64_t ldo, hipStream_t st,
-                    void* self_out, int64_t ldso, LaunchTimer* timer) {
+                    void* self_out, int64_t ldso, LaunchTimer* timer, const GatherAhead* ahead) {
     GS_REQUIRE(op == GS_AGG_MEAN || op == GS_AGG_MAX, GS_EINVAL, "agg_func must be MEAN or MAX");
     GS_REQUIRE(F >= 1 && n_dst >= 0 && k >= 1 && ldx >= F && ldo >= F, GS_EINVAL, "bad sizes");
     GS_REQUIRE(!self_out || (dst_ids && ldso >= F), GS_EINVAL, "self rows need dst_ids and ldso >= F");
+    GS_REQUIRE(!ahead || n_dst > 0, GS_EINVAL, "roles behind the gather need a gather");
     if (n_dst == 0) return;
     const int V = dt == GS_F32 ? 4 : 8;
     const bool vec = F % V == 0 && ldx % V == 0 && ldo % V == 0 && aligned16(X) && aligned16(out) &&
                      (!self_out || (ldso % V == 0 && aligned16(self_out)));
     const int f = static_cast<int>(F), n = static_cast<int>(n_dst);
     static const int cap = agg_ids_block_cap();
+    AheadRoles roles{};
+    int64_t extra = 0;
+    if (ahead) {
+        const GatherAhead& g = *ahead;
+        GS_REQUIRE(g.n_top >= 0 && g.n_rec >= 0 && (g.n_top + g.n_rec == 0 || g.tk >= 1) &&
+                       g.n_top * (g.tk + 1) < (int64_t(1) << 30) && g.n_rec < (int64_t(1) << 27) &&
+                       (g.n_top == 0 || (g.tptr && g.tnbr && g.tself && g.tout)) &&
+                       (g.n_rec == 0 || (g.rptr && g.ridx && g.rout)),
+                   GS_EINVAL, "bad record sizes");
+        GS_REQUIRE(g.n_dst >= 0 && (g.n_dst == 0 || (g.k >= 1 && g.n_dst * g.k < (int64_t(1) << 31) && g.ptr &&
+                                                     g.ent && g.col && g.dst_ids && g.ids)),
+                   GS_EINVAL, "bad sizes of the next batch's resolve");
+        GS_REQUIRE(g.n_dst == 0 || g.ids != ids, GS_EINVAL, "the next batch's ids would overwrite this gather's");
+        const int64_t rec_words = g.n_top * (g.tk + 1) + g.n_rec * 8;
+        roles.rec_blocks = static_cast<int>((rec_words + kBlock - 1) / kBlock);
+        roles.n_top = static_cast<int>(g.n_top);
+        roles.tk = std::max(g.tk, 1);
+        roles.tptr = g.tptr;
+        roles.tnbr = g.tnbr;
+        roles.tself = g.tself;
+        roles.tout = g.tout;
+        roles.n_rec = static_cast<int>(g.n_rec);
+        roles.rptr = g.rptr;
+        roles.ridx = g.ridx;
+        roles.rout = g.rout;
+        roles.n_dst = static_cast<int>(g.n_dst);
+        roles.k = std::max(g.k, 1);
+        roles.gcn = g.gcn;
+        roles.ptr = g.ptr;
+        roles.ent = g.ent;
+        roles.col = g.col;
+        roles.dst_ids = g.dst_ids;
+        roles.ids = g.ids;
+        extra = roles.rec_blocks + (g.n_dst * roles.k + kBlock - 1) / kBlock;
+    }
+#define GS_IDS3(OPV, TT, VV, GG, SELFV, ONE, NRV, SO)                                                            \
+    do {                                                                                                         \
+        if (ahead) {                                                                                             \
+            roles.gather_blocks = static_cast<int>(grid_.x);                                                     \
+            GS_REQUIRE(grid_.x + extra < (int64_t(1) << 31), GS_EINVAL, "grid too large");                       \
+            launch_k(timer, agg_ids_kernel<OPV, TT, VV, GG, SELFV, ONE, NRV, AheadRoles>,                        \
+                     dim3(static_cast<unsigned>(grid_.x + extra)), dim3(kBlock), 0, st,                          \
+                     static_cast<const TT*>(X), ldx, f, n, k, ids, dst_ids, gcn, static_cast<TT*>(out), ldo,      \
+                     static_cast<TT*>(SO), ldso, roles);                                                         \
+        } else {                                                                                                 \
+            launch_k(timer, agg_ids_kernel<OPV, TT, VV, GG, SELFV, ONE, NRV>, grid_, dim3(kBlock), 0, st,        \
+                     static_cast<const TT*>(X), ldx, f, n, k, ids, dst_ids, gcn, static_cast<TT*>(out), ldo,      \
+                     static_cast<TT*>(SO), ldso);                                                                \
+        }                                                                                                        \
+    } while (0)
 #define GS_IDS2(OPV, TT, VV, GG, ONE, NRV)                                                                       \
     do {                                                                                                         \
         const dim3 grid_(std::min((n + (kBlock / GG) - 1) / (kBlock / GG), cap));                                \
-        if (self_out)                                                                                            \
-            launch_k(timer, agg_ids_kernel<OPV, TT, VV, GG, true, ONE, NRV>, grid_, dim3(kBlock), 0, st,         \
-                     static_cast<const TT*>(X), ldx, f, n, k, ids, dst_ids, gcn, static_cast<TT*>(out), ldo,      \
-                     static_cast<TT*>(self_out), ldso);                                                          \
-        else                                                                                                     \
-            launch_k(timer, agg_ids_kernel<OPV, TT, VV, GG, false, ONE, NRV>, grid_, dim3(kBlock), 0, st,        \
-                     static_cast<const TT*>(X), ldx, f, n, k, ids, dst_ids, gcn, static_cast<TT*>(out), ldo,      \
-                     static_cast<TT*>(nullptr), ldso);                                                           \
+        if (self_out) GS_IDS3(OPV, TT, VV, GG, true, ONE, NRV, self_out);                                        \
+        else GS_IDS3(OPV, TT, VV, GG, false, ONE, NRV, nullptr);                                                 \
     } while (0)
 #define GS_IDS1(OPV, TT, VV, GG, ONE)                                                                            \
     do {                                                                                                         \
@@ -318,6 +396,7 @@
 #undef GS_IDS
 #undef GS_IDS1
 #undef GS_IDS2
+#undef GS_IDS3
     check_launch("agg_ids");
 }
 
diff --git a/graphsage-pytorch_amd/csrc/kernels/internal.hpp b/graphsage-pytorch_amd/csrc/kernels/internal.hpp
--- a/graphsage-pytorch_amd/csrc/kernels/internal.hpp
+++ b/graphsage-pytorch_amd/csrc/kernels/internal.hpp
@@ -50,9 +50,23 @@
                         const int32_t* tnbr, const int32_t* tself, int32_t* tout, hipStream_t st, int64_t n_rec = 0,
                         const int32_t* rptr = nullptr, const int32_t* ridx = nullptr, int32_t* rout = nullptr);
 void trainer_reserve_top(gs_trainer* t, int64_t B, int32_t tk);
+struct GatherAhead {
+    int64_t n_top = 0;
+    int tk = 1;
+    const int32_t *tptr = nullptr, *tnbr = nullptr, *tself = nullptr;
+    int32_t* tout = nullptr;
+    int64_t n_rec = 0;
+    const int32_t *rptr = nullptr, *ridx = nullptr;
+    int32_t* rout = nullptr;
+    int64_t n_dst = 0;
+    int k = 1, gcn = 0;
+    const int32_t *ptr = nullptr, *ent = nullptr, *col = nullptr, *dst_ids = nullptr;
+    int32_t* ids = nullptr;
+};
 void agg_ids_launch(gs_agg op, gs_dtype dt, const void* X, int64_t ldx, int64_t F, int64_t n_dst, int k,
                     const int32_t* ids, const int32_t* dst_ids, int gcn, void* out, int64_t ldo, hipStream_t st,
-                    void* self_out = nullptr, int64_t ldso = 0, LaunchTimer* timer = nullptr);
+                    void* self_out = nullptr, int64_t ldso = 0, LaunchTimer* timer = nullptr,
+                    const GatherAhead* ahead = nullptr);
 void agg_fwd_launch(gs_agg op, gs_dtype xdt, const void* X, int64_t ldx, int64_t F, int64_t n_dst,
                     const int32_t* ptr, const int32_t* idx, const int64_t* row_ptr, const int32_t* col,
                     const int32_t* dst_ids, int32_t gcn, void* out, gs_dtype odt, int64_t ldo, int32_t* argmax,
diff --git a/graphsage-pytorch_amd/csrc/kernels/step.hip b/graphsage-pytorch_amd/csrc/kernels/step.hip
--- a/graphsage-pytorch_amd/csrc/kernels/step.hip
+++ b/graphsage-pytorch_amd/csrc/kernels/step.hip
@@ -27,41 +27,97 @@
     timed_done(T, 0, timed);
 }
 
+struct NextBatch {
+    const int32_t* pack = nullptr;
+    const int64_t *hop_sizes = nullptr, *offsets = nullptr;
+    int slot = -1;
+    int64_t tag = -1;
+};
+
 static void gather1_ids(gs_trainer& T, const int32_t* pack, const int64_t* hop_sizes, const int64_t* offsets,
-                        int slot, hipStream_t st) {
+                        int slot, hipStream_t st, int64_t tag = -1, const NextBatch& next = {}) {
     const gs_trainer_config& c = T.cfg;
     const int L = c.n_layers;
     auto fld = [&](int f) { return pack_field(pack, offsets, L, f); };
     const int64_t n_dst = hop_sizes[4 * (L - 1)];
     int32_t* ids = T.ids_slot[slot];
+    const gs_trainer::IdsTag was = T.ids_tag[slot];
+    T.ids_tag[slot] = {};
+    const bool have = T.gather_ahead && tag >= 0 && was.tag == tag && was.pack == pack && was.n_dst == n_dst &&
+                      was.stream == st && n_dst > 0;
     const int64_t n_top = hop_sizes[0];
     T.top_ready[slot] = T.top_k > 0 && L == 2 && !c.gcn && n_top <= T.top_rows && T.top_slot[slot] &&
                         hop_sizes[3] <= n_top * T.top_k;
     const int64_t n_rec = hop_sizes[2];
     T.rec_ready[slot] = T.top_ready[slot] && T.rec_slot[slot] && n_rec <= T.rec_rows;
-    if (T.top_ready[slot]) {
+    GatherAhead ga;
+    bool fused = false;
+    if (have) {
+        if (T.top_ready[slot]) {
+            auto f1 = [&](int f) { return pack_field(pack, offsets, 1, f); };
+            ga.n_top = n_top;
+            ga.tk = T.top_k;
+            ga.tptr = f1(GS_PK_NBR_PTR);
+            ga.tnbr = f1(GS_PK_NBR);
+            ga.tself = f1(GS_PK_SELF);
+            ga.tout = T.top_slot[slot];
+            if (T.rec_ready[slot]) {
+                ga.n_rec = n_rec;
+                ga.rptr = f1(GS_PK_TPTR);
+                ga.ridx = f1(GS_PK_TIDX);
+                ga.rout = T.rec_slot[slot];
+            }
+            fused = true;
+        }
+    } else if (T.top_ready[slot]) {
         auto f1 = [&](int f) { return pack_field(pack, offsets, 1, f); };
         resolve_top_launch(n_dst, T.k_ids, fld(GS_PK_POS_PTR), fld(GS_PK_POS), c.col, fld(GS_PK_DST_IDS), c.gcn, ids,
                            n_top, T.top_k, f1(GS_PK_NBR_PTR), f1(GS_PK_NBR), f1(GS_PK_SELF), T.top_slot[slot], st,
                            T.rec_ready[slot] ? n_rec : 0, f1(GS_PK_TPTR), f1(GS_PK_TIDX), T.rec_slot[slot]);
+        ++T.n_resolve;
     } else {
         resolve_ids_launch(n_dst, T.k_ids, fld(GS_PK_POS_PTR), fld(GS_PK_POS), c.col, fld(GS_PK_DST_IDS), c.gcn, ids,
                            st);
-    }
+        ++T.n_resolve;
+    }
+    bool tag_next = false;
+    if (T.gather_ahead && n_dst > 0 && next.pack && next.tag >= 0 && next.slot >= 0 && next.slot != slot) {
+        const int64_t m_dst = next.hop_sizes[4 * (L - 1)], m_pos = next.hop_sizes[4 * (L - 1) + 1];
+        if (m_dst > 0 && m_dst <= T.a1_rows && m_pos <= m_dst * T.k_ids && T.ids_slot[next.slot]) {
+            auto fn = [&](int f) { return pack_field(next.pack, next.offsets, L, f); };
+            ga.n_dst = m_dst;
+            ga.k = T.k_ids;
+            ga.gcn = c.gcn;
+            ga.ptr = fn(GS_PK_POS_PTR);
+            ga.ent = fn(GS_PK_POS);
+            ga.col = c.col;
+            ga.dst_ids = fn(GS_PK_DST_IDS);
+            ga.ids = T.ids_slot[next.slot];
+            fused = tag_next = true;
+        }
+    }
+    const GatherAhead* gap = fused ? &ga : nullptr;
     LaunchTimer timed = timed_arm(T, 0);
     if (T.self_rows) {
         char* base = static_cast<char*>(T.a1_slot[slot]);
         const int64_t xsz = c.feat_dtype == GS_BF16 ? 2 : 4;
         agg_ids_launch(static_cast<gs_agg>(c.agg), static_cast<gs_dtype>(c.feat_dtype), c.X, c.feat_ld, c.feat_dim,
                        n_dst, T.k_ids, ids, fld(GS_PK_DST_IDS), c.gcn, base + c.feat_dim * xsz, 2 * c.feat_dim, st,
-                       base, 2 * c.feat_dim, &timed);
+                       base, 2 * c.feat_dim, &timed, gap);
         T.self_in_slot[slot] = true;
     } else {
         agg_ids_launch(static_cast<gs_agg>(c.agg), static_cast<gs_dtype>(c.feat_dtype), c.X, c.feat_ld, c.feat_dim,
                        n_dst, T.k_ids, ids, fld(GS_PK_DST_IDS), c.gcn, T.a1_slot[slot], c.feat_dim, st, nullptr, 0,
-                       &timed);
+                       &timed, gap);
     }
     timed_done(T, 0, timed);
+    if (fused) ++T.n_ahead;
+    if (tag_next) {
+        T.ids_tag[next.slot].tag = next.tag;
+        T.ids_tag[next.slot].n_dst = ga.n_dst;
+        T.ids_tag[next.slot].pack = next.pack;
+        T.ids_tag[next.slot].stream = st;
+    }
 }
 
 struct StepPlan {
@@ -542,6 +598,10 @@
         case GS_TOPT_TOP_LAUNCH: t->use_top = on; break;
         case GS_TOPT_SELF_ROWS: t->want_self_rows = on; break;
         case GS_TOPT_DEFER_UPDATE: t->opt_defer = on; break;
+        case GS_TOPT_GATHER_AHEAD:
+            t->gather_ahead = on;
+            t->clear_ids_tags();
+            break;
         default: GS_REQUIRE(false, GS_EINVAL, "unknown trainer option");
     }
     GS_API_END
@@ -586,6 +646,7 @@
     GS_API_BEGIN
     GS_REQUIRE(t && max_rows >= 0 && max_fanout >= 0, GS_EINVAL, "bad arguments");
     const bool self_rows = t->want_self_rows && !t->cfg.gcn && t->cfg.n_layers >= 1;
+    t->clear_ids_tags();
     if (max_rows <= t->a1_rows && max_fanout <= t->k_ids && self_rows == t->self_rows) return GS_OK;
     max_rows = std::max(max_rows, t->a1_rows);
     t->self_rows = self_rows;
@@ -612,25 +673,79 @@
     GS_API_END
 }
 
-int gs_trainer_gather(gs_trainer* t, const int32_t* pack, const int64_t* hop_sizes, const int64_t* offsets,
-                      int32_t slot, void* stream) {
+int gs_trainer_gather_ahead(gs_trainer* t, const int32_t* pack, const int64_t* hop_sizes, const int64_t* offsets,
+                            int32_t slot, int64_t tag, const int32_t* next_pack, const int64_t* next_hop_sizes,
+                            const int64_t* next_offsets, int32_t next_slot, int64_t next_tag, void* stream) {
     GS_API_BEGIN
     GS_REQUIRE(t && pack && hop_sizes && offsets && slot >= 0 && slot < gs_trainer::kSlots, GS_EINVAL,
                "bad arguments");
     const int L = t->cfg.n_layers;
     GS_REQUIRE(hop_sizes[4 * (L - 1)] <= t->a1_rows && t->a1_slot[slot], GS_EINVAL,
                "gather slot too small (gs_trainer_gather_reserve)");
+    gs::NextBatch next;
+    if (next_pack && next_hop_sizes && next_offsets && next_tag >= 0) {
+        GS_REQUIRE(next_slot >= 0 && next_slot < gs_trainer::kSlots && next_slot != slot, GS_EINVAL,
+                   "the next batch needs a gather slot of its own");
+        next = {next_pack, next_hop_sizes, next_offsets, next_slot, next_tag};
+    }
     const int64_t n_dst = hop_sizes[4 * (L - 1)], n_pos = hop_sizes[4 * (L - 1) + 1];
     if (t->k_ids > 0 && n_pos <= n_dst * t->k_ids) {
-        gs::gather1_ids(*t, pack, hop_sizes, offsets, slot, gs::as_stream(stream));
+        gs::gather1_ids(*t, pack, hop_sizes, offsets, slot, gs::as_stream(stream), tag, next);
     } else if (t->self_rows) {
         const int64_t F = t->cfg.feat_dim, xsz = t->cfg.feat_dtype == GS_BF16 ? 2 : 4;
+        t->ids_tag[slot] = {};
         gs::gather1(*t, pack, hop_sizes, offsets, static_cast<char*>(t->a1_slot[slot]) + F * xsz,
                     gs::as_stream(stream), 2 * F);
         t->self_in_slot[slot] = false;
     } else {
+        t->ids_tag[slot] = {};
         gs::gather1(*t, pack, hop_sizes, offsets, t->a1_slot[slot], gs::as_stream(stream));
     }
+    GS_API_END
+}
+
+int gs_trainer_gather(gs_trainer* t, const int32_t* pack, const int64_t* hop_sizes, const int64_t* offsets,
+                      int32_t slot, void* stream) {
+    return gs_trainer_gather_ahead(t, pack, hop_sizes, offsets, slot, -1, nullptr, nullptr, nullptr, -1, -1, stream);
+}
+
+int gs_trainer_gather_slot_info(const gs_trainer* t, int32_t slot, int64_t* info) {
+    GS_API_BEGIN
+    GS_REQUIRE(t && info && slot >= 0 && slot < gs_trainer::kSlots, GS_EINVAL, "bad arguments");
+    const int64_t v[12] = {t->a1_rows,
+                           t->k_ids,
+                           t->top_rows,
+                           t->top_k,
+                           t->rec_rows,
+                           t->ids_tag[slot].tag,
+                           t->top_ready[slot],
+                           t->rec_ready[slot],
+                           t->n_resolve,
+                           t->n_ahead,
+                           t->self_rows,
+                           0};
+    std::copy(v, v + 12, info);
+    GS_API_END
+}
+
+int gs_trainer_gather_slot_copy(gs_trainer* t, int32_t slot, int32_t which, void* buf, int64_t bytes, int32_t write,
+                                void* stream) {
+    GS_API_BEGIN
+    GS_REQUIRE(t && buf && bytes >= 0 && slot >= 0 && slot < gs_trainer::kSlots, GS_EINVAL, "bad arguments");
+    const int64_t xsz = t->cfg.feat_dtype == GS_BF16 ? 2 : 4;
+    void* p = nullptr;
+    int64_t cap = 0;
+    switch (which) {
+        case 0: p = t->a1_slot[slot], cap = t->a1_rows * t->cfg.feat_dim * (t->self_rows ? 2 : 1) * xsz; break;
+        case 1: p = t->ids_slot[slot], cap = t->a1_rows * t->k_ids * 4; break;
+        case 2: p = t->top_slot[slot], cap = t->top_rows * (t->top_k + 1) * 4; break;
+        case 3: p = t->rec_slot[slot], cap = t->rec_rows * 32; break;
+        default: GS_REQUIRE(false, GS_EINVAL, "unknown slot buffer");
+    }
+    GS_REQUIRE(p && bytes <= cap, GS_EINVAL, "slot buffer not reserved or smaller than the copy");
+    GS_REQUIRE(hipMemcpyAsync(write ? p : buf, write ? buf : p, static_cast<size_t>(bytes), hipMemcpyDeviceToDevice,
+                              gs::as_stream(stream)) == hipSuccess,
+               GS_EHIP, "hipMemcpyAsync(gather slot)");
     GS_API_END
 }
 
diff --git a/graphsage-pytorch_amd/csrc/kernels/trainer.hpp b/graphsage-pytorch_amd/csrc/kernels/trainer.hpp
--- a/graphsage-pytorch_amd/csrc/kernels/trainer.hpp
+++ b/graphsage-pytorch_amd/csrc/kernels/trainer.hpp
@@ -26,6 +26,15 @@
     bool self_in_slot[kSlots] = {};
     int32_t* ids_slot[kSlots] = {};
     int k_ids = 0;
+    struct IdsTag {
+        int64_t tag = -1, n_dst = 0;
+        const int32_t* pack = nullptr;
+        hipStream_t stream = nullptr;
+    } ids_tag[kSlots];
+    void clear_ids_tags() {
+        for (IdsTag& g : ids_tag) g = IdsTag{};
+    }
+    int64_t n_resolve = 0, n_ahead = 0;
     int32_t* top_slot[kSlots] = {};
     bool top_ready[kSlots] = {};
     int64_t top_rows = 0;
@@ -37,6 +46,7 @@
     bool use_top = true;
     bool want_self_rows = true;
     bool opt_defer = true;
+    bool gather_ahead = false;
     float* norm_part = nullptr;
     int pstride = 0;
     int npart[2] = {0, 0};
diff --git a/graphsage-pytorch_amd/csrc/runtime/runner.hip b/graphsage-pytorch_amd/csrc/runtime/runner.hip
--- a/graphsage-pytorch_amd/csrc/runtime/runner.hip
+++ b/graphsage-pytorch_amd/csrc/runtime/runner.hip
@@ -188,6 +188,9 @@
     void recycle(gs::SamplerStream& s, bool block);
     bool issue(int64_t b, bool block);
     int take_slot(int64_t b, bool block);
+    const gs::PackSlot* peek_slot(int64_t b);
+    bool dev_peek(int64_t b, DevResult& R);
+    DevResult peeked{};
 };
 
 void gs_runner::recycle(gs::SamplerStream& s, bool block) {
@@ -290,6 +293,24 @@
     GS_REQUIRE(slot.batch == b, GS_EINVAL, "sampler ring out of order");
     if (slot.status != GS_OK) fail(slot.status, slot.error);
     return slot_id;
+}
+
+const gs::PackSlot* gs_runner::peek_slot(int64_t b) {
+    if (b >= n_units) return nullptr;
+    gs::SamplerStream& s = *streams[b % cfg.n_streams];
+    std::unique_lock<std::mutex> lk(s.mu, std::try_to_lock);
+    if (!lk.owns_lock() || s.ready.empty()) return nullptr;
+    const gs::PackSlot& slot = s.slots[s.ready.front()];
+    return slot.batch == b && slot.status == GS_OK ? &slot : nullptr;
+}
+
+bool gs_runner::dev_peek(int64_t b, DevResult& R) {
+    if (b >= n_units) return false;
+    std::unique_lock<std::recursive_mutex> lk(dev_mu, std::try_to_lock);
+    if (!lk.owns_lock()) return false;
+    DevStream& d = dstreams[b % cfg.n_streams];
+    if (d.nq == 0 || d.qb[0] != b || !gs::dsampler_run_ready(d.ds, d.qrun[0])) return false;
+    return gs_dsampler_result_of(d.ds, d.qrun[0], R.hop_sizes, R.offsets, &R.used) == GS_OK;
 }
 
 void gs_runner::dev_enqueue(int w) {
@@ -384,9 +405,14 @@
     const int k = static_cast<int>(b % kDev);
     wait_entry(k);
     stats.wait_ring_s += secs(tr, Clock::now());
+    const int k1 = static_cast<int>((b + 1) % kDev);
     if (devmode) {
         const DevResult& R = dres[b % n_dpack];
-        const int rc = gs_trainer_gather(cfg.trainer, dpack[b % n_dpack], R.hop_sizes, R.offsets, k, side);
+        const bool nx = dev_peek(b + 1, peeked);
+        const int rc = gs_trainer_gather_ahead(cfg.trainer, dpack[b % n_dpack], R.hop_sizes, R.offsets, k, b,
+                                               nx ? dpack[(b + 1) % n_dpack] : nullptr,
+                                               nx ? peeked.hop_sizes : nullptr, nx ? peeked.offsets : nullptr, k1,
+                                               nx ? b + 1 : -1, side);
         if (rc != GS_OK) fail(rc, gs_last_error());
         hip_ok(hipEventRecord(gathered[k], side), "hipEventRecord");
         inflight[k] = {-1, static_cast<int>(b % n_dpack)};
@@ -396,7 +422,10 @@
     }
     const Inflight f{static_cast<int>(b % cfg.n_streams), slot_id};
     PackSlot& slot = streams[f.stream]->slots[f.slot];
-    const int rc = gs_trainer_gather(cfg.trainer, slot.dev, slot.hop_sizes, slot.offsets, k, side);
+    const PackSlot* nx = peek_slot(b + 1);
+    const int rc = gs_trainer_gather_ahead(cfg.trainer, slot.dev, slot.hop_sizes, slot.offsets, k, b,
+                                           nx ? nx->dev : nullptr, nx ? nx->hop_sizes : nullptr,
+                                           nx ? nx->offsets : nullptr, k1, nx ? b + 1 : -1, side);
     if (rc != GS_OK) fail(rc, gs_last_error());
     hip_ok(hipEventRecord(gathered[k], side), "hipEventRecord");
     inflight[k] = f;
diff --git a/graphsage-pytorch_amd/train.py b/graphsage-pytorch_amd/train.py
--- a/graphsage-pytorch_amd/train.py
+++ b/graphsage-pytorch_amd/train.py
@@ -157,7 +157,8 @@
         return out
 
     _OPTIONS = {"fused_bwd": _lib.GS_TOPT_FUSED_BWD, "top_launch": _lib.GS_TOPT_TOP_LAUNCH,
-                "self_rows": _lib.GS_TOPT_SELF_ROWS, "defer_update": _lib.GS_TOPT_DEFER_UPDATE}
+                "self_rows": _lib.GS_TOPT_SELF_ROWS, "defer_update": _lib.GS_TOPT_DEFER_UPDATE,
+                "gather_ahead": _lib.GS_TOPT_GATHER_AHEAD}
 
     def set_option(self, name, value):
         check(lib().gs_trainer_set_option(self._h, self._OPTIONS[name], int(bool(value))))
diff --git a/include/graphsage_amd.h b/include/graphsage_amd.h
--- a/include/graphsage_amd.h
+++ b/include/graphsage_amd.h
@@ -268,6 +268,14 @@
 int gs_trainer_gather_reserve(gs_trainer* t, int64_t max_rows, int32_t max_fanout);
 int gs_trainer_gather(gs_trainer* t, const int32_t* pack, const int64_t* hop_sizes,
                       const int64_t* offsets, int32_t slot, void* stream);
+int gs_trainer_gather_ahead(gs_trainer* t, const int32_t* pack, const int64_t* hop_sizes,
+                            const int64_t* offsets, int32_t slot, int64_t tag,
+                            const int32_t* next_pack, const int64_t* next_hop_sizes,
+                            const int64_t* next_offsets, int32_t next_slot, int64_t next_tag,
+                            void* stream);
+int gs_trainer_gather_slot_info(const gs_trainer* t, int32_t slot, int64_t* info);
+int gs_trainer_gather_slot_copy(gs_trainer* t, int32_t slot, int32_t which, void* buf, int64_t bytes,
+                                int32_t write, void* stream);
 int gs_trainer_forward_backward_gathered(gs_trainer* t, const int32_t* pack,
                                          const int64_t* hop_sizes, const int64_t* offsets,
                                          const int32_t* roots, int64_t n_roots, int32_t slot,
@@ -292,7 +300,13 @@
 int gs_trainer_capture(gs_trainer* t, float* emb, int64_t emb_stride, float* grads, int64_t max_steps);
 int64_t gs_trainer_captured(const gs_trainer* t);
 int gs_trainer_defer(gs_trainer* t, int32_t on, int32_t* active, void* stream);
-enum { GS_TOPT_FUSED_BWD = 0, GS_TOPT_TOP_LAUNCH = 1, GS_TOPT_SELF_ROWS = 2, GS_TOPT_DEFER_UPDATE = 3 };
+enum {
+    GS_TOPT_FUSED_BWD = 0,
+    GS_TOPT_TOP_LAUNCH = 1,
+    GS_TOPT_SELF_ROWS = 2,
+    GS_TOPT_DEFER_UPDATE = 3,
+    GS_TOPT_GATHER_AHEAD = 5
+};
 int gs_trainer_set_option(gs_trainer* t, int32_t opt, int32_t value);
 enum { GS_OPT_SGD = 0, GS_OPT_ADAM = 1 };
 typedef struct {
```

New measurement: 10.14 million. -2.2%, worse.
